# hotchpotch/open_provence

Hardware: AMD Instinct MI355X
Metric: query-context pairs/sec @ seq_len 512, xsmall-v1 (higher is better)
Workload: dtype fp16 single pass (11 significant bits per operand), fp32 accumulate

## Files before the change

include/open_provence_hip.h:

```cpp
#ifndef OPEN_PROVENCE_HIP_H
#define OPEN_PROVENCE_HIP_H

#include <stddef.h>
#include <stdint.h>

#ifdef __cplusplus
extern "C" {
#endif

#define OP_ABI_VERSION 10
#define OP_MAX_LAYERS 128

typedef struct op_handle op_handle;

enum op_status {
  OP_OK = 0,
  OP_ERR_INVALID = -1,
  OP_ERR_UNSUPPORTED = -2,
  OP_ERR_HIP = -3,
  OP_ERR_STATE = -4,
  OP_ERR_WORKSPACE = -5,
  OP_ERR_NOMEM = -6
};

enum op_dtype { OP_DTYPE_F32 = 0, OP_DTYPE_BF16 = 1, OP_DTYPE_F16 = 2 };

enum op_precision { OP_PRECISION_BF16X3 = 0, OP_PRECISION_BF16 = 1, OP_PRECISION_BF16X2 = 2, OP_PRECISION_CUSTOM = 3 };
enum op_term { OP_TERM_LEFT_LO = 1, OP_TERM_RIGHT_LO = 2 };
enum op_gemm_family {
  OP_FAM_WQKV = 0,
  OP_FAM_QK = 1,
  OP_FAM_PV = 2,
  OP_FAM_ATTN_OUT = 3,
  OP_FAM_WI = 4,
  OP_FAM_MLP_OUT = 5,
  OP_FAM_COUNT = 6
};

enum op_flags {
  OP_FLAG_FORCE_TILED = 1,
  OP_FLAG_NO_SMALL_BLOCKS = 2,
  OP_FLAG_ATT_WAVES_4 = 4,
  OP_FLAG_ATT_WAVES_8 = 8,
  OP_FLAG_NO_POLICY_KERNELS = 16,
  OP_FLAG_NO_LAYER_FUSION = 32,
  OP_FLAG_LAYER_8X16 = 64,
  OP_FLAG_NO_HEAD_FUSION = 256,
  OP_FLAG_LAYER_M32 = 128,
  OP_FLAG_ATTN_XCD_GROUP = 1024,
  OP_FLAG_PANEL_F8 = 2048,
  OP_FLAG_PANEL_F8_WI = 4096,
  OP_FLAG_NO_LAYER_PAIRS = 8192,
  OP_FLAG_NO_F8 = 512
};

enum op_pooling { OP_POOL_CLS = 0, OP_POOL_MEAN = 1 };

typedef struct op_config {
  uint32_t struct_bytes;
  int32_t device_id;
  int32_t vocab_size;
  int32_t hidden_size;
  int32_t intermediate_size;
  int32_t num_layers;
  int32_t num_heads;
  int32_t num_labels;
  int32_t local_attention;
  int32_t max_position_embeddings;
  int32_t pooling;
  int32_t precision;
  float norm_eps;
  float global_rope_theta;
  float local_rope_theta;
  int32_t chunk_rows;
  uint8_t layer_is_global[OP_MAX_LAYERS];
  uint8_t terms[8];
  uint32_t flags;
  int32_t prune_pre_final_norm;
} op_config;

int op_abi_version(void);

int op_create(const op_config* cfg, op_handle** out);

int op_load_weight(op_handle* h, const char* name, const void* data, int dtype, const int64_t* shape, int ndim);

int op_weights_ready(op_handle* h);

size_t op_workspace_bytes(const op_handle* h, int n_seqs, int total_tokens, int max_seqlen);

int op_effective_policy(op_handle* h, uint8_t* terms_out, int* kernel_set);

enum op_kernel_set {
  OP_KS_AUTO = -1,
  OP_KS_BF16X3 = 0,
  OP_KS_BF16_WEIGHTS = 1,
  OP_KS_BF16 = 2,
  OP_KS_F16_F8 = 3,
  OP_KS_F16_F8_W = 4,
  OP_KS_BF16X3_WI_F8 = 5,
  OP_KS_BF16_WEIGHTS_WI_F8 = 6,
  OP_KS_F16 = 7,
  OP_KS_F16_MLP_F8_W = 8,
  OP_KS_F16_MLP_F8 = 9,
  OP_KS_F16_F8_W_ATTN_F16 = 10,
  OP_KS_F16_F8_ATTN_F16 = 11,
  OP_KS_COUNT = 12
};

int op_select_kernel_set(op_handle* h, int kernel_set);

typedef struct op_calibration {
  uint32_t struct_bytes;
  float tolerance;
  int32_t reference_set;
  int32_t default_set;
  int32_t chosen_set;
  int32_t n_candidates;
  int32_t candidate_set[16];
  float candidate_err[16];
  int32_t n_rows, n_tokens;
  float default_err;
  uint32_t flags;
  float mlp_layers_err;
  uint64_t mlp_layers;
} op_calibration;
#define OP_CAL_FULL_REPORT 1u
#define OP_CAL_WHOLE_DEPTH 2u
int op_calibrate(op_handle* h, float tolerance, const int32_t* ids_host, const int32_t* cu_seqlens_host, int n_seqs,
                 op_calibration* report);

int op_mlp_correction_layers(op_handle* h, uint64_t* layer_mask);
int op_select_mlp_correction_layers(op_handle* h, uint64_t layer_mask);

int op_set_compact_operands(op_handle* h, int enabled, int* changed);

int op_forward_packed(op_handle* h, const int32_t* ids_dev, const int32_t* cu_seqlens_dev,
                      const int32_t* cu_seqlens_host, int n_seqs, int total_tokens, int max_seqlen,
                      float* prune_logits_dev, float* rank_logits_dev, float* keep_prob_dev,
                      void* workspace_dev, size_t workspace_bytes, void* hip_stream);

enum op_hidden_dtype { OP_HIDDEN_F32 = 0, OP_HIDDEN_BF16 = 1 };
typedef struct op_hidden_request {
  uint32_t struct_bytes;
  int32_t dtype;
  int32_t pad_width;
  const uint8_t* select;
  void* out_dev;
} op_hidden_request;
int op_forward_packed_hidden(op_handle* h, const int32_t* ids_dev, const int32_t* cu_seqlens_dev,
                             const int32_t* cu_seqlens_host, int n_seqs, int total_tokens, int max_seqlen,
                             float* prune_logits_dev, float* rank_logits_dev, float* keep_prob_dev,
                             void* workspace_dev, size_t workspace_bytes, void* hip_stream, const op_hidden_request* req);

int op_segment_means(op_handle* h, const float* keep_prob_dev, int n_values, const int32_t* seg_dev, int n_seg,
                     float* out_dev, void* hip_stream);

int op_debug_capture_hidden(op_handle* h, float* hidden_dev);

typedef struct op_profile_entry {
  int32_t kind;
  int32_t launches;
  double total_ms;
} op_profile_entry;
int op_profile_enable(op_handle* h, int enabled);
int op_profile_read(op_handle* h, op_profile_entry* entries, int max_entries);
int op_profile_reset(op_handle* h);
const char* op_profile_kind_name(int kind);

int op_debug_clock_probe(op_handle* h, int spin_us, unsigned long long* out_dev, void* hip_stream);

int op_device_count(int* count);

void op_destroy(op_handle* h);
const char* op_last_error(const op_handle* h);

#ifdef __cplusplus
}
#endif
#endif
```

open_provence_amd/_lib.py:

```python

from __future__ import annotations

import ctypes
import os
from pathlib import Path

OP_MAX_LAYERS = 128
OP_ABI_VERSION = 10

OP_OK = 0
OP_ERR_INVALID, OP_ERR_UNSUPPORTED, OP_ERR_HIP, OP_ERR_STATE, OP_ERR_WORKSPACE, OP_ERR_NOMEM = -1, -2, -3, -4, -5, -6
OP_DTYPE_F32, OP_DTYPE_BF16, OP_DTYPE_F16 = 0, 1, 2
OP_PRECISION_BF16X3, OP_PRECISION_BF16, OP_PRECISION_BF16X2, OP_PRECISION_CUSTOM = 0, 1, 2, 3
OP_TERM_LEFT_LO, OP_TERM_RIGHT_LO = 1, 2
OP_FAMILIES = ("wqkv", "qk", "pv", "attn_out", "wi", "mlp_out")
OP_FLAG_FORCE_TILED, OP_FLAG_NO_SMALL_BLOCKS, OP_FLAG_ATT_WAVES_4, OP_FLAG_ATT_WAVES_8, OP_FLAG_NO_POLICY_KERNELS = 1, 2, 4, 8, 16
OP_FLAG_NO_LAYER_FUSION = 32
OP_FLAG_LAYER_8X16 = 64
OP_FLAG_LAYER_M32 = 128
OP_FLAG_NO_HEAD_FUSION = 256
OP_FLAG_NO_F8 = 512
OP_FLAG_ATTN_XCD_GROUP = 1024
OP_FLAG_PANEL_F8 = 2048
OP_FLAG_PANEL_F8_WI = 4096
OP_FLAG_NO_LAYER_PAIRS = 8192
OP_POOL_CLS, OP_POOL_MEAN = 0, 1
OP_KS_AUTO = -1
KERNEL_SET_NAMES = {0: "bf16x3", 1: "bf16-weights", 2: "bf16", 3: "f16-f8", 4: "f16-f8-w", 5: "bf16x3+wi-f16-f8-w",
                    6: "bf16-weights+wi-f16-f8", 7: "f16", 8: "f16+mlp-f16-f8-w", 9: "f16+mlp-f16-f8",
                    10: "f16-f8-w+attn-f16", 11: "f16-f8+attn-f16",
                    -1: "all-terms kernels, cleared lo operands"}
KERNEL_SET_IDS = {name: number for number, name in KERNEL_SET_NAMES.items() if number >= 0}
FP16_PLANE_SETS = ("f16-f8", "f16-f8-w", "bf16x3+wi-f16-f8-w", "bf16-weights+wi-f16-f8", "f16", "f16+mlp-f16-f8-w", "f16+mlp-f16-f8",
                   "f16-f8-w+attn-f16", "f16-f8+attn-f16")

LIB_NAME = "libopenprovence_hip.so"

EXPORTED_SYMBOLS = (
    "op_abi_version",
    "op_create",
    "op_load_weight",
    "op_weights_ready",
    "op_effective_policy",
    "op_set_compact_operands",
    "op_select_kernel_set",
    "op_mlp_correction_layers",
    "op_select_mlp_correction_layers",
    "op_calibrate",
    "op_workspace_bytes",
    "op_forward_packed",
    "op_forward_packed_hidden",
    "op_segment_means",
    "op_debug_capture_hidden",
    "op_profile_enable",
    "op_profile_read",
    "op_profile_reset",
    "op_profile_kind_name",
    "op_device_count",
    "op_debug_clock_probe",
    "op_destroy",
    "op_last_error",
)


class HipLibraryError(RuntimeError):
    """The HIP library is missing, failed to load, or returned an error code."""


class OpConfig(ctypes.Structure):
    _fields_ = [
        ("struct_bytes", ctypes.c_uint32),
        ("device_id", ctypes.c_int32),
        ("vocab_size", ctypes.c_int32),
        ("hidden_size", ctypes.c_int32),
        ("intermediate_size", ctypes.c_int32),
        ("num_layers", ctypes.c_int32),
        ("num_heads", ctypes.c_int32),
        ("num_labels", ctypes.c_int32),
        ("local_attention", ctypes.c_int32),
        ("max_position_embeddings", ctypes.c_int32),
        ("pooling", ctypes.c_int32),
        ("precision", ctypes.c_int32),
        ("norm_eps", ctypes.c_float),
        ("global_rope_theta", ctypes.c_float),
        ("local_rope_theta", ctypes.c_float),
        ("chunk_rows", ctypes.c_int32),
        ("layer_is_global", ctypes.c_uint8 * OP_MAX_LAYERS),
        ("terms", ctypes.c_uint8 * 8),
        ("flags", ctypes.c_uint32),
        ("prune_pre_final_norm", ctypes.c_int32),
    ]


class OpCalibration(ctypes.Structure):
    _fields_ = [
        ("struct_bytes", ctypes.c_uint32),
        ("tolerance", ctypes.c_float),
        ("reference_set", ctypes.c_int32),
        ("default_set", ctypes.c_int32),
        ("chosen_set", ctypes.c_int32),
        ("n_candidates", ctypes.c_int32),
        ("candidate_set", ctypes.c_int32 * 16),
        ("candidate_err", ctypes.c_float * 16),
        ("n_rows", ctypes.c_int32),
        ("n_tokens", ctypes.c_int32),
        ("default_err", ctypes.c_float),
        ("flags", ctypes.c_uint32),
        ("mlp_layers_err", ctypes.c_float),
        ("mlp_layers", ctypes.c_uint64),
    ]


class OpHiddenRequest(ctypes.Structure):

    _fields_ = [
        ("struct_bytes", ctypes.c_uint32),
        ("dtype", ctypes.c_int32),
        ("pad_width", ctypes.c_int32),
        ("select", ctypes.POINTER(ctypes.c_uint8)),
        ("out_dev", ctypes.c_void_p),
    ]


OP_HIDDEN_F32, OP_HIDDEN_BF16 = 0, 1

OP_CAL_FULL_REPORT = 1
OP_CAL_WHOLE_DEPTH = 2


class OpProfileEntry(ctypes.Structure):
    _fields_ = [("kind", ctypes.c_int32), ("launches", ctypes.c_int32), ("total_ms", ctypes.c_double)]


def library_path() -> Path:
    override = os.environ.get("OPEN_PROVENCE_HIP_LIB")
    if override:
        return Path(override)
    return Path(__file__).resolve().parent / LIB_NAME


_LIB: ctypes.CDLL | None = None


def load_library() -> ctypes.CDLL:

    global _LIB
    if _LIB is not None:
        return _LIB
    path = library_path()
    if not path.exists():
        raise HipLibraryError(
            f"{path} not found. Build it with `python -c 'import __graft_entry__ as g; g.build()'` "
            "(hipcc --offload-arch=gfx950). There is no CPU or PyTorch fallback for the forward path."
        )
    try:
        lib = ctypes.CDLL(str(path))
    except OSError as exc:
        raise HipLibraryError(f"failed to load {path}: {exc}") from exc

    vp, ci, cs = ctypes.c_void_p, ctypes.c_int, ctypes.c_size_t
    lib.op_abi_version.restype = ci
    lib.op_abi_version.argtypes = []
    lib.op_create.restype = ci
    lib.op_create.argtypes = [ctypes.POINTER(OpConfig), ctypes.POINTER(vp)]
    lib.op_load_weight.restype = ci
    lib.op_load_weight.argtypes = [vp, ctypes.c_char_p, vp, ci, ctypes.POINTER(ctypes.c_int64), ci]
    lib.op_weights_ready.restype = ci
    lib.op_weights_ready.argtypes = [vp]
    lib.op_workspace_bytes.restype = cs
    lib.op_workspace_bytes.argtypes = [vp, ci, ci, ci]
    lib.op_forward_packed.restype = ci
    lib.op_forward_packed.argtypes = [vp, vp, vp, vp, ci, ci, ci, vp, vp, vp, vp, cs, vp]
    if hasattr(lib, "op_forward_packed_hidden"):
        lib.op_forward_packed_hidden.restype = ci
        lib.op_forward_packed_hidden.argtypes = [vp, vp, vp, vp, ci, ci, ci, vp, vp, vp, vp, cs, vp, ctypes.POINTER(OpHiddenRequest)]
    lib.op_effective_policy.restype = ci
    lib.op_effective_policy.argtypes = [vp, ctypes.POINTER(ctypes.c_uint8), ctypes.POINTER(ci)]
    if hasattr(lib, "op_set_compact_operands"):
# ... 50 lines not shown
```

open_provence_amd/csrc/op_api.hip:

```cpp
#include "../../include/open_provence_hip.h"

#include <hip/hip_runtime.h>

#include <algorithm>
#include <cmath>
#include <cstdarg>
#include <cstdio>
#include <cstdlib>
#include <cstring>
#include <string>
#include <vector>

#define OPK_PACK_KERNELS 1
#include "op_internal.h"
#include "opk_small.hip.h"
#include "opk_tiled.hip.h"

using namespace opk;
using opl::Policy;

namespace {

thread_local std::string g_last_error;

// ... 158 lines not shown

struct Launcher {
  op_handle* h;
  hipStream_t stream;
  int begin(int kind) {
    if (!h->profiling) return OP_OK;
    ProfileEvent ev;
    ev.kind = kind;
    OP_HIP(h, hipEventCreate(&ev.start));
    OP_HIP(h, hipEventCreate(&ev.stop));
    OP_HIP(h, hipEventRecord(ev.start, stream));
    h->events.push_back(ev);
    return OP_OK;
  }
  int end() {
    OP_HIP(h, hipGetLastError());
    if (!h->profiling) return OP_OK;
    OP_HIP(h, hipEventRecord(h->events.back().stop, stream));
    return OP_OK;
  }
};

#define OP_TRY(expr)             \
  do {                           \
    int _rc = (expr);            \
    if (_rc != OP_OK) return _rc; \
  } while (0)

int drain_profile(op_handle* h) {
  for (auto& ev : h->events) {
    OP_HIP(h, hipEventSynchronize(ev.stop));
    float ms = 0.f;
    OP_HIP(h, hipEventElapsedTime(&ms, ev.start, ev.stop));
    h->prof_ms[ev.kind] += ms;
    h->prof_launches[ev.kind] += 1;
    (void)hipEventDestroy(ev.start);
    (void)hipEventDestroy(ev.stop);
  }
  h->events.clear();
  return OP_OK;
}

struct Workspace {
  float* x;
  u16 *ln_hi, *ln_lo;
  u16 *q_hi, *q_lo, *k_hi, *k_lo;
  u16 *vt_hi, *vt_lo;
  u16 *o_hi, *o_lo;
  u16 *h_hi, *h_lo;
  int32_t *row_seq, *row_pos, *row_tok, *roff, *qboff, *qboff_l;
  float* cls;
  int* range_flag;
  size_t bytes;
};

int chunk_row_capacity(const op_handle* h, int n_seqs, int total_tokens, int max_seqlen) {
  const long upper = (long)total_tokens + (long)(ROW_ALIGN - 1) * n_seqs;
  const long all_rows = align_up((int)std::min<long>(upper, 1L << 30), ROW_ALIGN);
  const int one_seq = align_up(std::max(max_seqlen, 1), ROW_ALIGN);
  const long cap = std::max(h->chunk_rows, one_seq);
  return (int)std::min<long>(all_rows, cap);
}

void carve(const op_handle* h, char* base, int cap_rows_pad, int n_seqs, Workspace& ws) {
  size_t off = 0;
  auto take = [&](size_t bytes) {
    char* p = base ? base + off : nullptr;
    off += align_up_sz(bytes, 256);
    return p;
  };
  const size_t R = (size_t)cap_rows_pad;
  const size_t H = (size_t)h->H, I = (size_t)h->I;
  ws.x = (float*)take(R * H * 4);
  ws.ln_hi = (u16*)take(R * H * 2);
  ws.ln_lo = (u16*)take(R * H * 2);
  ws.q_hi = (u16*)take(R * H * 2);
  ws.q_lo = (u16*)take(R * H * 2);
  ws.k_hi = (u16*)take(R * H * 2);
  ws.k_lo = (u16*)take(R * H * 2);
  ws.vt_hi = (u16*)take(R * H * 2);
  ws.vt_lo = (u16*)take(R * H * 2);
  ws.o_hi = (u16*)take(R * H * 2);
  ws.o_lo = (u16*)take(R * H * 2);
  ws.h_hi = (u16*)take(R * I * 2);
  ws.h_lo = (u16*)take(R * I * 2);
  ws.row_seq = (int32_t*)take(R * 4);
  ws.row_pos = (int32_t*)take(R * 4);
  ws.row_tok = (int32_t*)take(R * 4);
  ws.roff = (int32_t*)take(((size_t)n_seqs + 1) * 4);
  ws.qboff = (int32_t*)take(((size_t)n_seqs + 1) * 4);
  ws.qboff_l = (int32_t*)take(((size_t)n_seqs + 1) * 4);
  ws.cls = (float*)take(std::max<size_t>((size_t)n_seqs, 1) * H * 4);
  ws.range_flag = (int*)take(sizeof(int));
  ws.bytes = off;
}

template <int EPI>
int launch_gemm(Launcher& L, int kind, const GemmParams& p, bool split) {
  OP_TRY(L.begin(kind));
  const dim3 grid((unsigned)(p.n_tiles * p.m_tiles));
  if (split)
    hipLaunchKernelGGL((gemm_kernel<EPI, true>), grid, dim3(256), 0, L.stream, p);
  else
    hipLaunchKernelGGL((gemm_kernel<EPI, false>), grid, dim3(256), 0, L.stream, p);
  return L.end();
}

int clear_lo(Launcher& L, u16* base, int unit, size_t n_pairs) {
  OP_TRY(L.begin(PK_CLEAR_LO));
  const size_t n = n_pairs * (size_t)(unit / 8);
  hipLaunchKernelGGL(zero_odd_units_kernel, dim3((unsigned)((n + 255) / 256)), dim3(256), 0, L.stream, base, unit, n_pairs);
  return L.end();
}

struct HiddenReq {
  char* out;
  int bf16, pad;
  size_t entry_bytes;
  std::vector<int> slot;
};

struct AttnPlan {
  int waves_g;
  int items_g;
  int items_l;
};

struct ChunkPass {
  op_handle* h;
  Launcher& L;
  const Workspace& ws;
  const int32_t* ids_dev;
  const int32_t* cu_dev;
  int s0, ns, rows, max_len, total_tokens;
  const AttnPlan& plan;
  float *prune_out, *rank_out, *keep_prob;
  const HiddenReq* hid;

  int H, I;
  bool fp_layout;
  int r_pad, m_tiles;
  unsigned row_blocks;
  hipStream_t st;
  Policy E, V;
  bool clr_q, clr_k, clr_v, clr_o, clr_h, clr_ln_attn, clr_ln_mlp, zero_p_lo, split;
  bool o_f8, f16, attn16, range_flagged, embed_in_qkv0;
  size_t plane_bytes;
  int q_tiles;
  bool small_blocks;
  unsigned row_grid;
  const char* no_kernel = "internal: no row-stationary kernel for hidden %d";
  bool layer_fused, head_in_last_layer;
  bool pair_layers;
  bool head_done = false;
  int hidden_stored = -1;

  ChunkPass(op_handle* h_, Launcher& L_, const Workspace& ws_, const int32_t* ids_dev_, const int32_t* cu_dev_, int s0_, int ns_, int rows_,
            int max_len_, int total_tokens_, const AttnPlan& plan_, float* prune_out_, float* rank_out_, float* keep_prob_,
            const HiddenReq* hid_)
      : h(h_), L(L_), ws(ws_), ids_dev(ids_dev_), cu_dev(cu_dev_), s0(s0_), ns(ns_), rows(rows_), max_len(max_len_),
        total_tokens(total_tokens_), plan(plan_), prune_out(prune_out_), rank_out(rank_out_), keep_prob(keep_prob_), hid(hid_) {
    H = h->H;
    I = h->I;
    fp_layout = h->row_path || h->panel_path;
    r_pad = fp_layout ? align_up(rows, ROW_BM) : align_up(rows + 64, 256);
    m_tiles = r_pad / GEMM_BM;
    row_blocks = (unsigned)((r_pad + 3) / 4);
    st = L.stream;
    E = h->eff;
    V = opl::kPolicies[h->pi];
    auto extra = [](int v, int e, int bit) { return (v & bit) != 0 && (e & bit) == 0; };
    clr_q = extra(V.qk, E.qk, 1);
    clr_k = extra(V.qk, E.qk, 2);
    clr_v = extra(V.pv, E.pv, 2);
    clr_o = extra(V.attn_out, E.attn_out, 1);
    clr_h = extra(V.mlp_out, E.mlp_out, 1);
    clr_ln_attn = extra(V.wqkv, E.wqkv, 1);
    clr_ln_mlp = extra(V.wi, E.wi, 1);
    zero_p_lo = extra(V.pv, E.pv, 1);
    split = (E.wqkv | E.qk | E.pv | E.attn_out | E.wi | E.mlp_out) != 0;
    o_f8 = (h->pi == opl::PI_F16_F8 || h->pi == opl::PI_F16_F8_W) && !h->emulate;
    f16 = h->pi == opl::PI_F16 && !h->emulate;
    attn16 = o_f8 && h->attn_f16 && h->panel_path;
    range_flagged = h->panel_path && !h->emulate && (o_f8 || (f16 && h->mlp_f8));
    embed_in_qkv0 = h->row_path && !h->capture && !(h->cfg.flags & OP_FLAG_NO_HEAD_FUSION);
    plane_bytes = (size_t)r_pad * H * sizeof(u16);
    q_tiles = (max_len + ATT_BQ - 1) / ATT_BQ;
    small_blocks = (r_pad / ROW_BM) <= h->n_cus && !(h->cfg.flags & OP_FLAG_NO_SMALL_BLOCKS);
    row_grid = (unsigned)(r_pad / (small_blocks ? 64 : ROW_BM));
    layer_fused = h->row_path && !h->emulate && opl::has_row_layer_fused(h->pi) && !(h->cfg.flags & OP_FLAG_NO_LAYER_FUSION);
    head_in_last_layer = layer_fused && h->cfg.pooling != OP_POOL_MEAN && !h->capture && !(h->cfg.flags & OP_FLAG_NO_HEAD_FUSION);
    pair_layers = layer_fused && H == 256 && I % 64 == 0 && (f16 || h->pi == 2) && !h->capture &&
                  !(h->cfg.flags & (OP_FLAG_NO_LAYER_PAIRS | OP_FLAG_LAYER_8X16 | OP_FLAG_LAYER_M32)) &&
                  h->layers[0].wo_pp[f16 ? 1 : 0] != nullptr;
  }

  int prologue() {
    OP_TRY(L.begin(PK_ROWMAP));
    hipLaunchKernelGGL(seq_offsets_kernel, dim3(1), dim3(1024), 0, st, cu_dev, s0, ns, ROW_ALIGN, ROW_ALIGN, ws.roff);
    if (fp_layout) {
      hipLaunchKernelGGL(seq_offsets_kernel, dim3(1), dim3(1024), 0, st, cu_dev, s0, ns, plan.waves_g * 32, 1, ws.qboff);
      hipLaunchKernelGGL(seq_offsets_kernel, dim3(1), dim3(1024), 0, st, cu_dev, s0, ns, 128, 1, ws.qboff_l);
    }
    hipLaunchKernelGGL(row_map_kernel, dim3((unsigned)((r_pad + 255) / 256)), dim3(256), 0, st, cu_dev, s0, ns, ws.roff,
                       r_pad, ws.row_seq, ws.row_pos, ws.row_tok);
    OP_TRY(L.end());

    if (range_flagged) OP_HIP(h, hipMemsetAsync(ws.range_flag, 0, sizeof(int), st));
    if (fp_layout && o_f8) {
      const size_t n16 = (size_t)((r_pad - rows) / 16);
      if (n16) OP_HIP(h, hipMemsetAsync(ws.o_hi + (size_t)(rows / 16) * (H / 32) * 512, 0, n16 * (H / 32) * 512 * sizeof(u16), st));
      if (n16) OP_HIP(h, hipMemsetAsync(ws.o_lo + (size_t)(rows / 16) * h->nh * 512, 0, n16 * h->nh * 512 * sizeof(u16), st));
    } else if (fp_layout) {
      const size_t tail_off = (size_t)(rows / 16) * (H / 32) * 2 * 512;
      const size_t tail_bytes = (size_t)((r_pad - rows) / 16) * (H / 32) * 2 * 512 * sizeof(u16);
      if (tail_bytes) OP_HIP(h, hipMemsetAsync(ws.o_hi + tail_off, 0, tail_bytes, st));
    } else {
      const size_t tail_off = (size_t)rows * H;
      const size_t tail_bytes = (size_t)(r_pad - rows) * H * sizeof(u16);
      if (tail_bytes) OP_HIP(h, hipMemsetAsync(ws.o_hi + tail_off, 0, tail_bytes, st));
      if (tail_bytes && split) OP_HIP(h, hipMemsetAsync(ws.o_lo + tail_off, 0, tail_bytes, st));
    }

    if (!embed_in_qkv0) {
      OP_TRY(L.begin(PK_EMBED_LN));
      if (split)
        hipLaunchKernelGGL((embed_ln_kernel<true>), dim3(row_blocks), dim3(256), 0, st, ids_dev, ws.row_tok, h->emb,
                           h->emb_norm, h->cfg.norm_eps, H, r_pad, h->V, ws.x, ws.ln_hi, ws.ln_lo);
      else
        hipLaunchKernelGGL((embed_ln_kernel<false>), dim3(row_blocks), dim3(256), 0, st, ids_dev, ws.row_tok, h->emb,
                           h->emb_norm, h->cfg.norm_eps, H, r_pad, h->V, ws.x, ws.ln_hi, ws.ln_lo);
      OP_TRY(L.end());
    }
    return OP_OK;
  }

  int capture(int index) {
    if (!h->capture) return OP_OK;
    OP_TRY(L.begin(PK_CAPTURE));
    hipLaunchKernelGGL(capture_rows_kernel, dim3(row_blocks), dim3(256), 0, st, ws.x, ws.row_tok, H, r_pad,
                       h->capture + (size_t)index * total_tokens * H);
    return L.end();
  }

  void* hidden_entry(int index) const {
    if (!hid || hid->slot[index] < 0) return nullptr;
    return hid->out + (size_t)hid->slot[index] * hid->entry_bytes;
  }
  int hidden(int index, const float* ln = nullptr) {
    void* dst = hidden_entry(index);
    if (!dst) return OP_OK;
    OP_TRY(L.begin(PK_CAPTURE));
    hipLaunchKernelGGL(hidden_rows_kernel, dim3(row_blocks), dim3(256), 0, st, ws.x, ln, h->cfg.norm_eps, H, r_pad,
                       ws.row_tok, ws.row_seq, ws.row_pos, s0, hid->pad, hid->bf16, dst);
    return L.end();
  }

  int attention(bool is_global) {
    OP_TRY(L.begin(is_global ? PK_ATTN_GLOBAL : PK_ATTN_LOCAL));
    const int window = is_global ? -1 : h->cfg.local_attention / 2;
    if (fp_layout) {
      AttnFpParams ap;
      ap.q_fp = ws.q_hi;
      ap.k_fp = ws.k_hi;
      ap.vt_fp = ws.vt_hi;
      ap.o_fp = ws.o_hi;
      ap.o_lo8 = ws.o_lo;
      ap.cu = cu_dev;
      ap.s0 = s0;
      ap.roff = ws.roff;
      ap.qboff = is_global ? ws.qboff : ws.qboff_l;
      ap.ns = ns;
      ap.H = H;
      ap.r_pad = r_pad;
      ap.window = window;
      ap.n_items = is_global ? plan.items_g : plan.items_l;
      ap.n_heads = h->nh;
      ap.xcd_group = (h->panel_path || o_f8 || (h->cfg.flags & OP_FLAG_ATTN_XCD_GROUP)) ? 1 : 0;
      ap.range_flag = range_flagged ? ws.range_flag : nullptr;
      const unsigned item_span = 8u * opk::ATT_ITEM_GROUP;
      const dim3 grid((ap.xcd_group ? ((unsigned)ap.n_items + item_span - 1) / item_span * item_span : (unsigned)ap.n_items) *
                      (unsigned)h->nh);
      if (!opl::launch_attn(st, ap, is_global ? plan.waves_g : 4, is_global ? 2 : 1, h->pi, zero_p_lo && !attn16, grid, attn16))
        return fail(h, OP_ERR_UNSUPPORTED, "internal: no attention kernel for this configuration");
    } else {
      const dim3 grid((unsigned)q_tiles, (unsigned)h->nh, (unsigned)ns);
      AttnParams ap;
      ap.q_hi = ws.q_hi;
      ap.q_lo = ws.q_lo;
      ap.k_hi = ws.k_hi;
      ap.k_lo = ws.k_lo;
      ap.vt_hi = ws.vt_hi;
      ap.vt_lo = ws.vt_lo;
      ap.o_hi = ws.o_hi;
      ap.o_lo = ws.o_lo;
      ap.cu = cu_dev;
      ap.s0 = s0;
      ap.roff = ws.roff;
      ap.H = H;
      ap.r_pad = r_pad;
      ap.window = window;
      ap.zero_p_lo = (E.pv & 1) ? 0 : 1;
      if (split)
        hipLaunchKernelGGL((attn_kernel<true>), grid, dim3(256), 0, st, ap);
      else
        hipLaunchKernelGGL((attn_kernel<false>), grid, dim3(256), 0, st, ap);
    }
    OP_TRY(L.end());
    if (fp_layout && clr_o) OP_TRY(clear_lo(L, ws.o_hi, 512, (size_t)(r_pad / 16) * (H / 32)));
    if (!fp_layout && split && !(E.attn_out & 1)) OP_HIP(h, hipMemsetAsync(ws.o_lo, 0, plane_bytes, st));
    return OP_OK;
  }
  int clear_qkv() {
    if (clr_q) OP_TRY(clear_lo(L, ws.q_hi, 512, (size_t)(r_pad / 16) * (H / 32)));
    if (clr_k) OP_TRY(clear_lo(L, ws.k_hi, 512, (size_t)(r_pad / 16) * (H / 32)));
    if (clr_v) OP_TRY(clear_lo(L, ws.vt_hi, 2048, (size_t)h->nh * (r_pad / 32)));
    return OP_OK;
  }
  int clear_h() {
    if (clr_h) OP_TRY(clear_lo(L, ws.h_hi, 512, (size_t)(r_pad / 16) * (I / 32)));
    return OP_OK;
  }

  RowGemmParams qkv_params(int li) {
    const LayerWeights& lw = h->layers[li];
    const bool is_global = h->cfg.layer_is_global[li] != 0;
    RowGemmParams rp;
    memset(&rp, 0, sizeof(rp));
    rp.eps = h->cfg.norm_eps;
    rp.hidden = H;
    rp.r_pad = r_pad;
    rp.row_pos = ws.row_pos;
    rp.rope_cos = h->rope_cos[is_global ? 1 : 0];
    rp.rope_sin = h->rope_sin[is_global ? 1 : 0];
    rp.max_pos = h->max_pos;
    rp.x_in = ws.x;
    rp.ln_w = lw.attn_norm;
    rp.wp = f16 ? lw.wqkv_h16 : lw.wqkv_pk;
    rp.n_chunks = 3 * H / ROW_CHUNK;
    rp.n_swapped = 2 * H / ROW_CHUNK;
    rp.o0_hi = ws.q_hi;
    rp.o1_hi = ws.k_hi;
    rp.o2_hi = ws.vt_hi;
    rp.ld_out = H;
    rp.zero_a_lo = clr_ln_attn ? 1 : 0;
    return rp;
  }

  int row_layer(int li) {
    const LayerWeights& lw = h->layers[li];
    const bool is_global = h->cfg.layer_is_global[li] != 0;
    if (li == 0) {
      RowGemmParams rp = qkv_params(0);
      if (embed_in_qkv0) {
        rp.emb_table = h->emb;
        rp.emb_ids = ids_dev;
        rp.emb_vocab = h->V;
        rp.row_tok = ws.row_tok;
        rp.ln_w = h->emb_norm;
        rp.x_io = ws.x;
      }
      OP_TRY(L.begin(PK_ROW_QKV));
      if (!opl::launch_row_qkv0(st, rp, H / 32, small_blocks, h->pi, row_grid)) return fail(h, OP_ERR_UNSUPPORTED, no_kernel, H);
      OP_TRY(L.end());
      OP_TRY(clear_qkv());
      if (embed_in_qkv0) OP_TRY(hidden(0));
    }
    OP_TRY(attention(is_global));

    if (layer_fused) {
      const bool with_qkv = li + 1 < h->N;
      if ((h->cfg.flags & OP_FLAG_LAYER_M32) && lw.wo_p32 && opl::has_layer32(h->pi) && I % 64 == 0) {
        Layer32Params lp;
        memset(&lp, 0, sizeof(lp));
        const LayerWeights& nx = h->layers[with_qkv ? li + 1 : li];
        lp.o_fp = ws.o_hi;
        lp.x_io = ws.x;
        lp.ln_mlp = lw.mlp_norm;
        lp.ln_next = with_qkv ? nx.attn_norm : nullptr;
        lp.eps = h->cfg.norm_eps;
        lp.wo_p = lw.wo_p32;
        lp.wi_p = lw.wi_p32;
        lp.wo2_p = lw.wo2_p32;
        lp.wqkv_p = nx.wqkv_p32;
        lp.n_pairs = I / 32;
        lp.q_fp = ws.q_hi;
        lp.k_fp = ws.k_hi;
        lp.vt_fp = ws.vt_hi;
        lp.r_pad = r_pad;
        lp.row_pos = ws.row_pos;
        const int gl = h->cfg.layer_is_global[with_qkv ? li + 1 : li] ? 1 : 0;
        lp.rope_cos = h->rope_cos[gl];
        lp.rope_sin = h->rope_sin[gl];
        lp.max_pos = h->max_pos;
        OP_TRY(L.begin(PK_FUSED_LAYER));
        if (!opl::launch_layer32(st, lp, h->pi, with_qkv, (unsigned)(r_pad / ROW_BM))) return fail(h, OP_ERR_UNSUPPORTED, no_kernel, H);
        OP_TRY(L.end());
        return OP_OK;
      }
      if (pair_layers && with_qkv) {
        Layer32Params lp;
        memset(&lp, 0, sizeof(lp));
        const LayerWeights& nx = h->layers[li + 1];
        lp.o_fp = ws.o_hi;
        lp.x_io = ws.x;
        lp.ln_mlp = lw.mlp_norm;
        lp.ln_next = nx.attn_norm;
        lp.eps = h->cfg.norm_eps;
        lp.wo_p = lw.wo_pp[f16 ? 1 : 0];
        lp.wi_p = lw.wi_pp[f16 ? 1 : 0];
        lp.wo2_p = lw.wo2_pp[f16 ? 1 : 0];
        lp.wqkv_p = nx.wqkv_pp[f16 ? 1 : 0];
        lp.n_pairs = I / 32;
        lp.q_fp = ws.q_hi;
        lp.k_fp = ws.k_hi;
        lp.vt_fp = ws.vt_hi;
        lp.r_pad = r_pad;
        lp.row_pos = ws.row_pos;
        const int gl = h->cfg.layer_is_global[li + 1] ? 1 : 0;
        lp.rope_cos = h->rope_cos[gl];
        lp.rope_sin = h->rope_sin[gl];
        lp.max_pos = h->max_pos;
        lp.hid_out = hidden_entry(li + 1);
        if (lp.hid_out) {
          lp.row_tok = ws.row_tok;
          lp.row_seq = ws.row_seq;
          lp.hid_bf16 = hid->bf16;
          lp.hid_pad = hid->pad;
          lp.hid_s0 = s0;
          hidden_stored = li + 1;
        }
        OP_TRY(L.begin(PK_FUSED_LAYER));
        if (!opl::launch_layer16p(st, lp, f16, true, li > 0, li + 2 < h->N, (unsigned)(r_pad / ROW_BM),
                                  lp.hid_out != nullptr))
          return fail(h, OP_ERR_UNSUPPORTED, no_kernel, H);
        OP_TRY(L.end());
        return OP_OK;
      }
      RowGemmParams rl = qkv_params(with_qkv ? li + 1 : li);
      rl.a1_fp = ws.o_hi;
      rl.w1p = f16 ? lw.wo_h16 : lw.wo_ks;
      rl.k1_steps = H / 32;
      rl.x_io = ws.x;
      rl.ln_w_mlp = lw.mlp_norm;
      rl.wi_pk = f16 ? lw.wi_h16 : lw.wi_pk;
      rl.wo2_ks = f16 ? lw.wo2_h16 : lw.wo2_pk;
      rl.n_pairs = I / 32;
      if (o_f8) {
        rl.a1_lo8 = ws.o_lo;
        rl.w1p = lw.wo_f16;
        rl.w1p8 = lw.wo_f8;
        rl.wi_pk = lw.wi_f8;
        rl.wo2_ks = lw.wo2_f16;
        rl.wp = h->layers[with_qkv ? li + 1 : li].wqkv_f8;
      }
      if (!with_qkv && head_in_last_layer) {
        rl.fin_ln = h->final_norm;
        rl.fin_pw = h->prune_w;
        rl.fin_pb = h->prune_b;
        rl.row_tok = ws.row_tok;
        rl.row_seq = ws.row_seq;
        rl.fin_prune = prune_out;
        rl.fin_keep = keep_prob;
        rl.fin_cls = ws.cls;
        rl.fin_pre_norm = h->cfg.prune_pre_final_norm ? 1 : 0;
        head_done = true;
        rl.hid_out = hidden_entry(h->N);
        if (rl.hid_out) {
          rl.hid_bf16 = hid->bf16;
          rl.hid_pad = hid->pad;
          rl.hid_s0 = s0;
        }
      }
      OP_TRY(L.begin(PK_FUSED_LAYER));
      if (!opl::launch_row_layer_fused(st, rl, H / 32, h->pi, with_qkv, (unsigned)(r_pad / ROW_BM),
                                       (h->cfg.flags & OP_FLAG_LAYER_8X16) != 0 || (opl::kPolicies[h->pi].wi & 1) == 0,
                                       rl.hid_out != nullptr))
        return fail(h, OP_ERR_UNSUPPORTED, no_kernel, H);
      OP_TRY(L.end());
      return OP_OK;
    }

    RowGemmParams rp;
    memset(&rp, 0, sizeof(rp));
    rp.eps = h->cfg.norm_eps;
    rp.hidden = H;
    rp.r_pad = r_pad;
    rp.ln_w = lw.mlp_norm;
    rp.wp = lw.wi_pk;
    rp.n_chunks = 2 * I / ROW_CHUNK;
    rp.o0_hi = ws.h_hi;
    rp.ld_out = I;
    rp.a1_fp = ws.o_hi;
    rp.w1p = lw.wo_ks;
    rp.k1_steps = H / 32;
    rp.x_io = ws.x;
    rp.zero_a_lo = clr_ln_mlp ? 1 : 0;
    OP_TRY(L.begin(PK_FUSED_ATTN_OUT_WI));
    if (!opl::launch_row_geglu_fused(st, rp, H / 32, small_blocks, h->pi, row_grid)) return fail(h, OP_ERR_UNSUPPORTED, no_kernel, H);
    OP_TRY(L.end());
    OP_TRY(clear_h());

    if (li + 1 < h->N) {
      RowGemmParams rq = qkv_params(li + 1);
      rq.a1_fp = ws.h_hi;
      rq.w1p = lw.wo2_pk;
      rq.k1_steps = I / 32;
      rq.x_io = ws.x;
      OP_TRY(L.begin(PK_FUSED_MLP_OUT_QKV));
      if (!opl::launch_row_qkv_fused(st, rq, H / 32, small_blocks, h->pi, row_grid)) return fail(h, OP_ERR_UNSUPPORTED, no_kernel, H);
      OP_TRY(L.end());
      OP_TRY(clear_qkv());
    } else {
      KStreamParams kp;
      kp.a_fp = ws.h_hi;
      kp.wp = lw.wo2_pk;
      kp.n_ksteps = I / 32;
      kp.x = ws.x;
      OP_TRY(L.begin(PK_KSTREAM_MLP_OUT));
      if (!opl::launch_kstream(st, kp, H / 16, h->pi, (unsigned)(r_pad / ROW_BM))) return fail(h, OP_ERR_UNSUPPORTED, no_kernel, H);
      OP_TRY(L.end());
    }
    return OP_OK;
  }

  int panel_layer(int li) {
    const LayerWeights& lw = h->layers[li];
    const bool is_global = h->cfg.layer_is_global[li] != 0;
    const dim3 ln_grid((unsigned)(r_pad / 16));
    const bool pf8 = o_f8;
    const bool mlp8 = f16 && h->mlp_f8 && (li >= 64 || ((h->mlp_layers >> li) & 1ull) != 0);
    const bool wlo8 = h->pi == opl::PI_F16_F8_W || (h->wi_f8 && h->pi == opl::PI_ALL_TERMS) || (mlp8 && h->mlp_wlo);
    auto layer_norm_fp = [&](const float* w, bool with_lo, bool clear, bool f8_here = false) -> int {
      OP_TRY(L.begin(PK_LN));
      if (pf8 || f8_here) {
        hipLaunchKernelGGL(ln_fp8_kernel, ln_grid, dim3(256), 0, st, ws.x, w, h->cfg.norm_eps, H, r_pad, w ? 1 : 0, ws.ln_hi,
                           ws.ln_lo);
        return L.end();
      }
      if (with_lo)
        hipLaunchKernelGGL((ln_fp_kernel<true>), ln_grid, dim3(256), 0, st, ws.x, w, h->cfg.norm_eps, H, r_pad,
                           w ? 1 : 0, ws.ln_hi);
      else if (f16)
        hipLaunchKernelGGL((ln_fp_kernel<false, true>), ln_grid, dim3(256), 0, st, ws.x, w, h->cfg.norm_eps, H, r_pad,
                           w ? 1 : 0, ws.ln_hi);
      else
        hipLaunchKernelGGL((ln_fp_kernel<false>), ln_grid, dim3(256), 0, st, ws.x, w, h->cfg.norm_eps, H, r_pad,
                           w ? 1 : 0, ws.ln_hi);
      OP_TRY(L.end());
      if (clear) OP_TRY(clear_lo(L, ws.ln_hi, 512, (size_t)(r_pad / 16) * (H / 32)));
      return OP_OK;
    };
    auto panel = [&](int kind, int epi, const PanelParams& pp, int n_tiles, bool f8_here = false, bool f8_full = false) -> int {
      OP_TRY(L.begin(kind));
      PanelParams q = pp;
      q.n_tiles = n_tiles;
      q.row_group = 8;
      const unsigned per_xcd = ((unsigned)(r_pad / ROW_BM) + 7) / 8;
      const unsigned groups = (per_xcd + q.row_group - 1) / q.row_group;
      const dim3 grid(8u * groups * (unsigned)q.row_group * (unsigned)n_tiles);
      const bool ok = f8_here ? opl::launch_panel_f8(st, q, 103, wlo8, grid)
                      : f8_full ? opl::launch_panel_f8(st, q, epi, wlo8, grid)
                      : pf8   ? (epi == 102 ? opl::launch_panel_f8_qkv(st, q, wlo8, attn16, grid) : opl::launch_panel_f8(st, q, epi, wlo8, grid))
                              : (epi == 102 ? opl::launch_panel_qkv(st, q, h->pi, grid) : opl::launch_panel(st, q, epi, h->pi, grid));
      if (!ok) return fail(h, OP_ERR_UNSUPPORTED, "internal: no panel kernel");
      return L.end();
    };
    OP_TRY(layer_norm_fp(li != 0 ? lw.attn_norm : nullptr, (V.wqkv & 1) != 0, clr_ln_attn));
    PanelParams pp;
    memset(&pp, 0, sizeof(pp));
    pp.r_pad = r_pad;
    pp.hidden = H;
    pp.range_flag = range_flagged ? ws.range_flag : nullptr;
    pp.row_pos = ws.row_pos;
    pp.rope_cos = h->rope_cos[is_global ? 1 : 0];
    pp.rope_sin = h->rope_sin[is_global ? 1 : 0];
    pp.max_pos = h->max_pos;
    pp.a_fp = ws.ln_hi;
    pp.a_lo8 = ws.ln_lo;
    pp.n_ksteps = H / 32;
    pp.wp = pf8 ? lw.wqkv_p16 : (f16 ? lw.wqkv_h16 : lw.wqkv_pk);
    pp.wp8 = lw.wqkv_p8;
    pp.w8_lo_off = (size_t)3 * H * H / 2;
    pp.o0 = ws.q_hi;
    pp.o1 = ws.k_hi;
    if (pf8 || !(h->cfg.flags & OP_FLAG_NO_LAYER_FUSION)) {
      pp.o2 = ws.vt_hi;
// ... 1236 lines not shown
```

open_provence_amd/csrc/op_internal.h:

```cpp
#pragma once

#include <hip/hip_runtime.h>
#include <stdint.h>

#include "opk_attn.hip.h"
#include "opk_common.hip.h"
#include "opk_layer32.hip.h"
#include "opk_layer16p.hip.h"
#include "opk_panel.hip.h"
#include "opk_rowgemm.hip.h"

namespace opl {

struct Policy {
  int wqkv, qk, pv, attn_out, wi, mlp_out;
  int fmt = 0;
  constexpr bool operator==(const Policy& o) const {
    return wqkv == o.wqkv && qk == o.qk && pv == o.pv && attn_out == o.attn_out && wi == o.wi && mlp_out == o.mlp_out;
  }
};

constexpr Policy kPolicies[] = {
    {3, 3, 3, 3, 3, 3},
    {1, 3, 3, 1, 1, 1},
    {0, 0, 0, 0, 0, 0},
    {1, 3, 3, 1, 1, 1, 1},
    {3, 3, 3, 3, 3, 3, 1},
    {0, 0, 0, 0, 0, 0, 2},
};
constexpr int PI_ALL_TERMS = 0, PI_BF16_WEIGHTS = 1, PI_BF16 = 2, PI_F16_F8 = 3, PI_F16_F8_W = 4, PI_F16 = 5;
constexpr int N_POLICIES = (int)(sizeof(kPolicies) / sizeof(kPolicies[0]));

constexpr int qkv_olo(const Policy& p) { return (p.qk & 1) | (p.qk & 2) | ((p.pv & 2) ? 4 : 0); }
constexpr int h_olo(const Policy& p) { return p.mlp_out & 1; }
constexpr bool o_lo(const Policy& p) { return (p.attn_out & 1) != 0; }

bool launch_row_qkv0(hipStream_t st, const opk::RowGemmParams& p, int ks, bool small, int pi, unsigned grid);
bool launch_row_geglu_fused(hipStream_t st, const opk::RowGemmParams& p, int ks, bool small, int pi, unsigned grid);
bool launch_row_qkv_fused(hipStream_t st, const opk::RowGemmParams& p, int ks, bool small, int pi, unsigned grid);
bool launch_kstream(hipStream_t st, const opk::KStreamParams& p, int nf, int pi, unsigned grid);
bool has_row_layer_fused(int pi);
bool launch_row_layer_fused(hipStream_t st, const opk::RowGemmParams& p, int ks, int pi, bool with_qkv, unsigned grid,
                            bool waves8, bool hout = false);
bool launch_row_layer_f8(hipStream_t st, const opk::RowGemmParams& p, int ks, bool with_qkv, unsigned grid, bool hout);
bool launch_row_layer_f8w(hipStream_t st, const opk::RowGemmParams& p, int ks, bool with_qkv, unsigned grid, bool hout);
bool launch_row_qkv0_h16(hipStream_t st, const opk::RowGemmParams& p, int ks, bool small, unsigned grid);
bool launch_row_layer_h16(hipStream_t st, const opk::RowGemmParams& p, int ks, bool with_qkv, unsigned grid, bool waves8, bool hout);
bool has_layer32(int pi);
bool launch_layer32(hipStream_t st, const opk::Layer32Params& p, int pi, bool with_qkv, unsigned grid);
bool launch_layer16p(hipStream_t st, const opk::Layer32Params& p, bool h16, bool with_qkv, bool xin_t, bool xout_t, unsigned grid,
                     bool hout = false);
bool launch_attn(hipStream_t st, const opk::AttnFpParams& p, int waves, int kt, int pi, bool zero_p_lo, dim3 grid,
                 bool f16_in_f8_out = false);
bool launch_panel(hipStream_t st, const opk::PanelParams& p, int epi, int pi, dim3 grid);
bool launch_panel_qkv(hipStream_t st, const opk::PanelParams& p, int pi, dim3 grid);
bool launch_panel_f8(hipStream_t st, const opk::PanelParams& p, int epi, bool wlo, dim3 grid);
bool launch_panel_f8_qkv(hipStream_t st, const opk::PanelParams& p, bool wlo, bool o16, dim3 grid);

}
```

open_provence_amd/csrc/op_launch_layer32.hip:

```cpp
#include "op_internal.h"

namespace opl {
using namespace opk;

namespace {
template <int PI>
bool launch_pi(hipStream_t st, const Layer32Params& p, bool with_qkv, unsigned grid) {
  constexpr Policy P = kPolicies[PI];
  constexpr bool single_plane = ((P.wqkv | P.attn_out | P.wi | P.mlp_out) & 2) == 0;
  constexpr bool uniform = (P.wqkv & 1) == (P.attn_out & 1) && (P.wi & 1) == (P.mlp_out & 1) && (P.wqkv & 1) == (P.wi & 1);
  if constexpr (!single_plane || !uniform) {
    return false;
  } else {
    constexpr bool ALO = (P.wi & 1) != 0;
    if (with_qkv) hipLaunchKernelGGL((layer32_kernel<8, true, ALO, qkv_olo(P)>), dim3(grid), dim3(256), 0, st, p);
    else hipLaunchKernelGGL((layer32_kernel<8, false, ALO, 0>), dim3(grid), dim3(256), 0, st, p);
    return true;
  }
}
}

bool has_layer32(int pi) {
  if (pi < 0 || pi >= N_POLICIES || kPolicies[pi].fmt != 0) return false;
  const Policy& P = kPolicies[pi];
  return ((P.wqkv | P.attn_out | P.wi | P.mlp_out) & 2) == 0 && (P.wqkv & 1) == (P.attn_out & 1) &&
         (P.wi & 1) == (P.mlp_out & 1) && (P.wqkv & 1) == (P.wi & 1);
}

bool launch_layer32(hipStream_t st, const Layer32Params& p, int pi, bool with_qkv, unsigned grid) {
  static_assert(N_POLICIES == 6, "extend the switch");
  switch (pi) {
    case 0: return launch_pi<0>(st, p, with_qkv, grid);
    case 1: return launch_pi<1>(st, p, with_qkv, grid);
    case 2: return launch_pi<2>(st, p, with_qkv, grid);
    case 3:
    case 4:
    case 5: return false;
    default: return false;
  }
}

bool launch_layer16p(hipStream_t st, const Layer32Params& p, bool h16, bool with_qkv, bool xin_t, bool xout_t, unsigned grid, bool hout) {
  if (hout && !with_qkv) return false;
  const dim3 g(grid), b(512);
#define OPL_L16P(H16, XI, XO)                                                                              \
  do {                                                                                                     \
    if (hout) hipLaunchKernelGGL((layer16p_hout_kernel<8, true, H16, XI, XO>), g, b, 0, st, p);            \
    else if (with_qkv) hipLaunchKernelGGL((layer16p_kernel<8, true, H16, XI, XO>), g, b, 0, st, p);        \
    else hipLaunchKernelGGL((layer16p_kernel<8, false, H16, XI, XO>), g, b, 0, st, p);                     \
  } while (0)
  if (h16) {
    if (xin_t && xout_t) OPL_L16P(true, true, true);
    else if (xin_t) OPL_L16P(true, true, false);
    else if (xout_t) OPL_L16P(true, false, true);
    else OPL_L16P(true, false, false);
  } else {
    if (xin_t && xout_t) OPL_L16P(false, true, true);
    else if (xin_t) OPL_L16P(false, true, false);
    else if (xout_t) OPL_L16P(false, false, true);
    else OPL_L16P(false, false, false);
  }
#undef OPL_L16P
  return true;
}

}
```

open_provence_amd/csrc/op_launch_row.hip:

```cpp
#include "op_internal.h"

namespace opl {
using namespace opk;

namespace {

template <int KS, int EPI, int PRO, int T1, int T2, int OLO>
void launch_shape(hipStream_t st, const RowGemmParams& p, bool small, unsigned grid) {
  if (small)
    hipLaunchKernelGGL((rowgemm_kernel<KS, EPI, PRO, T1, T2, OLO, 4, 1>), dim3(grid), dim3(256), 0, st, p);
  else
    hipLaunchKernelGGL((rowgemm_kernel<KS, EPI, PRO, T1, T2, OLO, 4, 2>), dim3(grid), dim3(256), 0, st, p);
}

template <int KS, int T1, int WAVES, int MF, int TW, int TM, int F8 = 0, bool H16 = false>
void launch_last_layer(hipStream_t st, const RowGemmParams& p, unsigned grid, bool hout) {
  if (hout)
    hipLaunchKernelGGL((rowgemm_hout_kernel<KS, RE_NONE, RP_MLP, T1, 0, 0, WAVES, MF, TW, TM, F8, H16>), dim3(grid), dim3(WAVES * 64), 0,
                       st, p);
  else
    hipLaunchKernelGGL((rowgemm_kernel<KS, RE_NONE, RP_MLP, T1, 0, 0, WAVES, MF, TW, TM, F8, H16>), dim3(grid), dim3(WAVES * 64), 0,
                       st, p);
}

template <int EPI, int PRO, int T1, int T2, int OLO>
bool launch_ks(hipStream_t st, const RowGemmParams& p, int ks, bool small, unsigned grid) {
  if (ks == 8) launch_shape<8, EPI, PRO, T1, T2, OLO>(st, p, small, grid);
  else if (ks == 4) launch_shape<4, EPI, PRO, T1, T2, OLO>(st, p, small, grid);
  else return false;
  return true;
}

}

#define OPL_SWITCH(CALL)                              \
  static_assert(N_POLICIES == 6, "extend the switch"); \
  switch (pi) {                                       \
    case 0: return CALL(0);                           \
    case 1: return CALL(1);                           \
    case 2: return CALL(2);                           \
    case 3: return CALL(1);                           \
    case 4: return CALL(0);                           \
    default: return false;                            \
  }

#if OPL_ROW_PART == 0
bool launch_row_geglu_fused(hipStream_t st, const RowGemmParams& p, int ks, bool small, int pi, unsigned grid) {
#define OPL_CALL(PI) (launch_ks<RE_GEGLU, RP_KSTREAM, kPolicies[PI].attn_out, kPolicies[PI].wi, h_olo(kPolicies[PI])>(st, p, ks, small, grid))
  OPL_SWITCH(OPL_CALL)
#undef OPL_CALL
}
#endif

#if OPL_ROW_PART == 1
bool launch_row_qkv_fused(hipStream_t st, const RowGemmParams& p, int ks, bool small, int pi, unsigned grid) {
#define OPL_CALL(PI) (launch_ks<RE_QKV, RP_KSTREAM, kPolicies[PI].mlp_out, kPolicies[PI].wqkv, qkv_olo(kPolicies[PI])>(st, p, ks, small, grid))
  OPL_SWITCH(OPL_CALL)
#undef OPL_CALL
}
#endif

#if OPL_ROW_PART == 2
bool launch_row_qkv0(hipStream_t st, const RowGemmParams& p, int ks, bool small, int pi, unsigned grid) {
  if (pi == PI_F16) return launch_row_qkv0_h16(st, p, ks, small, grid);
#define OPL_CALL(PI) (launch_ks<RE_QKV, RP_SPLIT, 0, kPolicies[PI].wqkv, qkv_olo(kPolicies[PI])>(st, p, ks, small, grid))
  OPL_SWITCH(OPL_CALL)
#undef OPL_CALL
}

namespace {
template <int T>
bool launch_kstream_t(hipStream_t st, const KStreamParams& p, int nf, unsigned grid) {
  if (nf == 16) hipLaunchKernelGGL((kstream_gemm_kernel<16, T, 4>), dim3(grid), dim3(256), 0, st, p);
  else if (nf == 8) hipLaunchKernelGGL((kstream_gemm_kernel<8, T, 4>), dim3(grid), dim3(256), 0, st, p);
  else return false;
  return true;
}
}

bool launch_kstream(hipStream_t st, const KStreamParams& p, int nf, int pi, unsigned grid) {
#define OPL_CALL(PI) (launch_kstream_t<kPolicies[PI].mlp_out>(st, p, nf, grid))
  OPL_SWITCH(OPL_CALL)
#undef OPL_CALL
}
#endif

#if OPL_ROW_PART == 3
namespace {
template <int PI, int KS>
bool launch_layer_ks(hipStream_t st, const RowGemmParams& p, bool with_qkv, unsigned grid, bool waves8, bool hout) {
  constexpr Policy P = kPolicies[PI];
  if constexpr ((P.wi & 2) != 0 || (P.mlp_out & 2) != 0) {
    return false;
  } else {
    if (waves8 && with_qkv)
      hipLaunchKernelGGL((rowgemm_kernel<KS, RE_QKV, RP_MLP, P.attn_out, P.wqkv, qkv_olo(P), 8, 1, P.wi, P.mlp_out>), dim3(grid),
                         dim3(512), 0, st, p);
    else if (waves8)
      launch_last_layer<KS, P.attn_out, 8, 1, P.wi, P.mlp_out>(st, p, grid, hout);
    else if (with_qkv)
      hipLaunchKernelGGL((rowgemm_kernel<KS, RE_QKV, RP_MLP, P.attn_out, P.wqkv, qkv_olo(P), 4, 2, P.wi, P.mlp_out>), dim3(grid),
                         dim3(256), 0, st, p);
    else
      launch_last_layer<KS, P.attn_out, 4, 2, P.wi, P.mlp_out>(st, p, grid, hout);
    return true;
  }
}
template <int PI>
bool launch_layer_pi(hipStream_t st, const RowGemmParams& p, int ks, bool with_qkv, unsigned grid, bool waves8, bool hout) {
  if (ks == 8) return launch_layer_ks<PI, 8>(st, p, with_qkv, grid, waves8, hout);
  if (ks == 4) return launch_layer_ks<PI, 4>(st, p, with_qkv, grid, waves8, hout);
  return false;
}
}

bool has_row_layer_fused(int pi) {
  return pi == PI_F16_F8_W || pi == PI_F16 || (pi >= 0 && pi < N_POLICIES && (kPolicies[pi].wi & 2) == 0 && (kPolicies[pi].mlp_out & 2) == 0);
}

bool launch_row_layer_fused(hipStream_t st, const RowGemmParams& p, int ks, int pi, bool with_qkv, unsigned grid, bool waves8, bool hout) {
  if (hout && (with_qkv || p.fin_ln == nullptr)) return false;
  if (pi == PI_F16_F8) return !waves8 && launch_row_layer_f8(st, p, ks, with_qkv, grid, hout);
  if (pi == PI_F16_F8_W) return !waves8 && launch_row_layer_f8w(st, p, ks, with_qkv, grid, hout);
  if (pi == PI_F16) return launch_row_layer_h16(st, p, ks, with_qkv, grid, waves8, hout);
#define OPL_CALL(PI) (launch_layer_pi<PI>(st, p, ks, with_qkv, grid, waves8, hout))
  OPL_SWITCH(OPL_CALL)
#undef OPL_CALL
}
#endif

#if OPL_ROW_PART == 4
namespace {
template <int KS>
void launch_layer_f8_ks(hipStream_t st, const RowGemmParams& p, bool with_qkv, unsigned grid, bool hout) {
  constexpr Policy P = kPolicies[PI_F16_F8];
  if (with_qkv)
    hipLaunchKernelGGL((rowgemm_kernel<KS, RE_QKV, RP_MLP, P.attn_out, P.wqkv, qkv_olo(P), 4, 2, P.wi, P.mlp_out, 1>), dim3(grid),
                       dim3(256), 0, st, p);
  else
    launch_last_layer<KS, P.attn_out, 4, 2, P.wi, P.mlp_out, 1>(st, p, grid, hout);
}
}

bool launch_row_layer_f8(hipStream_t st, const RowGemmParams& p, int ks, bool with_qkv, unsigned grid, bool hout) {
  if (ks == 8) launch_layer_f8_ks<8>(st, p, with_qkv, grid, hout);
  else if (ks == 4) launch_layer_f8_ks<4>(st, p, with_qkv, grid, hout);
  else return false;
  return true;
}
#endif

#if OPL_ROW_PART == 5
namespace {
template <int KS>
void launch_layer_f8w_ks(hipStream_t st, const RowGemmParams& p, bool with_qkv, unsigned grid, bool hout) {
  constexpr Policy P = kPolicies[PI_F16_F8_W];
  if (with_qkv)
    hipLaunchKernelGGL((rowgemm_kernel<KS, RE_QKV, RP_MLP, P.attn_out, P.wqkv, qkv_olo(P), 4, 2, P.wi, P.mlp_out, 2>), dim3(grid),
                       dim3(256), 0, st, p);
  else
    launch_last_layer<KS, P.attn_out, 4, 2, P.wi, P.mlp_out, 2>(st, p, grid, hout);
}
}

bool launch_row_layer_f8w(hipStream_t st, const RowGemmParams& p, int ks, bool with_qkv, unsigned grid, bool hout) {
  if (ks == 8) launch_layer_f8w_ks<8>(st, p, with_qkv, grid, hout);
  else if (ks == 4) launch_layer_f8w_ks<4>(st, p, with_qkv, grid, hout);
  else return false;
  return true;
}
#endif

#if OPL_ROW_PART == 6
namespace {
template <int KS>
void launch_qkv0_h16_ks(hipStream_t st, const RowGemmParams& p, bool small, unsigned grid) {
  if (small) hipLaunchKernelGGL((rowgemm_kernel<KS, RE_QKV, RP_SPLIT, 0, 0, 0, 4, 1, 0, 0, 0, true>), dim3(grid), dim3(256), 0, st, p);
  else hipLaunchKernelGGL((rowgemm_kernel<KS, RE_QKV, RP_SPLIT, 0, 0, 0, 4, 2, 0, 0, 0, true>), dim3(grid), dim3(256), 0, st, p);
}
template <int KS>
void launch_layer_h16_ks(hipStream_t st, const RowGemmParams& p, bool with_qkv, unsigned grid, bool waves8, bool hout) {
  if (waves8 && with_qkv)
    hipLaunchKernelGGL((rowgemm_kernel<KS, RE_QKV, RP_MLP, 0, 0, 0, 8, 1, 0, 0, 0, true>), dim3(grid), dim3(512), 0, st, p);
  else if (waves8)
    launch_last_layer<KS, 0, 8, 1, 0, 0, 0, true>(st, p, grid, hout);
  else if (with_qkv)
    hipLaunchKernelGGL((rowgemm_kernel<KS, RE_QKV, RP_MLP, 0, 0, 0, 4, 2, 0, 0, 0, true>), dim3(grid), dim3(256), 0, st, p);
  else
    launch_last_layer<KS, 0, 4, 2, 0, 0, 0, true>(st, p, grid, hout);
}
}

bool launch_row_qkv0_h16(hipStream_t st, const RowGemmParams& p, int ks, bool small, unsigned grid) {
  if (ks == 8) launch_qkv0_h16_ks<8>(st, p, small, grid);
  else if (ks == 4) launch_qkv0_h16_ks<4>(st, p, small, grid);
  else return false;
  return true;
}

bool launch_row_layer_h16(hipStream_t st, const RowGemmParams& p, int ks, bool with_qkv, unsigned grid, bool waves8, bool hout) {
  if (ks == 8) launch_layer_h16_ks<8>(st, p, with_qkv, grid, waves8, hout);
  else if (ks == 4) launch_layer_h16_ks<4>(st, p, with_qkv, grid, waves8, hout);
  else return false;
  return true;
}
#endif

}
```

open_provence_amd/csrc/opk_layer16p_body.inc:

```
  static_assert(NT == 8, "written for hidden = 256");
  static_assert(!HOUT || QKV, "the hidden-state store rides on the q / k / v^T loop's x stores");
  constexpr int H = NT * 32;
  constexpr int KP = NT;
  constexpr int CHUNK = KP * 2 * 512;
  constexpr int SLAB = NT * 2 * 512;
  constexpr int STAGE = 2 * CHUNK + SLAB;
  constexpr int STAGE_B = STAGE * 2;
  constexpr int EXTRA = 16 * 512;
  constexpr int XCH_B = STAGE_B;
  constexpr int HX_B = 2 * STAGE_B;
  constexpr int STAGE_PIECES = STAGE / 512;
  constexpr int O_PIECE0 = 80;
  constexpr int SW_ELEMS = (O_PIECE0 + 64) * 512;
  static_assert(SW_ELEMS >= 2 * STAGE + EXTRA && O_PIECE0 * 512 >= STAGE + 32 * 512, "the o pieces lie behind phase 1's stages");
  __shared__ __attribute__((aligned(16))) u16 sW[SW_ELEMS];
  __shared__ __attribute__((aligned(16))) float sLn[2 * H];
  __shared__ __attribute__((aligned(16))) float sStat[8 * 2 * 16 * 2];

  const int tid = threadIdx.x;
  const int lane = tid & 63;
  const int wave = __builtin_amdgcn_readfirstlane(tid >> 6);
  const int pw = wave & 3, hf = wave >> 2;
  const int n16 = lane & 15, g = lane >> 4;
  const int m0 = blockIdx.x * 128 + pw * 32;
  int hid_row[2] = {-1, -1};
  if constexpr (HOUT) {
#pragma unroll
    for (int mf = 0; mf < 2; ++mf) {
      const int row = m0 + 16 * mf + n16;
      const int tok = p.row_tok[row];
      if (tok >= 0) hid_row[mf] = (int)hidden_dst_row(tok, p.row_seq[row], p.row_pos[row], p.hid_pad, p.hid_s0);
    }
  }
#ifdef OPK_TIMING
  unsigned long long opk_ts[8] = {0, 0, 0, 0, 0, 0, 0, 0}, opk_wait = 0, opk_x[4] = {0, 0, 0, 0};
  const unsigned long long opk_rt0 = wall_clock64();
#define L16P_STAMP(i) opk_ts[i] = __builtin_readcyclecounter()
#else
#define L16P_STAMP(i)
#endif
  L16P_STAMP(0);
  if (hf) __builtin_amdgcn_s_setprio(1);

  const int ln_i = tid < H ? tid : H - 1;
  const float ln_fill0 = p.ln_mlp[ln_i];
  float ln_fill1 = 0.f;
  if (QKV) ln_fill1 = p.ln_next[ln_i];

  const uint32_t lds0 = (uint32_t)(uintptr_t)((__attribute__((address_space(3))) u16*)&sW[0]) + (uint32_t)lane * 16u;
  const uint32_t stat_addr = (uint32_t)(uintptr_t)((__attribute__((address_space(3))) float*)&sStat[0]);
  auto dma_piece = [&](const u16* src_piece0, int dst_piece) {
    __builtin_amdgcn_global_load_lds((const __attribute__((address_space(1))) void*)(src_piece0 + lane * 8),
                                     (__attribute__((address_space(3))) void*)(&sW[dst_piece * 512]), 16, 0, 0);
  };
  const uint32_t lane16 = (uint32_t)lane * 16u;
  auto weight_rsrc = [](const u16* base) { return __builtin_amdgcn_make_buffer_rsrc(const_cast<u16*>(base), 0, 0x7fffffff, 0x00020000); };
  const __amdgpu_buffer_rsrc_t rs_wo = weight_rsrc(p.wo_p), rs_wi = weight_rsrc(p.wi_p), rs_wo2 = weight_rsrc(p.wo2_p), rs_qkv = weight_rsrc(p.wqkv_p);
  auto dma_weight = [&](__amdgpu_buffer_rsrc_t rsrc, uint32_t byte_off, int dst_piece) {
    __builtin_amdgcn_raw_ptr_buffer_load_lds(rsrc, (__attribute__((address_space(3))) void*)(&sW[dst_piece * 512]), 16, (int)lane16, (int)byte_off, 0, 0);
  };
  const f32x4 zero4 = {0.f, 0.f, 0.f, 0.f};

  bf16x8 a[2][KP];
  const size_t rb0 = (size_t)(m0 >> 4);
#pragma unroll
  for (int j = 0; j < 8; ++j) {
    const int mf = j >> 2, kp = 4 * hf + (j & 3);
    dma_piece(p.o_fp + (((rb0 + mf) * NT + kp) * 2) * 512, O_PIECE0 + (2 * pw + mf) * 8 + kp);
  }
  auto stage_p1 = [&](int j, int stage) {
#pragma unroll
    for (int u = 0; u < 4; ++u) {
      const int piece = wave + 8 * u;
      dma_weight(rs_wo, (uint32_t)(((2 * j) * SLAB + piece * 512) * 2), stage * STAGE_PIECES + piece);
    }
  };
  stage_p1(0, 0);
  stage_p1(1, 1);
  __builtin_amdgcn_sched_barrier(0);
  float* xrow = p.x_io + (size_t)(m0 + n16) * H + 128 * hf + 8 * g;
  float* xtile = p.x_io + ((size_t)(m0 >> 5) * NT + 4 * hf) * 1024 + lane * 4;
  float4 xa[4][2][2];
#pragma unroll
  for (int i = 0; i < 4; ++i)
#pragma unroll
    for (int mf = 0; mf < 2; ++mf)
#pragma unroll
      for (int fh = 0; fh < 2; ++fh)
        xa[i][mf][fh] = XIN_T ? load_stream_f4(xtile + i * 1024 + (2 * mf + fh) * 256) : load_stream_f4(xrow + (size_t)(16 * mf) * H + 32 * i + 4 * fh);
  __builtin_amdgcn_sched_barrier(0);
  sLn[ln_i] = ln_fill0;
  sLn[H + ln_i] = ln_fill1;
  asm volatile("s_waitcnt lgkmcnt(0)" ::: "memory");
  asm volatile("s_waitcnt vmcnt(16)" ::: "memory");
  block_barrier();
#ifdef OPK_TIMING
  opk_x[0] = __builtin_readcyclecounter();
#endif
  {
    const uint32_t o_addr = lds0 + (uint32_t)(O_PIECE0 * 1024) + (uint32_t)pw * 16384u;
    static_for<16>([&](auto f_tag) {
      constexpr int f = decltype(f_tag)::value;
      a[f >> 3][f & 7] = lds_read_frag<f * 1024>(o_addr);
    });
    asm volatile("s_waitcnt lgkmcnt(0)"
                 : "+v"(a[0][0]), "+v"(a[0][1]), "+v"(a[0][2]), "+v"(a[0][3]), "+v"(a[0][4]), "+v"(a[0][5]), "+v"(a[0][6]), "+v"(a[0][7]),
                   "+v"(a[1][0]), "+v"(a[1][1]), "+v"(a[1][2]), "+v"(a[1][3]), "+v"(a[1][4]), "+v"(a[1][5]), "+v"(a[1][6]), "+v"(a[1][7]));
  }

  f32x4 acc1[4][2][2];
  struct P1Off {
    static constexpr int at(int st, int j) { return ((st >> 2) * 16 + 2 * (st & 3) + j) * 1024; }
    static constexpr int base(int, int) { return 0; }
  };
  auto p1_stage = [&](auto j_tag) {
    constexpr int j = decltype(j_tag)::value;
    const uint32_t addr[1] = {lds0 + (uint32_t)((j & 1) * STAGE_B) + (uint32_t)hf * 8192u};
    frag_stream_m<8, 2, 2, P1Off, 1>(addr, [&](auto step_tag, bf16x8(&w)[2]) {
      constexpr int st = decltype(step_tag)::value;
      constexpr int kp = 2 * j + (st >> 2), i = st & 3;
#pragma unroll
      for (int fh = 0; fh < 2; ++fh)
#pragma unroll
        for (int mf = 0; mf < 2; ++mf) acc1[i][fh][mf] = mfma16x<H16>(w[fh], a[mf][kp], kp == 0 ? zero4 : acc1[i][fh][mf]);
    });
  };
  p1_stage(std::integral_constant<int, 0>{});
  block_barrier();
  stage_p1(2, 0);
  p1_stage(std::integral_constant<int, 1>{});
  block_barrier();
  stage_p1(3, 1);
  asm volatile("s_waitcnt vmcnt(4)" ::: "memory");
  block_barrier();
  p1_stage(std::integral_constant<int, 2>{});
  asm volatile("s_waitcnt vmcnt(0)" ::: "memory");
  block_barrier();

  const int n_it = p.n_pairs;
  auto stage_piece = [&](auto u_tag, int t, int stage) {
    constexpr int u = decltype(u_tag)::value;
    const int tc = t < n_it ? t : n_it - 1;
    const int ts = t >= 2 ? (t - 2 < n_it ? t - 2 : n_it - 1) : 0;
    const int piece = wave + 8 * u;
    if constexpr (u < 4) dma_weight(rs_wi, (uint32_t)(((2 * tc) * CHUNK + piece * 512) * 2), stage * STAGE_PIECES + piece);
    else dma_weight(rs_wo2, (uint32_t)((ts * SLAB + (piece - 32) * 512) * 2), stage * STAGE_PIECES + piece);
  };
  static_for<6>([&](auto u) { stage_piece(u, 0, 0); });
  p1_stage(std::integral_constant<int, 3>{});
  block_barrier();
  L16P_STAMP(1);

  auto layer_ln = [&](auto load_tag, int which) {
    constexpr bool LOAD = decltype(load_tag)::value;
    float mean_a[2], m2_a[2];
    if constexpr (!LOAD) {
      asm volatile("s_nop 15\n\ts_nop 7"
                   : "+v"(acc1[0][0][0]), "+v"(acc1[0][0][1]), "+v"(acc1[0][1][0]), "+v"(acc1[0][1][1]), "+v"(acc1[1][0][0]), "+v"(acc1[1][0][1]),
                     "+v"(acc1[1][1][0]), "+v"(acc1[1][1][1]), "+v"(acc1[2][0][0]), "+v"(acc1[2][0][1]), "+v"(acc1[2][1][0]), "+v"(acc1[2][1][1]),
                     "+v"(acc1[3][0][0]), "+v"(acc1[3][0][1]), "+v"(acc1[3][1][0]), "+v"(acc1[3][1][1]));
    }
#pragma unroll
    for (int mf = 0; mf < 2; ++mf) {
      f32x2 v[4][4];
#pragma unroll
      for (int i = 0; i < 4; ++i)
#pragma unroll
        for (int fh = 0; fh < 2; ++fh) {
          f32x4 t = acc1[i][fh][mf];
          if constexpr (LOAD) {
            const float4 x4 = xa[i][mf][fh];
            t[0] += x4.x;
            t[1] += x4.y;
            t[2] += x4.z;
            t[3] += x4.w;
            acc1[i][fh][mf] = t;
          }
          v[i][2 * fh] = f32x2{t[0], t[1]};
          v[i][2 * fh + 1] = f32x2{t[2], t[3]};
        }
      f32x2 s4[4];
#pragma unroll
      for (int i = 0; i < 4; ++i)
#pragma unroll
        for (int q = 0; q < 4; ++q) s4[q] = i == 0 ? v[i][q] : pk_add(s4[q], v[i][q]);
      const f32x2 st2 = pk_add(pk_add(s4[0], s4[1]), pk_add(s4[2], s4[3]));
      float sum = st2.x + st2.y;
      sum += __shfl_xor(sum, 16, 64);
      sum += __shfl_xor(sum, 32, 64);
      mean_a[mf] = sum * (1.0f / 128.0f);
      const f32x2 ma2 = f32x2{mean_a[mf], mean_a[mf]};
      f32x2 q4s[4];
#pragma unroll
      for (int i = 0; i < 4; ++i)
#pragma unroll
        for (int q = 0; q < 4; ++q) {
          const f32x2 c = pk_sub(v[i][q], ma2);
          q4s[q] = i == 0 ? pk_mul(c, c) : pk_fma(c, c, q4s[q]);
        }
      const f32x2 qt2 = pk_add(pk_add(q4s[0], q4s[1]), pk_add(q4s[2], q4s[3]));
// ... 35 lines not shown
    const uint32_t oth = lds0 + (uint32_t)XCH_B + (uint32_t)(((wave ^ 4) * 8) * 1024);
    static_for<8>([&](auto f_tag) {
      constexpr int f = decltype(f_tag)::value;
      a[f >> 2][4 + (f & 3)] = lds_read_frag<f * 1024>(oth);
    });
    asm volatile("s_waitcnt lgkmcnt(0)" : "+v"(a[0][4]), "+v"(a[0][5]), "+v"(a[0][6]), "+v"(a[0][7]), "+v"(a[1][4]), "+v"(a[1][5]), "+v"(a[1][6]), "+v"(a[1][7]));
  };
  auto store_rows = [&]() {
#pragma unroll
    for (int i = 0; i < 4; ++i)
#pragma unroll
      for (int mf = 0; mf < 2; ++mf)
#pragma unroll
        for (int fh = 0; fh < 2; ++fh) {
          const f32x4 t = acc1[i][fh][mf];
          store_stream16(XOUT_T ? xtile + i * 1024 + (2 * mf + fh) * 256 : xrow + (size_t)(16 * mf) * H + 32 * i + 4 * fh, make_float4(t[0], t[1], t[2], t[3]));
        }
  };
  const std::true_type yes_{};
  const std::false_type no_{};

  layer_ln(yes_, 0);
  block_barrier();
  const uint32_t hx_pair = lds0 + (uint32_t)HX_B + (uint32_t)((pw * 2) * 1024);
  const uint32_t hx_own = hx_pair + (uint32_t)hf * 8u;
  {
    lds_write_u2(hx_own, 0u, 0u);
    lds_write_u2(hx_own + 1024u, 0u, 0u);
    lds_write_u2(hx_own + 8192u, 0u, 0u);
    lds_write_u2(hx_own + 8192u + 1024u, 0u, 0u);
  }

  f32x4 na[2][2][2];
#pragma unroll
  for (int q = 0; q < 8; ++q) na[q >> 2][(q >> 1) & 1][q & 1] = zero4;
  float gx[8], gq[8];
#pragma unroll
  for (int i = 0; i < 8; ++i) gx[i] = gq[i] = 0.f;
  const uint32_t b_lo = lds0 + (uint32_t)hf * (16384u + 8192u);
  const uint32_t b_hi = lds0 + (uint32_t)hf * (16384u - 8192u);
  const uint32_t b_wo = lds0 + 32768u + (uint32_t)hf * 8192u;
  struct MlpOff {
    static constexpr int at(int s, int j) { return j == 1 ? s * 1024 : (2 * s + (j >> 1)) * 1024; }
    static constexpr int base(int s, int j) { return j == 1 ? 2 : (s < 4 ? 0 : 1); }
  };
  struct WoOff {
    static constexpr int at(int s, int j) { return (2 * s + j) * 1024; }
    static constexpr int base(int, int) { return 0; }
  };
  auto geglu_stage = [&](auto stg_tag, const f32x4 (&src)[2][2], uint32_t dst_addr) {
    constexpr int stg = decltype(stg_tag)::value;
    static_for<8>([&](auto i_tag) {
      constexpr int i = decltype(i_tag)::value, mf = i >> 2, r = i & 3;
      if constexpr (stg == 0) {
        gx[i] = src[0][mf][r];
        gq[i] = gelu_erf_poly(0.f, fabsf(gx[i]), 0);
      } else if constexpr (stg < 5) gq[i] = gelu_erf_poly(gq[i], fabsf(gx[i]), stg);
      else if constexpr (stg == 5) gq[i] = __builtin_amdgcn_exp2f(gq[i]);
      else if constexpr (stg == 6) gq[i] = gelu_erf_finish(gq[i], gx[i]);
      else gq[i] = gq[i] * src[1][mf][r];
    });
    if constexpr (stg == 7) {
      lds_write_u2(dst_addr, pack2x<H16>(gq[0], gq[1]), pack2x<H16>(gq[2], gq[3]));
      lds_write_u2(dst_addr + 1024u, pack2x<H16>(gq[4], gq[5]), pack2x<H16>(gq[6], gq[7]));
    }
  };
  auto interleave6 = [&]() {
#pragma unroll
    for (int i = 0; i < 6; ++i) {
      __builtin_amdgcn_sched_group_barrier(0x008, 1, 0);
      __builtin_amdgcn_sched_group_barrier(0x002, 2, 0);
    }
  };
  auto end_of_stage = [&]() {
#ifdef OPK_TIMING
    const unsigned long long w0_ = __builtin_readcyclecounter();
#endif
    asm volatile("s_waitcnt vmcnt(0) lgkmcnt(0)" ::: "memory");
    block_barrier();
#ifdef OPK_TIMING
    opk_wait += __builtin_readcyclecounter() - w0_;
#endif
  };
  auto macro = [&](int t, auto par_tag) {
    constexpr int P = decltype(par_tag)::value;
    bf16x8 hb[2];
    hb[0] = lds_read_frag<0>(hx_pair + (uint32_t)(P * 8192));
    hb[1] = lds_read_frag<1024>(hx_pair + (uint32_t)(P * 8192));
    const uint32_t addr[3] = {b_lo + (uint32_t)(P * STAGE_B), b_hi + (uint32_t)(P * STAGE_B), b_wo + (uint32_t)(P * STAGE_B)};
    const uint32_t h_dst = hx_own + (uint32_t)((P ^ 1) * 8192);
    frag_stream_m<8, 3, 1, MlpOff, 3>(addr, [&](auto step_tag, bf16x8(&w)[3]) {
      constexpr int s = decltype(step_tag)::value;
      if constexpr (s == 0) asm volatile("" : "+v"(hb[0]), "+v"(hb[1]));
      if constexpr (s < 6) stage_piece(step_tag, t + 1, P ^ 1);
#pragma unroll
      for (int mf = 0; mf < 2; ++mf) na[P][0][mf] = mfma16x<H16>(w[0], a[mf][s], s == 0 ? zero4 : na[P][0][mf]);
#pragma unroll
      for (int mf = 0; mf < 2; ++mf) acc1[s >> 1][s & 1][mf] = mfma16x<H16>(w[1], hb[mf], acc1[s >> 1][s & 1][mf]);
#pragma unroll
      for (int mf = 0; mf < 2; ++mf) na[P][1][mf] = mfma16x<H16>(w[2], a[mf][s], s == 0 ? zero4 : na[P][1][mf]);
      geglu_stage(step_tag, na[P ^ 1], h_dst);
      interleave6();
    });
    end_of_stage();
  };
  asm volatile("s_waitcnt vmcnt(0) lgkmcnt(0)" ::: "memory");
  block_barrier();
  L16P_STAMP(2);
  {
    int t = 0;
    do {
      macro(t, std::integral_constant<int, 0>{});
      macro(t + 1, std::integral_constant<int, 1>{});
      t += 2;
    } while (t < n_it);
  }
  {
    bf16x8 hb[2];
    hb[0] = lds_read_frag<0>(hx_pair);
    hb[1] = lds_read_frag<1024>(hx_pair);
    {
      const uint32_t addr[1] = {b_wo};
      frag_stream_m<4, 2, 1, WoOff, 1>(addr, [&](auto step_tag, bf16x8(&w)[2]) {
        constexpr int s = decltype(step_tag)::value;
        if constexpr (s == 0) asm volatile("" : "+v"(hb[0]), "+v"(hb[1]));
        if constexpr (s < 2) stage_piece(std::integral_constant<int, 4 + s>{}, n_it + 1, 1);
#pragma unroll
        for (int fh = 0; fh < 2; ++fh)
#pragma unroll
          for (int mf = 0; mf < 2; ++mf) acc1[s][fh][mf] = mfma16x<H16>(w[fh], hb[mf], acc1[s][fh][mf]);
        geglu_stage(std::integral_constant<int, 2 * s>{}, na[1], hx_own + 8192u);
        geglu_stage(std::integral_constant<int, 2 * s + 1>{}, na[1], hx_own + 8192u);
      });
    }
    end_of_stage();
    hb[0] = lds_read_frag<0>(hx_pair + 8192u);
    hb[1] = lds_read_frag<1024>(hx_pair + 8192u);
    {
      const uint32_t addr[1] = {b_wo + (uint32_t)STAGE_B};
      frag_stream_m<4, 2, 1, WoOff, 1>(addr, [&](auto step_tag, bf16x8(&w)[2]) {
        constexpr int s = decltype(step_tag)::value;
        if constexpr (s == 0) asm volatile("" : "+v"(hb[0]), "+v"(hb[1]));
#pragma unroll
        for (int fh = 0; fh < 2; ++fh)
#pragma unroll
          for (int mf = 0; mf < 2; ++mf) acc1[s][fh][mf] = mfma16x<H16>(w[fh], hb[mf], acc1[s][fh][mf]);
      });
    }
  }
  block_barrier();
  L16P_STAMP(3);

  if constexpr (!QKV) {
    store_rows();
    L16P_STAMP(4);
  } else {
    constexpr int N_IT = 3 * NT / 2;
    constexpr int N_SW = 2 * NT / 2;
    auto stage_pair = [&](int it, int stage) {
#pragma unroll
      for (int u = 0; u < 4; ++u) {
        const int piece = wave + 8 * u;
        dma_weight(rs_qkv, (uint32_t)(((2 * it) * CHUNK + piece * 512) * 2), stage * STAGE_PIECES + piece);
      }
    };
    stage_pair(0, 0);
    f32x4 rc[2], rs[2];
#pragma unroll
    for (int mf = 0; mf < 2; ++mf) {
      int pos = p.row_pos[m0 + 16 * mf + n16];
      pos = pos < 0 ? 0 : (pos >= p.max_pos ? p.max_pos - 1 : pos);
      rc[mf] = *reinterpret_cast<const f32x4*>(p.rope_cos + (size_t)pos * ROPE_HALF + 16 * hf + 4 * g);
      rs[mf] = *reinterpret_cast<const f32x4*>(p.rope_sin + (size_t)pos * ROPE_HALF + 16 * hf + 4 * g);
    }
    layer_ln(no_, 1);
#ifdef OPK_TIMING
    opk_x[2] = __builtin_readcyclecounter();
#endif
    asm volatile("s_waitcnt vmcnt(0)" ::: "memory");
#ifdef OPK_TIMING
    opk_x[3] = __builtin_readcyclecounter();
#endif
    block_barrier();
    L16P_STAMP(4);

    struct QkvOff {
      static constexpr int at(int s, int j) { return (2 * s + j) * 1024; }
      static constexpr int base(int s, int) { return s < 4 ? 0 : 1; }
    };
    f32x4 qa[2][2][2];
    uint2 st_v[4];
    uint4 st_w[2];
    u16* st_p[2] = {nullptr, nullptr};
    float e_lo[4], e_hi[4];
    auto epilogue_slice = [&](int it, auto sw_tag, auto s_tag, const f32x4 (&c)[2][2]) {
      constexpr bool SW = decltype(sw_tag)::value;
      constexpr int s = decltype(s_tag)::value, mf = s >> 2, r = s & 3;
      if constexpr (SW) {
        const bool is_q = it < N_SW / 2;
        const float qscale = is_q ? 0.125f * 1.44269504088896340736f : 1.0f;
        const float cc = rc[mf][r], ss = rs[mf][r];
        e_lo[r] = rope_lo(c[0][mf][r], c[1][mf][r], cc, ss) * qscale;
        e_hi[r] = rope_hi(c[0][mf][r], c[1][mf][r], cc, ss) * qscale;
        if constexpr (r == 3) {
          st_v[2 * mf] = make_uint2(pack2x<H16>(e_lo[0], e_lo[1]), pack2x<H16>(e_lo[2], e_lo[3]));
          st_v[2 * mf + 1] = make_uint2(pack2x<H16>(e_hi[0], e_hi[1]), pack2x<H16>(e_hi[2], e_hi[3]));
          const int head = is_q ? it : it - N_SW / 2;
          u16* out = is_q ? p.q_fp : p.k_fp;
          st_p[mf] = out + (((rb0 + mf) * NT + 2 * head) * 2) * 512 + (16 * (2 * hf + (g >> 1)) + n16) * 8 + 4 * (g & 1);
        }
      } else {
        if constexpr (s == 7) {
#pragma unroll
          for (int fh = 0; fh < 2; ++fh)
            st_w[fh] = make_uint4(pack2x<H16>(c[fh][0][0], c[fh][0][1]), pack2x<H16>(c[fh][0][2], c[fh][0][3]),
                                  pack2x<H16>(c[fh][1][0], c[fh][1][1]), pack2x<H16>(c[fh][1][2], c[fh][1][3]));
          const size_t tb = (size_t)(m0 >> 5);
          st_p[0] = p.vt_fp + ((((size_t)(it - N_SW) * (size_t)(p.r_pad >> 5) + tb) * 2) * 4 + 2 * hf) * 512 + lane * 8;
        }
      }
    };
    auto epilogue_store = [&](auto sw_tag) {
      constexpr bool SW = decltype(sw_tag)::value;
      if constexpr (SW) {
#pragma unroll
        for (int mf = 0; mf < 2; ++mf) {
          store_stream8(st_p[mf], st_v[2 * mf]);
          store_stream8(st_p[mf] + 1024, st_v[2 * mf + 1]);
        }
      } else {
        store_stream16(st_p[0], st_w[0]);
        store_stream16(st_p[0] + 512, st_w[1]);
      }
    };
    auto interleave4 = [&]() {
#pragma unroll
      for (int i = 0; i < 4; ++i) {
        __builtin_amdgcn_sched_group_barrier(0x008, 1, 0);
        __builtin_amdgcn_sched_group_barrier(0x002, 2, 0);
      }
    };
    auto iteration = [&](auto it_tag, auto first_tag, auto sw_tag, auto swp_tag) {
      constexpr int it = decltype(it_tag)::value, cur = it & 1;
      constexpr bool FIRST = decltype(first_tag)::value, SW = decltype(sw_tag)::value, SWP = decltype(swp_tag)::value;
      constexpr bool XS = it < 8;
      stage_pair(it + 1 < N_IT ? it + 1 : it, cur ^ 1);
      __builtin_amdgcn_sched_barrier(0);
      const uint32_t addr[2] = {b_lo + (uint32_t)(cur * STAGE_B), b_hi + (uint32_t)(cur * STAGE_B)};
      frag_stream_m<8, 2, 2, QkvOff, 2>(addr, [&](auto step_tag, bf16x8(&w)[2]) {
        constexpr int s = decltype(step_tag)::value;
#pragma unroll
        for (int fh = 0; fh < 2; ++fh)
#pragma unroll
          for (int mf = 0; mf < 2; ++mf)
            qa[cur][fh][mf] = SW ? mfma16x<H16>(w[fh], a[mf][s], s == 0 ? zero4 : qa[cur][fh][mf]) : mfma16x<H16>(a[mf][s], w[fh], s == 0 ? zero4 : qa[cur][fh][mf]);
        if constexpr (!FIRST) {
          epilogue_slice(it - 1, swp_tag, step_tag, qa[cur ^ 1]);
          interleave4();
        }
      });
      if constexpr (!FIRST) epilogue_store(swp_tag);
      if constexpr (XS) {
#pragma unroll
        for (int fh = 0; fh < 2; ++fh) {
          const f32x4 t = acc1[it >> 1][fh][it & 1];
          store_stream16(XOUT_T ? xtile + (it >> 1) * 1024 + (2 * (it & 1) + fh) * 256 : xrow + (size_t)(16 * (it & 1)) * H + 32 * (it >> 1) + 4 * fh,
                       make_float4(t[0], t[1], t[2], t[3]));
        }
        if constexpr (HOUT) {
          const int hr = hid_row[it & 1];
          if (hr >= 0) {
#pragma unroll
            for (int fh = 0; fh < 2; ++fh) {
              const f32x4 t = acc1[it >> 1][fh][it & 1];
              const size_t e = (size_t)hr * H + 128 * hf + 8 * g + 32 * (it >> 1) + 4 * fh;
              if (p.hid_bf16)
                store_stream8(reinterpret_cast<u16*>(p.hid_out) + e, make_uint2(pack_bf16x2(t[0], t[1]), pack_bf16x2(t[2], t[3])));
              else
                store_stream16(reinterpret_cast<float*>(p.hid_out) + e, make_float4(t[0], t[1], t[2], t[3]));
            }
          }
        }
      }
      constexpr int N_STORES = (FIRST ? 0 : (SWP ? 4 : 2)) + (XS ? 2 : 0);
      asm volatile("s_waitcnt vmcnt(%0)" ::"n"(N_STORES) : "memory");
      block_barrier();
    };
    iteration(std::integral_constant<int, 0>{}, yes_, yes_, yes_);
    static_for<N_SW - 1>([&](auto j_tag) { iteration(std::integral_constant<int, 1 + decltype(j_tag)::value>{}, no_, yes_, yes_); });
    iteration(std::integral_constant<int, N_SW>{}, no_, no_, yes_);
    static_for<N_IT - N_SW - 1>([&](auto j_tag) { iteration(std::integral_constant<int, N_SW + 1 + decltype(j_tag)::value>{}, no_, no_, no_); });
    static_for<8>([&](auto s_tag) { epilogue_slice(N_IT - 1, no_, s_tag, qa[1]); });
    epilogue_store(no_);
  }
  L16P_STAMP(5);
#ifdef OPK_TIMING
  if (threadIdx.x == 0) {
    for (int i = 0; i < 8; ++i) p.dbg[(size_t)blockIdx.x * 16 + i] = opk_ts[i];
    p.dbg[(size_t)blockIdx.x * 16 + 8] = opk_wait;
    for (int i = 0; i < 4; ++i) p.dbg[(size_t)blockIdx.x * 16 + 11 + i] = opk_x[i];
    p.dbg[(size_t)blockIdx.x * 16 + 15] = wall_clock64() - opk_rt0;
  }
#endif
#undef L16P_STAMP
```

open_provence_amd/csrc/opk_layer32.hip.h:

```cpp
#pragma once

#include <type_traits>
#include <utility>

#include "opk_common.hip.h"

namespace opk {


typedef float f32x16 __attribute__((ext_vector_type(16)));

__device__ __forceinline__ f32x16 mfma32(bf16x8 a, bf16x8 b, f32x16 c) {
  return __builtin_amdgcn_mfma_f32_32x32x16_bf16(a, b, c, 0, 0, 0);
}

enum Layer32Pack { L32_RESID = 0, L32_GEGLU = 1, L32_QKV = 2 };

__host__ __device__ inline int l32_source_row(int mode, int T, int m, int H, int I) {
  const int j = m >> 3, hh = (m >> 2) & 1, r = m & 3;
  if (mode == L32_RESID)
    return 32 * T + 16 * (j >> 1) + 8 * hh + 4 * (j & 1) + r;
  if (mode == L32_GEGLU) {
    const int col = 16 * T + 8 * hh + 4 * (j & 1) + r;
    return j < 2 ? col : I + col;
  }
  const int per = H / 32;
  if (T < 2 * per) {
    const int blk = T / per, cc = T % per;
    const int d = 16 * (cc & 1) + 8 * hh + 4 * (j & 1) + r + (j >= 2 ? 32 : 0);
    return blk * H + (cc >> 1) * HEAD_DIM + d;
  }
  const int cv = T - 2 * per, nf = m >> 4, dd = m & 15;
  return 2 * H + (cv >> 1) * HEAD_DIM + 32 * (cv & 1) + 8 * (dd >> 2) + 4 * nf + (dd & 3);
}

#ifdef OPK_PACK_KERNELS
__global__ void pack_layer32_kernel(const float* __restrict__ src, int n_rows, int K, int mode, int kmajor, int H, int I,
                                    u16* __restrict__ dst, int f16 = 0) {
  const size_t idx = (size_t)blockIdx.x * blockDim.x + threadIdx.x;
  if (idx >= (size_t)n_rows * K) return;
  const int KS = K / 16, NT = n_rows / 32;
  size_t t = idx;
  const int e = (int)(t & 7); t >>= 3;
  const int l = (int)(t & 63); t >>= 6;
  int T, s;
  if (kmajor) {
    T = (int)(t % NT);
    s = (int)(t / NT);
  } else {
    s = (int)(t % KS);
    T = (int)(t / KS);
  }
  const int row = l32_source_row(mode, T, l & 31, H, I);
  const float v = src[(size_t)row * K + 16 * s + 8 * (l >> 5) + e];
  dst[idx] = f16 ? f2h(v) : f2bf(v);
}
#endif

struct Layer32Params {
#ifdef OPK_TIMING
  unsigned long long* dbg;
#endif
  const u16* o_fp;
  float* x_io;
  const float* ln_mlp;
  const float* ln_next;
  float eps;
  const u16* wo_p;
  const u16* wi_p;
  const u16* wo2_p;
  const u16* wqkv_p;
  int n_pairs;
  u16* q_fp;
  u16* k_fp;
  u16* vt_fp;
  int r_pad;
  const int32_t* row_pos;
  const float* rope_cos;
  const float* rope_sin;
  int max_pos;
  const int32_t* row_tok;
  const int32_t* row_seq;
  void* hid_out;
  int hid_bf16;
  int hid_pad;
  int hid_s0;
};

template <int NT, bool QKV, bool ALO, int OLO>
__global__ __launch_bounds__(256, 1) void layer32_kernel(Layer32Params p) {
  constexpr int H = NT * 32;
  constexpr int KS = NT * 2;
  constexpr int CHUNK = KS * 512;
  constexpr int SLAB = NT * 512;
  constexpr int STAGE = 2 * CHUNK + 2 * SLAB;
  static_assert(NT == 8, "written for hidden = 256 (4 waves share the DMA of a 48 KiB stage)");
  __shared__ __attribute__((aligned(16))) u16 sW[2][STAGE];
  __shared__ __attribute__((aligned(16))) float sLn[2 * H];

  const int tid = threadIdx.x;
  const int lane = tid & 63;
  const int wave = __builtin_amdgcn_readfirstlane(tid >> 6);
  const int n = lane & 31, hh = lane >> 5;
  const int m0 = blockIdx.x * 128 + wave * 32;
#ifdef OPK_TIMING
  unsigned long long opk_ts[8] = {0, 0, 0, 0, 0, 0, 0, 0}, opk_wait = 0;
  const unsigned long long opk_rt0 = wall_clock64();
#define L32_STAMP(i) opk_ts[i] = __builtin_readcyclecounter()
#else
#define L32_STAMP(i)
#endif
  L32_STAMP(0);

  const int ln_i = tid < H ? tid : H - 1;
  const float ln_fill0 = p.ln_mlp[ln_i];
  float ln_fill1 = 0.f;
  if (QKV) ln_fill1 = p.ln_next[ln_i];

  uint32_t lds_stage[2];
  lds_stage[0] = (uint32_t)(uintptr_t)((__attribute__((address_space(3))) u16*)&sW[0][0]) + (uint32_t)lane * 16u;
  lds_stage[1] = lds_stage[0] + (uint32_t)(STAGE * 2);
  auto dma_piece = [&](const u16* src_piece0, int stage, int dst_piece) {
    __builtin_amdgcn_global_load_lds((const __attribute__((address_space(1))) void*)(src_piece0 + lane * 8),
                                     (__attribute__((address_space(3))) void*)(&sW[stage][dst_piece * 512]), 16, 0, 0);
  };

  bf16x8 a_hi[KS], a_lo[KS];
  {
    const u16* o_base = p.o_fp + ((size_t)((m0 >> 4) + (n >> 4)) * NT * 2) * 512 + (16 * hh + (n & 15)) * 8;
#pragma unroll
    for (int ks = 0; ks < KS; ++ks) {
      const u16* src = o_base + ((ks >> 1) * 2) * 512 + (ks & 1) * 256;
      a_hi[ks] = load_stream_frag(src);
      a_lo[ks] = ALO ? load_stream_frag(src + 512) : a_hi[ks];
    }
  }
  auto stage_p1 = [&](int j, int stage) {
#pragma unroll
    for (int u = 0; u < NT; ++u) {
      const int piece = wave + 4 * u;
      dma_piece(p.wo_p + (size_t)(4 * j) * SLAB + piece * 512, stage, piece);
    }
  };
  stage_p1(0, 0);
  __builtin_amdgcn_sched_barrier(0);
  float* xrow = p.x_io + (size_t)(m0 + n) * H + 8 * hh;
  float4 xa[NT / 2][2][2];
#pragma unroll
  for (int T = 0; T < NT / 2; ++T)
#pragma unroll
    for (int jj = 0; jj < 2; ++jj)
#pragma unroll
      for (int q4 = 0; q4 < 2; ++q4) xa[T][jj][q4] = load_stream_f4(xrow + 32 * T + 16 * jj + 4 * q4);
  __builtin_amdgcn_sched_barrier(0);
  sLn[ln_i] = ln_fill0;
  sLn[H + ln_i] = ln_fill1;
  asm volatile("s_waitcnt lgkmcnt(0)" ::: "memory");
  asm volatile("s_waitcnt vmcnt(%0)" ::"n"(NT * 2) : "memory");
  __builtin_amdgcn_s_barrier();

  f32x16 acc1[NT];
  {
    struct P1Off {
      static constexpr int at(int st, int j) { return ((st >> 2) * NT + 2 * (st & 3) + j) * 1024; }
    };
    static_for<KS / 4>([&](auto j_tag) {
      constexpr int j = decltype(j_tag)::value;
      constexpr int cur = j & 1;
      if constexpr (j + 1 < KS / 4) stage_p1(j + 1, cur ^ 1);
      __builtin_amdgcn_sched_barrier(0);
      frag_stream2<16, 2, P1Off>(lds_stage[cur], [&](auto step_tag, bf16x8& w0, bf16x8& w1) {
        constexpr int st = decltype(step_tag)::value;
        constexpr int ks = 4 * j + (st >> 2), T = 2 * (st & 3);
        const f32x16 zero = {0.f, 0.f, 0.f, 0.f, 0.f, 0.f, 0.f, 0.f, 0.f, 0.f, 0.f, 0.f, 0.f, 0.f, 0.f, 0.f};
        if (ALO) {
          acc1[T] = mfma32(w0, a_lo[ks], ks == 0 ? zero : acc1[T]);
          acc1[T + 1] = mfma32(w1, a_lo[ks], ks == 0 ? zero : acc1[T + 1]);
        }
        acc1[T] = mfma32(w0, a_hi[ks], (ks == 0 && !ALO) ? zero : acc1[T]);
        acc1[T + 1] = mfma32(w1, a_hi[ks], (ks == 0 && !ALO) ? zero : acc1[T + 1]);
      });
      __syncthreads();
    });
  }
  L32_STAMP(1);

  auto layer_ln = [&](auto load_tag, auto lo_tag, int which) {
    constexpr bool LOAD = decltype(load_tag)::value, LO = decltype(lo_tag)::value;
    float4 xb[LOAD ? NT / 2 : 1][2][2];
    if (LOAD) {
#pragma unroll
      for (int T = NT / 2; T < NT; ++T)
#pragma unroll
        for (int jj = 0; jj < 2; ++jj)
#pragma unroll
          for (int q4 = 0; q4 < 2; ++q4) xb[LOAD ? T - NT / 2 : 0][jj][q4] = load_stream_f4(xrow + 32 * T + 16 * jj + 4 * q4);
    }
    const uint32_t ln_addr = (uint32_t)(uintptr_t)((__attribute__((address_space(3))) float*)&sLn[0]) + (uint32_t)(which * H + 8 * hh) * 4u;
    f32x4 wq[2][2];
    auto ln_read = [&](auto st_tag) {
      constexpr int st = decltype(st_tag)::value;
      wq[st & 1][0] = lds_read_f4<(32 * (st >> 1) + 16 * (st & 1)) * 4>(ln_addr);
      wq[st & 1][1] = lds_read_f4<(32 * (st >> 1) + 16 * (st & 1)) * 4 + 16>(ln_addr);
    };
    f32x2 v[NT][8];
    f32x2 s4[4];
#pragma unroll
    for (int T = 0; T < NT; ++T) {
      f32x16 a = acc1[T];
      if (LOAD) {
#pragma unroll
        for (int jj = 0; jj < 2; ++jj)
#pragma unroll
          for (int q4 = 0; q4 < 2; ++q4) {
            const float4 x4 = T < NT / 2 ? xa[T < NT / 2 ? T : 0][jj][q4] : xb[(LOAD && T >= NT / 2) ? T - NT / 2 : 0][jj][q4];
            a[8 * jj + 4 * q4 + 0] += x4.x;
            a[8 * jj + 4 * q4 + 1] += x4.y;
            a[8 * jj + 4 * q4 + 2] += x4.z;
            a[8 * jj + 4 * q4 + 3] += x4.w;
          }
        acc1[T] = a;
      }
#pragma unroll
      for (int pp = 0; pp < 8; ++pp) {
        v[T][pp] = f32x2{a[2 * pp], a[2 * pp + 1]};
        s4[pp & 3] = (T == 0 && pp < 4) ? v[T][pp] : pk_add(s4[pp & 3], v[T][pp]);
      }
    }
    const f32x2 st = pk_add(pk_add(s4[0], s4[1]), pk_add(s4[2], s4[3]));
    float sum = st.x + st.y;
    sum += __shfl_xor(sum, 32, 64);
    const float mean = sum * (1.0f / (float)H);
    const f32x2 m2 = f32x2{mean, mean};
    f32x2 q4s[4];
#pragma unroll
    for (int T = 0; T < NT; ++T)
#pragma unroll
      for (int pp = 0; pp < 8; ++pp) {
        v[T][pp] = pk_sub(v[T][pp], m2);
// ... 333 lines not shown
```

open_provence_amd/csrc/opk_rowgemm.hip.h:

```cpp
#pragma once

#include "opk_rowgemm_pack.hip.h"
#include "opk_rowgemm_stream.hip.h"
#include "opk_rowgemm_ln.hip.h"

namespace opk {

template <int KS, int EPI, int PRO, int T1, int T2, int OLO, int WAVES, int MF, int TW, int TM, int F8, bool H16, bool HOUT = false>
struct RowGemmBlock {
  static constexpr bool WLO = F8 == 2;
  static_assert(!H16 || (F8 == 0 && T1 == 0 && T2 == 0 && OLO == 0 && TW == 0 && TM == 0 && PRO != RP_KSTREAM && EPI != RE_GEGLU),
                "fp16 operands: the single-pass whole-layer / layer-0 q/k/v kernels only");
  static constexpr int TF8 = WLO ? 3 : T_LEFT_LO;
  static_assert(!F8 || (PRO == RP_MLP && WAVES == 4 && MF == 2 && KS % 4 == 0 && T1 == TF8 && TW == TF8 && TM == TF8 &&
                        (EPI == RE_NONE || T2 == TF8)),
                "f16 + fp8 kernel sets: whole-layer kernel, 4 waves x 32 rows, every activation lo term (+ F8 = 2: every weight lo term)");
  static constexpr int NS8 = F8 ? KS / 4 : 1;
  static_assert(MF == 1 || MF == 2, "one or two 16-row fragments per wave");
  static constexpr bool W_LO = !F8 && (T2 & T_RIGHT_LO) != 0, A_LO = (T2 & T_LEFT_LO) != 0;
  static constexpr bool PHASE1 = PRO == RP_KSTREAM || PRO == RP_MLP;
  static constexpr bool W_LO1 = !F8 && PHASE1 && (T1 & T_RIGHT_LO) != 0, A_LO1 = PHASE1 && (T1 & T_LEFT_LO) != 0;
  static_assert(PRO != RP_MLP || (((WAVES == 4 && MF == 2) || (WAVES == 8 && MF == 1)) && (WLO || ((TW & T_RIGHT_LO) == 0 && (TM & T_RIGHT_LO) == 0))),
                "fused MLP: 4 waves x 32 rows or 8 waves x 16 rows, single-plane Wi and Wo");
  static constexpr int PLANES = W_LO ? 2 : 1;
  static constexpr int PLANES1 = W_LO1 ? 2 : 1;
  static constexpr int K = KS * 32;
  static constexpr int CHUNK_PIECES8 = F8Chunk<KS, WLO>::PIECES;
  static constexpr int CHUNK_SRC = F8 ? F8Chunk<KS, WLO>::SRC_PIECES * 512 : KS * 2 * 1024;
  static constexpr int STAGE = F8 ? CHUNK_PIECES8 * 512 : KS * PLANES * 1024;
  static constexpr int MLP_UNIT = PRO == RP_MLP ? (WLO ? (CHUNK_PIECES8 + 2 * KS) * 512 : F8 ? (2 * CHUNK_PIECES8 + 2 * KS) * 512 : 3 * KS * 1024) : 0;
  static constexpr int STAGE_GEMM = WLO ? 8 * KS * 512 : F8 ? 6 * KS * 512 : KS * (PLANES > PLANES1 ? PLANES : PLANES1) * 1024;
  static constexpr int STAGE_ALLOC = STAGE_GEMM > MLP_UNIT ? STAGE_GEMM : MLP_UNIT;
  static_assert(STAGE % (WAVES * 512) == 0, "stage must split evenly over the waves");
  static constexpr bool LN_V2 = PRO == RP_MLP;
  static_assert(!F8 || LN_V2, "f16 + fp8 kernel set: LayerNorm phases of the whole-layer kernel");
  static constexpr bool FIN_HEAD = LN_V2 && EPI == RE_NONE;
  static constexpr int SLN_SIZE = LN_V2 ? (FIN_HEAD ? 4 : 2) * KS * 32 : 4;
  static constexpr int WAVE_PIECES = STAGE / (WAVES * 512);
  static constexpr bool QKV2 = PRO == RP_MLP && EPI == RE_QKV && !F8 && H16 && 2 * STAGE <= STAGE_ALLOC;
  static constexpr bool QKV_PAIRS = F8 != 0 && EPI == RE_QKV;
  static constexpr int FRAG_ILV = 4;
  static constexpr int PAIR_DMA = QKV_PAIRS ? 2 * CHUNK_PIECES8 / WAVES : 1;
  static constexpr int PAIR_GS = (2 * CHUNK_PIECES8 / 4) % WAVES == 0 ? 4 : 2;
  static_assert(!QKV_PAIRS || (CHUNK_PIECES8 % PAIR_GS == 0 && (2 * CHUNK_PIECES8 / PAIR_GS) % WAVES == 0 && 2 * STAGE <= STAGE_ALLOC),
                "a chunk pair is whole groups of pieces per wave and fits one LDS stage");
  static constexpr bool ROPE_PRELOAD = EPI == RE_QKV && PRO == RP_MLP;

  const RowGemmParams& p;
  u16 (&sW)[2][STAGE_ALLOC];
  float (&sLn)[SLN_SIZE];
  int tid, lane, wave, l15, g, m0, ln_i;
  float ln_fill0 = 0.f, ln_fill1 = 0.f, ln_fill2 = 0.f, ln_fill3 = 0.f;
  bf16x8 a_hi[MF][KS], a_lo[MF][KS];
  i32x8 a_lo8[MF][NS8];
  i32x8 a_h8[MF][NS8];
  const float* rope_c_row[MF];
  const float* rope_s_row[MF];
  f32x4 rope_c[MF], rope_s[MF];
  f32x4 rope_cc[MF][2], rope_ss[MF][2];
  static constexpr int NF1 = 2 * KS;
  f32x4 acc1[NF1][MF];
  float4 xq0[(PRO == RP_MLP) ? NF1 : 1];
  static constexpr bool MLP_REGS_IN_BLOCK = PRO == RP_MLP && WAVES == 8 && F8 == 0 && T1 == 0 && TW == 0 && TM == 0;
  struct MlpRegs {
    f32x4 acc_b[2][MF];
    uint2 hold_hi[MF];
    uint2 hold_lo[MF];
    bf16x8 h_hi[MF];
    bf16x8 h_lo[MF];
    float g_prev[MF][4];
    float g_cur[MF][4];
    float gx[MF * 4];
    float gq[MF * 4];
    uint2 pk_hi[MF];
    float pk_d[MF][4];
    f32x4 nbv[2][MF];
  } mlp_regs;
  uint32_t lds_stage[2];
#ifdef OPK_TIMING
  unsigned long long opk_ts[8] = {0, 0, 0, 0, 0, 0, 0, 0}, opk_wait = 0, opk_wait2 = 0, opk_wait1 = 0, opk_x[4] = {0, 0, 0, 0}, opk_rt0 = 0;
#ifdef OPK_SEG_TIMING
  unsigned long long opk_seg[3] = {0, 0, 0}, opk_seg_t = 0;
#endif
#endif

  __device__ __forceinline__ RowGemmBlock(const RowGemmParams& p_, u16 (&sW_)[2][STAGE_ALLOC], float (&sLn_)[SLN_SIZE]) : p(p_), sW(sW_), sLn(sLn_) {}

  __device__ __forceinline__ void stage_chunk(int chunk, int stage) {
    const u16* src = p.wp + (size_t)chunk * CHUNK_SRC;
    if constexpr (F8 != 0) {
      constexpr int PIECES = STAGE / 512;
      constexpr int GS = (PIECES / 4) % WAVES == 0 ? 4 : ((PIECES / 2) % WAVES == 0 ? 2 : 1);
      static_for<WAVE_PIECES>([&](auto u_tag) {
        constexpr int u = decltype(u_tag)::value;
        const int piece0 = GS * (wave + WAVES * (u / GS));
        __builtin_amdgcn_global_load_lds((const __attribute__((address_space(1))) void*)(src + piece0 * 512 + lane * 8),
                                         (__attribute__((address_space(3))) void*)(&sW[stage][piece0 * 512]), 16, (u % GS) * 1024, 0);
      });
      return;
    }
#pragma unroll
    for (int u = 0; u < WAVE_PIECES; ++u) {
      const int piece = wave + WAVES * u;
      const int elem = piece * 512;
      const int ks = elem / (PLANES * 1024);
      const int rem = elem % (PLANES * 1024);
      const int src_elem = F8 ? elem : ks * 2048 + rem;
      __builtin_amdgcn_global_load_lds(
          (const __attribute__((address_space(1))) void*)(src + src_elem + lane * 8),
          (__attribute__((address_space(3))) void*)(&sW[stage][elem]), 16, 0, 0);
    }
  }
  __device__ __forceinline__ void stage_chunk_at(int chunk, int stage, int elem_off) {
    const u16* src = p.wp + (size_t)chunk * CHUNK_SRC;
#pragma unroll
    for (int u = 0; u < WAVE_PIECES; ++u) {
      const int elem = (wave + WAVES * u) * 512;
      const int src_elem = (elem / 1024) * 2048 + elem % 1024;
      __builtin_amdgcn_global_load_lds((const __attribute__((address_space(1))) void*)(src + src_elem + lane * 8),
                                       (__attribute__((address_space(3))) void*)(&sW[stage][elem_off + elem]), 16, 0, 0);
    }
  }
  template <class UTag>
  __device__ __forceinline__ void stage_pair_piece(UTag u_tag, int pair, int stage) {
    constexpr int u = decltype(u_tag)::value;
    const int piece0 = PAIR_GS * (wave + WAVES * (u / PAIR_GS));
    const int second = piece0 >= CHUNK_PIECES8 ? 1 : 0;
    const u16* src = p.wp + (size_t)(2 * pair + second) * CHUNK_SRC + (piece0 - second * CHUNK_PIECES8) * 512 + lane * 8;
    __builtin_amdgcn_global_load_lds((const __attribute__((address_space(1))) void*)src,
                                     (__attribute__((address_space(3))) void*)(&sW[0][0] + stage * STAGE_ALLOC + piece0 * 512), 16,
                                     (u % PAIR_GS) * 1024, 0);
  }
  __device__ __forceinline__ void stage_pair(int pair, int stage) {
    static_for<PAIR_DMA>([&](auto u_tag) { stage_pair_piece(u_tag, pair, stage); });
  }
  __device__ __forceinline__ void rope_rows() {
#pragma unroll
    for (int mf = 0; mf < MF; ++mf) {
      int pos = p.row_pos[m0 + mf * 16 + l15];
      pos = pos < 0 ? 0 : (pos >= p.max_pos ? p.max_pos - 1 : pos);
      rope_c_row[mf] = p.rope_cos + (size_t)pos * ROPE_HALF + g * 8;
      rope_s_row[mf] = p.rope_sin + (size_t)pos * ROPE_HALF + g * 8;
      rope_c[mf] = rope_s[mf] = f32x4{0.f, 0.f, 0.f, 0.f};
    }
  }
  __device__ __forceinline__ void rope_preload() {
#pragma unroll
    for (int mf = 0; mf < MF; ++mf)
#pragma unroll
      for (int j = 0; j < 2; ++j) {
        rope_cc[mf][j] = *reinterpret_cast<const f32x4*>(rope_c_row[mf] + j * 4);
        rope_ss[mf][j] = *reinterpret_cast<const f32x4*>(rope_s_row[mf] + j * 4);
      }
  }

#ifdef OPK_SEG_TIMING
#define OPK_SEG_DUMP() for (int i_ = 0; i_ < 3; ++i_) p.dbg[(size_t)blockIdx.x * 16 + 11 + i_] = opk_seg[i_];
#else
#define OPK_SEG_DUMP()
#endif
#ifdef OPK_TIMING
#ifdef OPK_SEG_TIMING
#endif
#define OPK_STAMP(i) opk_ts[i] = __builtin_readcyclecounter()
#define OPK_DUMP()                                                                              \
  do {                                                                                          \
    if (threadIdx.x == 0) {                                                                     \
      for (int i_ = 0; i_ < 8; ++i_) p.dbg[(size_t)blockIdx.x * 16 + i_] = opk_ts[i_];          \
      p.dbg[(size_t)blockIdx.x * 16 + 8] = opk_wait;                                            \
      p.dbg[(size_t)blockIdx.x * 16 + 9] = opk_wait2;                                           \
      p.dbg[(size_t)blockIdx.x * 16 + 10] = opk_wait1;                                          \
      for (int i_ = 0; i_ < 4; ++i_) p.dbg[(size_t)blockIdx.x * 16 + 11 + i_] = opk_x[i_];     \
      OPK_SEG_DUMP()                                                                            \
      p.dbg[(size_t)blockIdx.x * 16 + 15] = wall_clock64() - opk_rt0;                           \
    }                                                                                           \
  } while (0)
#else
#define OPK_STAMP(i)
#define OPK_DUMP()
#endif

  __device__ __forceinline__ void phase1();
  __device__ __forceinline__ void mlp_phase();
  __device__ __forceinline__ void qkv_pairs_loop();
  __device__ __forceinline__ void chunk_loop();
  template <class LoadTag, class StoreTag, class LoTag>
  __device__ __forceinline__ void residual_ln(LoadTag, StoreTag, LoTag, const float* __restrict__ lnw) {
    rowgemm_residual_ln<KS, MF, PRO, LoadTag::value, StoreTag::value, LoTag::value>(p, m0, l15, g, lnw, acc1, xq0, a_hi, a_lo);
  }
  template <class LoadTag, class LoTag>
  __device__ __forceinline__ void layer_ln(LoadTag, LoTag, int which) {
    const uint32_t sln_addr = (uint32_t)(uintptr_t)((__attribute__((address_space(3))) float*)&sLn[0]);
#ifdef OPK_TIMING
    unsigned long long* const stamps = opk_x;
#else
    unsigned long long* const stamps = nullptr;
#endif
    rowgemm_layer_ln<KS, MF, F8, H16, LoadTag::value, LoTag::value>(p, m0, l15, g, sln_addr, which, acc1, xq0, a_hi, a_lo, a_lo8, a_h8, stamps);
  }
  __device__ __forceinline__ void store_rows() { rowgemm_store_rows<KS, MF>(p, m0, l15, g, acc1); }

  __device__ __forceinline__ void run() {
    tid = threadIdx.x;
    lane = tid & 63;
    wave = __builtin_amdgcn_readfirstlane(tid >> 6);
    l15 = lane & 15;
    g = lane >> 4;
    m0 = blockIdx.x * (WAVES * 16 * MF) + wave * (16 * MF);
    ln_i = tid < KS * 32 ? tid : KS * 32 - 1;
    if constexpr (LN_V2) {
      ln_fill0 = p.ln_w_mlp[ln_i];
      if (EPI != RE_NONE) ln_fill1 = p.ln_w[ln_i];
      if (FIN_HEAD && p.fin_ln != nullptr) {
        ln_fill1 = p.fin_ln[ln_i];
        ln_fill2 = p.fin_pw[ln_i];
        ln_fill3 = p.fin_pw[KS * 32 + ln_i];
      }
    }
#ifdef OPK_TIMING
    opk_rt0 = wall_clock64();
    OPK_STAMP(0);
#endif
    if constexpr (F8) set_saturating_conversions();
    if (ROPE_PRELOAD) rope_rows();
    lds_stage[0] = (uint32_t)(uintptr_t)((__attribute__((address_space(3))) u16*)&sW[0][0]) + (uint32_t)lane * 16u;
    lds_stage[1] = lds_stage[0] + (uint32_t)(STAGE_ALLOC * 2);
    if (PHASE1) {
      phase1();
      OPK_STAMP(1);
      const std::true_type yes_{};
      const std::false_type no_{};
      if constexpr (PRO == RP_KSTREAM) {
        stage_chunk(0, 0);
        residual_ln(yes_, yes_, std::integral_constant<bool, A_LO>{}, p.ln_w);
      } else {
        mlp_phase();
        if constexpr (EPI == RE_NONE) {
          if (FIN_HEAD && p.fin_ln != nullptr) rowgemm_final_head<KS, MF, HOUT>(p, sLn, m0, l15, g, acc1);
          else residual_ln(no_, yes_, no_, nullptr);
          OPK_STAMP(4);
          OPK_DUMP();
          return;
        } else {
          if constexpr (QKV_PAIRS) stage_pair(0, 0);
          else stage_chunk(0, 0);
          if constexpr (QKV2) stage_chunk_at(1, 0, STAGE);
          if (ROPE_PRELOAD) rope_preload();
          if constexpr (LN_V2) {
            layer_ln(no_, std::integral_constant<bool, A_LO>{}, 1);
#ifdef OPK_TIMING
            opk_x[2] = __builtin_readcyclecounter();
#endif
            asm volatile("s_waitcnt vmcnt(0)" ::: "memory");
#ifdef OPK_TIMING
            opk_x[3] = __builtin_readcyclecounter();
#endif
            store_rows();
          } else {
            residual_ln(no_, yes_, std::integral_constant<bool, A_LO>{}, p.ln_w);
          }
          OPK_STAMP(4);
        }
      }
    } else {
      stage_chunk(0, 0);
    }

    rowgemm_prologue_rows<KS, MF, PRO, A_LO, H16>(p, m0, l15, g, a_hi, a_lo);
    if (EPI == RE_QKV && !ROPE_PRELOAD) rope_rows();
    if constexpr (LN_V2) __builtin_amdgcn_s_barrier();
    else __syncthreads();

    if constexpr (QKV_PAIRS) qkv_pairs_loop();
    else chunk_loop();
  }
};

}

#define OPK_RG_TPL template <int KS, int EPI, int PRO, int T1, int T2, int OLO, int WAVES, int MF, int TW, int TM, int F8, bool H16, bool HOUT>
#define OPK_RG_BLOCK RowGemmBlock<KS, EPI, PRO, T1, T2, OLO, WAVES, MF, TW, TM, F8, H16, HOUT>
#include "opk_rowgemm_phase1.hip.h"
#include "opk_rowgemm_mlp.hip.h"
#include "opk_rowgemm_qkv_pairs.hip.h"
#include "opk_rowgemm_chunks.hip.h"
#undef OPK_RG_TPL
#undef OPK_RG_BLOCK
#undef OPK_STAMP
#undef OPK_DUMP

namespace opk {

template <int KS, int EPI, int PRO, int T1, int T2, int OLO, int WAVES, int MF = 2, int TW = 0, int TM = 0, int F8 = 0, bool H16 = false>
__global__ __launch_bounds__(WAVES * 64, PRO == RP_MLP ? (WAVES == 8 ? 2 : 1) : ((MF == 1 && WAVES == 8) ? 4 : 2)) void rowgemm_kernel(RowGemmParams p) {
  using Block = RowGemmBlock<KS, EPI, PRO, T1, T2, OLO, WAVES, MF, TW, TM, F8, H16>;
  __shared__ __attribute__((aligned(16))) u16 sW[2][Block::STAGE_ALLOC];
  __shared__ __attribute__((aligned(16))) float sLn[Block::SLN_SIZE];
  Block block(p, sW, sLn);
  block.run();
}

template <int KS, int EPI, int PRO, int T1, int T2, int OLO, int WAVES, int MF = 2, int TW = 0, int TM = 0, int F8 = 0, bool H16 = false>
__global__ __launch_bounds__(WAVES * 64, PRO == RP_MLP ? (WAVES == 8 ? 2 : 1) : ((MF == 1 && WAVES == 8) ? 4 : 2)) void rowgemm_hout_kernel(RowGemmParams p) {
  static_assert(EPI == RE_NONE && PRO == RP_MLP, "entry N is stored by the head epilogue of the last whole-layer launch");
  using Block = RowGemmBlock<KS, EPI, PRO, T1, T2, OLO, WAVES, MF, TW, TM, F8, H16, true>;
  __shared__ __attribute__((aligned(16))) u16 sW[2][Block::STAGE_ALLOC];
  __shared__ __attribute__((aligned(16))) float sLn[Block::SLN_SIZE];
  Block block(p, sW, sLn);
  block.run();
}

}

#include "opk_kstream.hip.h"
```

open_provence_amd/csrc/opk_rowgemm_ln.hip.h:

```cpp
#pragma once

#include "opk_rowgemm_stream.hip.h"

namespace opk {

template <int KS, int MF, int PRO, bool LOAD, bool STORE, bool LO, int NX>
__device__ __forceinline__ void rowgemm_residual_ln(const RowGemmParams& p, int m0, int l15, int g, const float* __restrict__ lnw,
                                                    f32x4 (&acc1)[2 * KS][MF], const float4 (&xq0)[NX], bf16x8 (&a_hi)[MF][KS],
                                                    bf16x8 (&a_lo)[MF][KS]) {
  constexpr int K = KS * 32, NF1 = 2 * KS;
  constexpr bool XPRE = LOAD && PRO == RP_MLP;
  float4 xq1[(XPRE && MF > 1) ? NF1 : 1];
  if (XPRE && MF > 1) {
    const float* xrow1 = p.x_io + (size_t)(m0 + 16 + l15) * K + g * 8;
#pragma unroll
    for (int nf = 0; nf < NF1; ++nf) xq1[nf] = load_stream_f4(xrow1 + 32 * (nf >> 1) + 4 * (nf & 1));
  }
#pragma unroll
  for (int mf = 0; mf < MF; ++mf) {
    float* xrow = p.x_io + (size_t)(m0 + mf * 16 + l15) * K + g * 8;
    float sum = 0.f;
#pragma unroll
    for (int nf = 0; nf < NF1; ++nf) {
      float4* px = reinterpret_cast<float4*>(xrow + 32 * (nf >> 1) + 4 * (nf & 1));
      float4 r4 = make_float4(acc1[nf][mf][0], acc1[nf][mf][1], acc1[nf][mf][2], acc1[nf][mf][3]);
      if (LOAD) {
        const float4 x4 = XPRE ? (mf == 0 ? xq0[nf] : xq1[(XPRE && MF > 1) ? nf : 0]) : load_stream_f4(reinterpret_cast<const float*>(px));
        r4.x += x4.x;
        r4.y += x4.y;
        r4.z += x4.z;
        r4.w += x4.w;
        acc1[nf][mf] = f32x4{r4.x, r4.y, r4.z, r4.w};
      }
      if (STORE) store_stream16(reinterpret_cast<float*>(px), r4);
      sum += (r4.x + r4.y) + (r4.z + r4.w);
      if (((LOAD && !XPRE) || STORE) && (nf & 3) == 3) __builtin_amdgcn_sched_barrier(0);
    }
    if (lnw == nullptr) continue;
    sum += __shfl_xor(sum, 16, 64);
    sum += __shfl_xor(sum, 32, 64);
    const float mean = sum / (float)K;
    float q = 0.f;
#pragma unroll
    for (int nf = 0; nf < NF1; ++nf)
#pragma unroll
      for (int r = 0; r < 4; ++r) {
        const float d = acc1[nf][mf][r] - mean;
        q += d * d;
      }
    q += __shfl_xor(q, 16, 64);
    q += __shfl_xor(q, 32, 64);
    const float rstd = 1.0f / sqrtf(q / (float)K + p.eps);
#pragma unroll
    for (int ks = 0; ks < KS; ++ks) {
      const float4 w0 = *reinterpret_cast<const float4*>(lnw + ks * 32 + g * 8);
      const float4 w1 = *reinterpret_cast<const float4*>(lnw + ks * 32 + g * 8 + 4);
      const float v[8] = {(acc1[2 * ks][mf][0] - mean) * rstd * w0.x,     (acc1[2 * ks][mf][1] - mean) * rstd * w0.y,
                          (acc1[2 * ks][mf][2] - mean) * rstd * w0.z,     (acc1[2 * ks][mf][3] - mean) * rstd * w0.w,
                          (acc1[2 * ks + 1][mf][0] - mean) * rstd * w1.x, (acc1[2 * ks + 1][mf][1] - mean) * rstd * w1.y,
                          (acc1[2 * ks + 1][mf][2] - mean) * rstd * w1.z, (acc1[2 * ks + 1][mf][3] - mean) * rstd * w1.w};
      pack8<LO>(v, a_hi[mf][ks], a_lo[mf][ks]);
    }
  }
}

template <int KS, int MF, int F8, bool H16, bool LOAD, bool LO, int NS8, int NX>
__device__ __forceinline__ void rowgemm_layer_ln(const RowGemmParams& p, int m0, int l15, int g, uint32_t sln_addr, int which,
                                                 f32x4 (&acc1)[2 * KS][MF], const float4 (&xq0)[NX], bf16x8 (&a_hi)[MF][KS],
                                                 bf16x8 (&a_lo)[MF][KS], i32x8 (&a_lo8)[MF][NS8], i32x8 (&a_h8)[MF][NS8],
                                                 unsigned long long* stamps) {
  constexpr int K = KS * 32, NF1 = 2 * KS;
  constexpr bool WLO = F8 == 2;
  float4 xq1[(LOAD && MF > 1) ? NF1 : 1];
  if (LOAD && MF > 1) {
    const float* xrow1 = p.x_io + (size_t)(m0 + 16 + l15) * K + g * 8;
#pragma unroll
    for (int nf = 0; nf < NF1; ++nf) xq1[nf] = load_stream_f4(xrow1 + 32 * (nf >> 1) + 4 * (nf & 1));
  }
  const uint32_t ln_addr = sln_addr + (uint32_t)(which * K + g * 8) * 4u;
  f32x4 wq[2][2];
  auto ln_read = [&](auto ks_tag) {
    constexpr int ks = decltype(ks_tag)::value;
    wq[ks & 1][0] = lds_read_f4<ks * 128>(ln_addr);
    wq[ks & 1][1] = lds_read_f4<ks * 128 + 16>(ln_addr);
  };
#pragma unroll
  for (int mf = 0; mf < MF; ++mf) {
    f32x2 v[2 * NF1];
#pragma unroll
    for (int nf = 0; nf < NF1; ++nf) {
      f32x4 a = acc1[nf][mf];
      if (LOAD) {
        const float4 x4 = mf == 0 ? xq0[nf] : xq1[(LOAD && MF > 1) ? nf : 0];
        a = f32x4{a[0] + x4.x, a[1] + x4.y, a[2] + x4.z, a[3] + x4.w};
        acc1[nf][mf] = a;
      }
      v[2 * nf] = f32x2{a[0], a[1]};
      v[2 * nf + 1] = f32x2{a[2], a[3]};
    }
    f32x2 s4[4] = {v[0], v[1], v[2], v[3]};
#pragma unroll
    for (int i = 4; i < 2 * NF1; ++i) s4[i & 3] = pk_add(s4[i & 3], v[i]);
    const f32x2 st = pk_add(pk_add(s4[0], s4[1]), pk_add(s4[2], s4[3]));
    float sum = st.x + st.y;
    sum += __shfl_xor(sum, 16, 64);
    sum += __shfl_xor(sum, 32, 64);
    const float mean = sum * (1.0f / (float)K);
    const f32x2 m2 = f32x2{mean, mean};
    f32x2 q4[4];
#pragma unroll
    for (int i = 0; i < 2 * NF1; ++i) {
      v[i] = pk_sub(v[i], m2);
      q4[i & 3] = i < 4 ? pk_mul(v[i], v[i]) : pk_fma(v[i], v[i], q4[i & 3]);
    }
    const f32x2 qt = pk_add(pk_add(q4[0], q4[1]), pk_add(q4[2], q4[3]));
    float q = qt.x + qt.y;
    q += __shfl_xor(q, 16, 64);
    q += __shfl_xor(q, 32, 64);
    const float rstd = 1.0f / sqrtf(q * (1.0f / (float)K) + p.eps);
    const f32x2 r2 = f32x2{rstd, rstd};
    ln_read(std::integral_constant<int, 0>{});
    if constexpr (KS > 1) ln_read(std::integral_constant<int, 1>{});
    static_for<KS>([&](auto ks_tag) {
      constexpr int ks = decltype(ks_tag)::value;
      f32x4& w0 = wq[ks & 1][0];
      f32x4& w1 = wq[ks & 1][1];
      lds_wait_f4<(ks + 1 < KS ? 2 : 0)>(w0, w1);
      const f32x2 lw[4] = {f32x2{w0[0], w0[1]}, f32x2{w0[2], w0[3]}, f32x2{w1[0], w1[1]}, f32x2{w1[2], w1[3]}};
      if constexpr (F8) {
        f32x2 y[4];
#pragma unroll
        for (int j = 0; j < 4; ++j) y[j] = pk_mul(pk_mul(v[4 * ks + j], r2), lw[j]);
        const float va[4] = {y[0].x, y[0].y, y[1].x, y[1].y}, vb[4] = {y[2].x, y[2].y, y[3].x, y[3].y};
        uint2 h0, h1;
        uint32_t l0, l1;
        split4_f8(va, h0, l0);
        split4_f8(vb, h1, l1);
        a_hi[mf][ks] = as_frag(make_uint4(h0.x, h0.y, h1.x, h1.y));
        constexpr int d0 = 4 * ((ks % 4) / 2) + 2 * (ks % 2);
        a_lo8[mf][ks / 4][d0] = (int)l0;
        a_lo8[mf][ks / 4][d0 + 1] = (int)l1;
        if constexpr (WLO) {
          a_h8[mf][ks / 4][d0] = (int)f32x4_to_e4m3(va);
          a_h8[mf][ks / 4][d0 + 1] = (int)f32x4_to_e4m3(vb);
        }
        if constexpr (LOAD && (ks % 4) == 3) {
          asm volatile("" : "+a"(a_lo8[mf][ks / 4]));
          if constexpr (WLO) asm volatile("" : "+a"(a_h8[mf][ks / 4]));
        }
      } else {
      uint32_t h[4], l[4];
#pragma unroll
      for (int j = 0; j < 4; ++j) split2x_pk<LO, H16>(pk_mul(pk_mul(v[4 * ks + j], r2), lw[j]), h[j], l[j]);
      a_hi[mf][ks] = as_frag(make_uint4(h[0], h[1], h[2], h[3]));
      a_lo[mf][ks] = as_frag(make_uint4(l[0], l[1], l[2], l[3]));
      if constexpr (LO && LOAD && MF == 2) asm volatile("" : "+a"(a_lo[mf][ks]));
      }
      if constexpr (ks + 2 < KS) ln_read(std::integral_constant<int, ks + 2>{});
    });
    if (stamps != nullptr && mf == 0) stamps[LOAD ? 0 : 1] = __builtin_readcyclecounter();
  }
}

template <int KS, int MF>
__device__ __forceinline__ void rowgemm_store_rows(const RowGemmParams& p, int m0, int l15, int g, const f32x4 (&acc1)[2 * KS][MF]) {
  constexpr int K = KS * 32, NF1 = 2 * KS;
#pragma unroll
  for (int mf = 0; mf < MF; ++mf) {
    float* xrow = p.x_io + (size_t)(m0 + mf * 16 + l15) * K + g * 8;
#pragma unroll
    for (int nf = 0; nf < NF1; ++nf)
      store_stream16(xrow + 32 * (nf >> 1) + 4 * (nf & 1),
                     make_float4(acc1[nf][mf][0], acc1[nf][mf][1], acc1[nf][mf][2], acc1[nf][mf][3]));
  }
}

template <int KS, int MF, int PRO, bool A_LO, bool H16>
__device__ __forceinline__ void rowgemm_prologue_rows(const RowGemmParams& p, int m0, int l15, int g, bf16x8 (&a_hi)[MF][KS],
                                                      bf16x8 (&a_lo)[MF][KS]) {
  constexpr int K = KS * 32;
  if (PRO == RP_SPLIT && p.emb_table != nullptr) {
    const float* lnw_g = p.ln_w + g * 8;
#pragma unroll
    for (int mf = 0; mf < MF; ++mf) {
      const int row = m0 + mf * 16 + l15;
      const int tok = p.row_tok[row];
      int id = p.emb_ids[tok < 0 ? 0 : tok];
      id = id < 0 ? 0 : (id >= p.emb_vocab ? p.emb_vocab - 1 : id);
      const float* src = p.emb_table + (size_t)id * K + g * 8;
      const float live = tok < 0 ? 0.f : 1.f;
      const f32x2 live2 = f32x2{live, live};
      f32x2 v[4 * KS];
#pragma unroll
      for (int ks = 0; ks < KS; ++ks) {
        const float4 f0 = *reinterpret_cast<const float4*>(src + ks * 32);
        const float4 f1 = *reinterpret_cast<const float4*>(src + ks * 32 + 4);
        v[4 * ks + 0] = pk_mul(f32x2{f0.x, f0.y}, live2);
        v[4 * ks + 1] = pk_mul(f32x2{f0.z, f0.w}, live2);
        v[4 * ks + 2] = pk_mul(f32x2{f1.x, f1.y}, live2);
        v[4 * ks + 3] = pk_mul(f32x2{f1.z, f1.w}, live2);
      }
      f32x2 s4[4] = {v[0], v[1], v[2], v[3]};
#pragma unroll
      for (int i = 4; i < 4 * KS; ++i) s4[i & 3] = pk_add(s4[i & 3], v[i]);
      const f32x2 st = pk_add(pk_add(s4[0], s4[1]), pk_add(s4[2], s4[3]));
      float sum = st.x + st.y;
      sum += __shfl_xor(sum, 16, 64);
      sum += __shfl_xor(sum, 32, 64);
      const float mean = sum * (1.0f / (float)K);
      const f32x2 m2 = f32x2{mean, mean};
      f32x2 q4[4];
#pragma unroll
      for (int i = 0; i < 4 * KS; ++i) {
        v[i] = pk_sub(v[i], m2);
        q4[i & 3] = i < 4 ? pk_mul(v[i], v[i]) : pk_fma(v[i], v[i], q4[i & 3]);
      }
      const f32x2 qt = pk_add(pk_add(q4[0], q4[1]), pk_add(q4[2], q4[3]));
      float q = qt.x + qt.y;
      q += __shfl_xor(q, 16, 64);
      q += __shfl_xor(q, 32, 64);
      const float rstd = 1.0f / sqrtf(q * (1.0f / (float)K) + p.eps);
      const f32x2 r2 = f32x2{rstd, rstd};
      float* xrow = p.x_io + (size_t)row * K + g * 8;
#pragma unroll
      for (int ks = 0; ks < KS; ++ks) {
        const float4 w0 = *reinterpret_cast<const float4*>(lnw_g + ks * 32);
        const float4 w1 = *reinterpret_cast<const float4*>(lnw_g + ks * 32 + 4);
        const f32x2 lw[4] = {f32x2{w0.x, w0.y}, f32x2{w0.z, w0.w}, f32x2{w1.x, w1.y}, f32x2{w1.z, w1.w}};
        f32x2 y[4];
        uint32_t hb[4], lb[4];
#pragma unroll
        for (int j = 0; j < 4; ++j) {
          y[j] = pk_mul(pk_mul(v[4 * ks + j], r2), lw[j]);
          split2x_pk<A_LO, H16>(y[j], hb[j], lb[j]);
        }
        store_stream16(xrow + ks * 32, make_float4(y[0].x, y[0].y, y[1].x, y[1].y));
        store_stream16(xrow + ks * 32 + 4, make_float4(y[2].x, y[2].y, y[3].x, y[3].y));
        a_hi[mf][ks] = as_frag(make_uint4(hb[0], hb[1], hb[2], hb[3]));
        a_lo[mf][ks] = as_frag(make_uint4(lb[0], lb[1], lb[2], lb[3]));
      }
    }
  } else if (PRO == RP_SPLIT) {
#pragma unroll
    for (int mf = 0; mf < MF; ++mf) {
      const size_t row = (size_t)(m0 + mf * 16 + l15);
#pragma unroll
      for (int ks = 0; ks < KS; ++ks) {
        const float4 f0 = load_stream_f4(p.x_in + row * K + ks * 32 + g * 8);
        const float4 f1 = load_stream_f4(p.x_in + row * K + ks * 32 + g * 8 + 4);
        const float v[8] = {f0.x, f0.y, f0.z, f0.w, f1.x, f1.y, f1.z, f1.w};
        pack8x<A_LO, H16>(v, a_hi[mf][ks], a_lo[mf][ks]);
      }
    }
  }
  if (A_LO && PRO != RP_MLP) {
    const unsigned keep = p.zero_a_lo ? 0u : 0xffffffffu;
#pragma unroll
    for (int mf = 0; mf < MF; ++mf)
#pragma unroll
      for (int ks = 0; ks < KS; ++ks) {
        FragU f;
        f.v = a_lo[mf][ks];
        f.u = make_uint4(f.u.x & keep, f.u.y & keep, f.u.z & keep, f.u.w & keep);
        a_lo[mf][ks] = f.v;
      }
  }
}

}
```

open_provence_amd/csrc/opk_small.hip.h:

```cpp
#pragma once

#include "opk_common.hip.h"

namespace opk {

__global__ __launch_bounds__(1024) void seq_offsets_kernel(const int32_t* __restrict__ cu, int s0, int ns, int unit,
                                                           int scale, int32_t* __restrict__ roff) {
  __shared__ int sh[1024];
  __shared__ int carry;
  const int tid = threadIdx.x;
  if (tid == 0) carry = 0;
  __syncthreads();
  for (int base = 0; base < ns; base += 1024) {
    const int i = base + tid;
    int v = 0;
    if (i < ns) {
      const int len = cu[s0 + i + 1] - cu[s0 + i];
      v = (len + unit - 1) / unit * scale;
    }
    sh[tid] = v;
    __syncthreads();
    for (int off = 1; off < 1024; off <<= 1) {
      const int t = tid >= off ? sh[tid - off] : 0;
      __syncthreads();
// ... 29 lines not shown
  }
  const int pos = r - roff[lo];
  const int start = cu[s0 + lo];
  const int len = cu[s0 + lo + 1] - start;
  row_seq[r] = lo;
  if (pos < len) {
    row_pos[r] = pos;
    row_tok[r] = start + pos;
  } else {
    row_pos[r] = -1;
    row_tok[r] = -1;
  }
}

constexpr int LN_MAX_CHUNKS = 4;

struct RowVec {
  float4 v[LN_MAX_CHUNKS];
};

__device__ __forceinline__ void row_load(const float* __restrict__ src, int H, int lane, RowVec& rv) {
  const int nchunk = H >> 2;
#pragma unroll
  for (int k = 0; k < LN_MAX_CHUNKS; ++k) {
    const int c = lane + 64 * k;
    rv.v[k] = (c < nchunk) ? reinterpret_cast<const float4*>(src)[c] : make_float4(0.f, 0.f, 0.f, 0.f);
  }
}

__device__ __forceinline__ void row_layer_norm(RowVec& rv, const float* __restrict__ w, int H, int lane, float eps) {
  const int nchunk = H >> 2;
  float s = 0.f;
#pragma unroll
  for (int k = 0; k < LN_MAX_CHUNKS; ++k) s += (rv.v[k].x + rv.v[k].y) + (rv.v[k].z + rv.v[k].w);
  const float mean = wave_sum(s) / (float)H;
  float q = 0.f;
#pragma unroll
  for (int k = 0; k < LN_MAX_CHUNKS; ++k) {
    const int c = lane + 64 * k;
    if (c < nchunk) {
      const float a = rv.v[k].x - mean, b = rv.v[k].y - mean, cc = rv.v[k].z - mean, d = rv.v[k].w - mean;
      q += (a * a + b * b) + (cc * cc + d * d);
    }
  }
  const float var = wave_sum(q) / (float)H;
  const float rstd = 1.0f / sqrtf(var + eps);
#pragma unroll
  for (int k = 0; k < LN_MAX_CHUNKS; ++k) {
    const int c = lane + 64 * k;
    if (c < nchunk) {
      const float4 ww = reinterpret_cast<const float4*>(w)[c];
      rv.v[k].x = (rv.v[k].x - mean) * rstd * ww.x;
      rv.v[k].y = (rv.v[k].y - mean) * rstd * ww.y;
      rv.v[k].z = (rv.v[k].z - mean) * rstd * ww.z;
      rv.v[k].w = (rv.v[k].w - mean) * rstd * ww.w;
    }
  }
}

template <bool SPLIT>
__device__ __forceinline__ void row_store_planes(const RowVec& rv, u16* __restrict__ hi, u16* __restrict__ lo, int H,
                                                 int lane) {
  const int nchunk = H >> 2;
#pragma unroll
  for (int k = 0; k < LN_MAX_CHUNKS; ++k) {
    const int c = lane + 64 * k;
    if (c < nchunk) {
      const float v[4] = {rv.v[k].x, rv.v[k].y, rv.v[k].z, rv.v[k].w};
      uint2 h2, l2;
      split4<SPLIT>(v, h2, l2);
      reinterpret_cast<uint2*>(hi)[c] = h2;
      if (SPLIT) reinterpret_cast<uint2*>(lo)[c] = l2;
    }
  }
}

__device__ __forceinline__ void row_store_f32(const RowVec& rv, float* __restrict__ dst, int H, int lane) {
  const int nchunk = H >> 2;
#pragma unroll
  for (int k = 0; k < LN_MAX_CHUNKS; ++k) {
    const int c = lane + 64 * k;
    if (c < nchunk) reinterpret_cast<float4*>(dst)[c] = rv.v[k];
  }
}

template <bool SPLIT>
__global__ __launch_bounds__(256) void embed_ln_kernel(const int32_t* __restrict__ ids,
                                                       const int32_t* __restrict__ row_tok,
                                                       const float* __restrict__ table, const float* __restrict__ lnw,
                                                       float eps, int H, int r_pad, int vocab, float* __restrict__ x,
                                                       u16* __restrict__ a_hi, u16* __restrict__ a_lo) {
  const int lane = threadIdx.x & 63;
  const int row = blockIdx.x * 4 + (threadIdx.x >> 6);
  if (row >= r_pad) return;
  const int tok = row_tok[row];
  RowVec rv;
  if (tok < 0) {
#pragma unroll
    for (int k = 0; k < LN_MAX_CHUNKS; ++k) rv.v[k] = make_float4(0.f, 0.f, 0.f, 0.f);
  } else {
    int id = ids[tok];
    id = id < 0 ? 0 : (id >= vocab ? vocab - 1 : id);
    row_load(table + (size_t)id * H, H, lane, rv);
    row_layer_norm(rv, lnw, H, lane, eps);
  }
  row_store_f32(rv, x + (size_t)row * H, H, lane);
  row_store_planes<SPLIT>(rv, a_hi + (size_t)row * H, a_lo + (size_t)row * H, H, lane);
}

template <bool SPLIT>
__global__ __launch_bounds__(256) void ln_kernel(const float* __restrict__ x, const float* __restrict__ lnw, float eps,
                                                 int H, int r_pad, u16* __restrict__ a_hi, u16* __restrict__ a_lo) {
  const int lane = threadIdx.x & 63;
  const int row = blockIdx.x * 4 + (threadIdx.x >> 6);
  if (row >= r_pad) return;
  RowVec rv;
  row_load(x + (size_t)row * H, H, lane, rv);
  row_layer_norm(rv, lnw, H, lane, eps);
  row_store_planes<SPLIT>(rv, a_hi + (size_t)row * H, a_lo + (size_t)row * H, H, lane);
}

__global__ __launch_bounds__(256) void capture_rows_kernel(const float* __restrict__ x,
                                                           const int32_t* __restrict__ row_tok, int H, int r_pad,
                                                           float* __restrict__ out) {
  const int lane = threadIdx.x & 63;
  const int row = blockIdx.x * 4 + (threadIdx.x >> 6);
  if (row >= r_pad) return;
  const int tok = row_tok[row];
  if (tok < 0) return;
  RowVec rv;
  row_load(x + (size_t)row * H, H, lane, rv);
  row_store_f32(rv, out + (size_t)tok * H, H, lane);
}

__global__ __launch_bounds__(256) void hidden_rows_kernel(const float* __restrict__ x, const float* __restrict__ lnw, float eps,
                                                          int H, int r_pad, const int32_t* __restrict__ row_tok,
                                                          const int32_t* __restrict__ row_seq, const int32_t* __restrict__ row_pos,
                                                          int s0, int pad, int bf16, void* __restrict__ out) {
  const int lane = threadIdx.x & 63;
  const int row = blockIdx.x * 4 + (threadIdx.x >> 6);
  if (row >= r_pad) return;
  const int tok = row_tok[row];
  if (tok < 0) return;
  RowVec rv;
  row_load(x + (size_t)row * H, H, lane, rv);
  if (lnw) row_layer_norm(rv, lnw, H, lane, eps);
  const size_t base = hidden_dst_row(tok, row_seq[row], row_pos[row], pad, s0) * (size_t)H;
  const int nchunk = H >> 2;
#pragma unroll
  for (int k = 0; k < LN_MAX_CHUNKS; ++k) {
    const int c = lane + 64 * k;
    if (c < nchunk) hidden_store4(out, bf16, base + 4 * c, rv.v[k].x, rv.v[k].y, rv.v[k].z, rv.v[k].w);
  }
}

__global__ __launch_bounds__(256) void final_ln_prune_kernel(float* __restrict__ x, const float* __restrict__ lnw,
                                                             float eps, int H, int r_pad,
                                                             const int32_t* __restrict__ row_tok,
                                                             const int32_t* __restrict__ row_seq,
                                                             const int32_t* __restrict__ row_pos,
                                                             const float* __restrict__ pw, const float* __restrict__ pb,
                                                             float* __restrict__ prune_out, float* __restrict__ keep_prob,
                                                             int pre_norm, int keep_all_rows, float* __restrict__ cls,
                                                             float* __restrict__ capture, const int* __restrict__ range_flag) {
  const int lane = threadIdx.x & 63;
  const int row = blockIdx.x * 4 + (threadIdx.x >> 6);
  if (row >= r_pad) return;
  const int tok = row_tok[row];
  if (tok < 0) return;
  RowVec rv;
  row_load(x + (size_t)row * H, H, lane, rv);
  const int nchunk = H >> 2;
  float d0 = 0.f, d1 = 0.f;
  auto head_dot = [&]() {
#pragma unroll
    for (int k = 0; k < LN_MAX_CHUNKS; ++k) {
      const int c = lane + 64 * k;
      if (c < nchunk) {
        const float4 w0 = reinterpret_cast<const float4*>(pw)[c];
        const float4 w1 = reinterpret_cast<const float4*>(pw + H)[c];
        d0 += (rv.v[k].x * w0.x + rv.v[k].y * w0.y) + (rv.v[k].z * w0.z + rv.v[k].w * w0.w);
        d1 += (rv.v[k].x * w1.x + rv.v[k].y * w1.y) + (rv.v[k].z * w1.z + rv.v[k].w * w1.w);
      }
    }
  };
  if (pre_norm) head_dot();
  row_layer_norm(rv, lnw, H, lane, eps);
  if (!pre_norm) head_dot();
  d0 = wave_sum(d0);
  d1 = wave_sum(d1);
  if (lane == 0) {
    const float poison = (range_flag != nullptr && *range_flag != 0) ? __builtin_nanf("") : 0.f;
    const float l0 = d0 + pb[0] + poison, l1 = d1 + pb[1] + poison;
    prune_out[(size_t)tok * 2 + 0] = l0;
    prune_out[(size_t)tok * 2 + 1] = l1;
    if (keep_prob) keep_prob[tok] = 1.0f / (1.0f + expf(l0 - l1));
  }
  if (keep_all_rows) row_store_f32(rv, x + (size_t)row * H, H, lane);
  if (row_pos[row] == 0) row_store_f32(rv, cls + (size_t)row_seq[row] * H, H, lane);
  if (capture) row_store_f32(rv, capture + (size_t)tok * H, H, lane);
}

__device__ __forceinline__ float block_sum_256(float v, float* red) {
  v = wave_sum(v);
  const int wave = threadIdx.x >> 6, lane = threadIdx.x & 63;
  __syncthreads();
  if (lane == 0) red[wave] = v;
  __syncthreads();
  return (red[0] + red[1]) + (red[2] + red[3]);
}

__global__ __launch_bounds__(256) void rank_head_kernel(const float* __restrict__ cls, const float* __restrict__ y,
                                                        const int32_t* __restrict__ cu, int s0,
                                                        const int32_t* __restrict__ roff, int mean_pool, int H, int nl,
                                                        const float* __restrict__ dense_t,
                                                        const float* __restrict__ head_norm, float eps,
                                                        const float* __restrict__ cls_w, const float* __restrict__ cls_b,
                                                        float* __restrict__ rank_out, const int* __restrict__ range_flag) {
  const bool poisoned = range_flag != nullptr && *range_flag != 0;
  __shared__ float pooled[1024];
  __shared__ float z[1024];
  __shared__ float red[4];
  const int s = blockIdx.x;
  const int tid = threadIdx.x;
  const int len = cu[s0 + s + 1] - cu[s0 + s];
  if (len <= 0) {
    if (tid < nl) rank_out[(size_t)(s0 + s) * nl + tid] = 0.f;
    return;
  }
  for (int k = tid; k < H; k += 256) {
    float v;
    if (mean_pool) {
      const float* base = y + (size_t)roff[s] * H + k;
      float acc = 0.f;
      for (int p = 0; p < len; ++p) acc += base[(size_t)p * H];
      v = acc / (float)len;
    } else {
      v = cls[(size_t)s * H + k];
    }
    pooled[k] = v;
  }
  __syncthreads();
  float lsum = 0.f;
  for (int n = tid; n < H; n += 256) {
    float acc = 0.f;
    for (int k = 0; k < H; ++k) acc = fmaf(pooled[k], dense_t[(size_t)k * H + n], acc);
    const float gl = gelu_erf(acc);
    z[n] = gl;
    lsum += gl;
  }
  const float mean = block_sum_256(lsum, red) / (float)H;
  float lq = 0.f;
  for (int n = tid; n < H; n += 256) {
    const float d = z[n] - mean;
    lq += d * d;
  }
  const float var = block_sum_256(lq, red) / (float)H;
  const float rstd = 1.0f / sqrtf(var + eps);
  for (int c = 0; c < nl; ++c) {
    float part = 0.f;
    for (int n = tid; n < H; n += 256) part += (z[n] - mean) * rstd * head_norm[n] * cls_w[(size_t)c * H + n];
    const float tot = block_sum_256(part, red);
    if (tid == 0) rank_out[(size_t)(s0 + s) * nl + c] = poisoned ? __builtin_nanf("") : tot + cls_b[c];
  }
}

__global__ void convert_to_f32_kernel(const void* __restrict__ src, int dtype, size_t n, float* __restrict__ dst) {
  const size_t i = (size_t)blockIdx.x * blockDim.x + threadIdx.x;
  if (i >= n) return;
  if (dtype == 0) {
    dst[i] = reinterpret_cast<const float*>(src)[i];
  } else if (dtype == 1) {
    dst[i] = bf2f(reinterpret_cast<const u16*>(src)[i]);
  } else {
    dst[i] = __half2float(reinterpret_cast<const __half*>(src)[i]);
  }
}

__global__ void split_planes_kernel(const float* __restrict__ src, int rows, int cols, int geglu_half,
                                    u16* __restrict__ hi, u16* __restrict__ lo, int zero_lo, int* __restrict__ any_lo) {
  const size_t i = (size_t)blockIdx.x * blockDim.x + threadIdx.x;
  if (i >= (size_t)rows * cols) return;
  const int r = (int)(i / cols), c = (int)(i % cols);
  int sr = r;
  if (geglu_half > 0) {
    const int b = r >> 6, j = r & 63;
    sr = (j < 32) ? (b * 32 + j) : (geglu_half + b * 32 + (j - 32));
  }
  const float v = src[(size_t)sr * cols + c];
  const u16 h = f2bf(v);
  const u16 l = f2bf(v - bf2f(h));
  if ((l & 0x7fffu) != 0) *any_lo = 1;
  hi[i] = h;
  lo[i] = zero_lo ? (u16)0 : l;
}

__global__ void transpose_f32_kernel(const float* __restrict__ src, int rows, int cols, float* __restrict__ dst) {
  const size_t i = (size_t)blockIdx.x * blockDim.x + threadIdx.x;
  if (i >= (size_t)rows * cols) return;
  const int r = (int)(i / cols), c = (int)(i % cols);
  dst[(size_t)c * rows + r] = src[i];
}

constexpr int LN_FP_SLAB = 16 * 16 + 16;

template <bool SPLIT, bool H16 = false>
// ... 191 lines not shown
```

open_provence_amd/engine.py:

```python

from __future__ import annotations

import ctypes
import os
from contextlib import contextmanager
from dataclasses import dataclass
from typing import Iterator, Mapping, Sequence

import numpy as np
import torch

from . import _lib
from .config import EncoderDims
from .packing import pack_rows

_PRECISIONS = {"bf16x3": _lib.OP_PRECISION_BF16X3, "bf16x2": _lib.OP_PRECISION_BF16X2, "bf16": _lib.OP_PRECISION_BF16}
_ENV_FLAGS = {
    "OPEN_PROVENCE_FORCE_TILED": _lib.OP_FLAG_FORCE_TILED,
    "OPEN_PROVENCE_NO_SMALL_BLOCKS": _lib.OP_FLAG_NO_SMALL_BLOCKS,
    "OPEN_PROVENCE_NO_POLICY_KERNELS": _lib.OP_FLAG_NO_POLICY_KERNELS,
    "OPEN_PROVENCE_NO_LAYER_FUSION": _lib.OP_FLAG_NO_LAYER_FUSION,
    "OPEN_PROVENCE_LAYER_8X16": _lib.OP_FLAG_LAYER_8X16,
    "OPEN_PROVENCE_LAYER_M32": _lib.OP_FLAG_LAYER_M32,
    "OPEN_PROVENCE_NO_HEAD_FUSION": _lib.OP_FLAG_NO_HEAD_FUSION,
    "OPEN_PROVENCE_NO_F8": _lib.OP_FLAG_NO_F8,
    "OPEN_PROVENCE_ATTN_XCD_GROUP": _lib.OP_FLAG_ATTN_XCD_GROUP,
    "OPEN_PROVENCE_PANEL_F8": _lib.OP_FLAG_PANEL_F8,
    "OPEN_PROVENCE_PANEL_F8_WI": _lib.OP_FLAG_PANEL_F8_WI,
    "OPEN_PROVENCE_NO_LAYER_PAIRS": _lib.OP_FLAG_NO_LAYER_PAIRS,
}


@dataclass(frozen=True)
class HiddenRequest:

    layers: "Sequence[int] | None" = None
    dtype: torch.dtype = torch.float32
    pad_width: int = 0


def parse_precision(precision: "str | Mapping[str, int]") -> tuple[int, list[int]]:

    terms = [3] * len(_lib.OP_FAMILIES) + [0] * (8 - len(_lib.OP_FAMILIES))
    if isinstance(precision, str) and precision in _PRECISIONS:
        return _PRECISIONS[precision], terms
    if isinstance(precision, str):
        try:
            mapping = {k.strip(): int(v) for k, v in (item.split("=") for item in precision.split(",") if item.strip())}
        except ValueError as exc:
            raise ValueError(f"precision must be one of {sorted(_PRECISIONS)} or 'family=mask,...': {precision!r}") from exc
    else:
        mapping = dict(precision)
    for name, mask in mapping.items():
        if name not in _lib.OP_FAMILIES:
            raise ValueError(f"unknown contraction family {name!r}; expected one of {_lib.OP_FAMILIES}")
        if int(mask) not in (0, 1, 2, 3):
            raise ValueError(f"term mask of {name!r} must be 0..3, got {mask!r}")
        terms[_lib.OP_FAMILIES.index(name)] = int(mask)
    return _lib.OP_PRECISION_CUSTOM, terms
_DTYPES = {torch.float32: _lib.OP_DTYPE_F32, torch.bfloat16: _lib.OP_DTYPE_BF16, torch.float16: _lib.OP_DTYPE_F16}

DEFAULT_CALIBRATION_TOLERANCE = 1e-4
PATH_TOLERANCE = 1e-3


def resolve_calibration_tolerance(calibrate: "bool | float | None") -> float:

    if isinstance(calibrate, (bool, np.bool_)):
        if not calibrate:
            return 0.0
        calibrate = None
    if calibrate is not None:
        tolerance = float(calibrate)
        if isinstance(calibrate, (int, np.integer)) and tolerance == 1.0:
            calibrate = None
        elif not tolerance < PATH_TOLERANCE:
            raise ValueError(f"calibration tolerance {calibrate!r} is not inside the path's own bar ({PATH_TOLERANCE:g} on a logit): "
                             "any candidate would pass; use kernel_set= to pin a set regardless of its error")
        else:
            return max(tolerance, 0.0)
    env = os.environ.get("OPEN_PROVENCE_CALIBRATE", "").strip().lower()
    if env in ("0", "off", "false", "no"):
        return 0.0
    if env and env not in ("1", "on", "true", "yes"):
        try:
            tolerance = max(float(env), 0.0)
            if not tolerance < PATH_TOLERANCE:
                raise ValueError
            return tolerance
        except ValueError as exc:
            raise ValueError(f"OPEN_PROVENCE_CALIBRATE must be 0 / off or a tolerance below {PATH_TOLERANCE:g}, got {env!r}") from exc
    return DEFAULT_CALIBRATION_TOLERANCE


def require_gpu(device: torch.device | str | int | None = None) -> torch.device:

    if not torch.cuda.is_available():
        raise _lib.HipLibraryError(
            "No HIP device visible to PyTorch-ROCm: the OpenProvence MI355X path runs only on a GPU "
            "(there is no CPU fallback; the CPU restatement under oracle/ is test infrastructure)."
        )
    if device is None:
        return torch.device("cuda", torch.cuda.current_device())
    dev = torch.device(device) if not isinstance(device, int) else torch.device("cuda", device)
    if dev.type != "cuda":
        raise _lib.HipLibraryError(f"device {dev} is not a HIP device")
    if dev.index is None:
        dev = torch.device("cuda", torch.cuda.current_device())
    return dev


class HipEncoder:

    def __init__(
        self,
        dims: EncoderDims,
        *,
        device: torch.device | str | int | None = None,
        precision: "str | Mapping[str, int]" = "bf16x3",
        chunk_rows: int | None = None,
        prune_pre_final_norm: bool = False,
        flags: int | None = None,
    ) -> None:
        precision_code, terms = parse_precision(precision)
        self.lib = _lib.load_library()
        self.device = require_gpu(device)
        self.dims = dims
        self.precision = precision
        if dims.num_layers > _lib.OP_MAX_LAYERS:
            raise ValueError("too many layers")
        cfg = _lib.OpConfig()
        cfg.struct_bytes = ctypes.sizeof(_lib.OpConfig)
        cfg.device_id = int(self.device.index)
        cfg.vocab_size = dims.vocab_size
        cfg.hidden_size = dims.hidden_size
        cfg.intermediate_size = dims.intermediate_size
        cfg.num_layers = dims.num_layers
        cfg.num_heads = dims.num_heads
        cfg.num_labels = dims.num_labels
        cfg.local_attention = dims.local_attention
        cfg.max_position_embeddings = dims.max_position_embeddings
        cfg.pooling = _lib.OP_POOL_MEAN if dims.classifier_pooling == "mean" else _lib.OP_POOL_CLS
        cfg.precision = precision_code
        for i, mask in enumerate(terms):
            cfg.terms[i] = mask
        if flags is None:
            flags = 0
            for name, bit in _ENV_FLAGS.items():
                if os.environ.get(name):
                    flags |= bit
            waves = os.environ.get("OPEN_PROVENCE_ATT_WAVES")
            if waves:
                flags |= _lib.OP_FLAG_ATT_WAVES_4 if int(waves) == 4 else _lib.OP_FLAG_ATT_WAVES_8
        cfg.flags = int(flags)
        cfg.prune_pre_final_norm = 1 if prune_pre_final_norm else 0
        self.prune_pre_final_norm = bool(prune_pre_final_norm)
        cfg.norm_eps = dims.norm_eps
        cfg.global_rope_theta = dims.global_rope_theta
        cfg.local_rope_theta = dims.local_rope_theta
        cfg.chunk_rows = int(chunk_rows or 0)
        for i, flag in enumerate(dims.layer_is_global):
            cfg.layer_is_global[i] = 1 if flag else 0
        handle = ctypes.c_void_p()
        code = self.lib.op_create(ctypes.byref(cfg), ctypes.byref(handle))
        _lib.check(self.lib, None, code, "op_create")
        self._handle = handle
        self._split_state: dict | None = None
        self._workspace: torch.Tensor | None = None
        self._capture: torch.Tensor | None = None
        self._capture_result: torch.Tensor | None = None
        self.calibration: dict | None = None

    def close(self) -> None:
        handle = getattr(self, "_handle", None)
        if handle is not None and handle.value:
            self.lib.op_destroy(handle)
            self._handle = ctypes.c_void_p()
        self._split_state = None

    def __del__(self) -> None:
        try:
            self.close()
# ... 528 lines not shown
```

Measured before the change: 68150.

## Keep residual stream in tiled layout at layer 0 and fuse final head into last layer

Layer 0's embedding+LayerNorm+QKV kernel now writes the residual stream directly in the tiled layout that the paired fused-layer kernels use. The first pair kernel can then read it tiled instead of converting from row layout. The last layer, which has no QKV, now also runs through the paired layer16p kernel, with the final norm, prune head and hidden capture fused in. This removes the row-layout conversions at both ends of the stack and the separate final head kernel. It adds more template variants and a new tiled hidden-capture kernel, and an env flag restores the old row-layout path.

```diff
diff --git a/include/open_provence_hip.h b/include/open_provence_hip.h
--- a/include/open_provence_hip.h
+++ b/include/open_provence_hip.h
@@ -51,6 +51,7 @@
   OP_FLAG_PANEL_F8 = 2048,
   OP_FLAG_PANEL_F8_WI = 4096,
   OP_FLAG_NO_LAYER_PAIRS = 8192,
+  OP_FLAG_ROW_LAYOUT_ENDS = 16384,
   OP_FLAG_NO_F8 = 512
 };
 
diff --git a/microbench/qkv0_stamps.hip b/microbench/qkv0_stamps.hip
--- /dev/null
+++ b/microbench/qkv0_stamps.hip
@@ -0,0 +1,151 @@
+#include <hip/hip_runtime.h>
+
+#include <cstdio>
+#include <cstdlib>
+#include <cstring>
+#include <vector>
+
+#include "opk_rowgemm.hip.h"
+
+using namespace opk;
+
+#define CHECK(x)                                                                    \
+  do {                                                                              \
+    hipError_t e_ = (x);                                                            \
+    if (e_ != hipSuccess) {                                                         \
+      fprintf(stderr, "%s:%d %s\n", __FILE__, __LINE__, hipGetErrorString(e_));     \
+      return 1;                                                                     \
+    }                                                                               \
+  } while (0)
+
+static u16 f2h_host(float f) {
+  _Float16 h = (_Float16)f;
+  u16 u;
+  memcpy(&u, &h, 2);
+  return u;
+}
+
+int main() {
+  const int R = getenv("Q0_ROWS") ? atoi(getenv("Q0_ROWS")) : 131072;
+  constexpr int H = 256, KS = 8, V = 102400, SEQ = 512;
+  if (R % 128) return 2;
+  std::vector<float> emb((size_t)V * H), lnw(H, 1.0f), cs((size_t)8192 * ROPE_HALF, 0.5f);
+  std::vector<u16> w((size_t)3 * H * H * 2);
+  std::vector<int32_t> ids(R), tok(R), pos(R);
+  unsigned s = 12345;
+  auto rnd = [&]() { s = s * 1664525u + 1013904223u; return s; };
+  for (auto& v : emb) v = ((int)(rnd() >> 9) / 8388608.0f - 0.5f) * 0.08f;
+  for (auto& v : w) v = f2h_host(((int)(rnd() >> 9) / 8388608.0f - 0.5f) * 0.08f);
+  for (int i = 0; i < R; ++i) {
+    ids[i] = (int32_t)(rnd() % V);
+    tok[i] = i;
+    pos[i] = i % SEQ;
+  }
+  float *d_emb, *d_ln, *d_cos, *d_sin, *d_x;
+  u16 *d_w, *d_q, *d_k, *d_v;
+  int32_t *d_ids, *d_tok, *d_pos;
+  CHECK(hipMalloc(&d_emb, emb.size() * 4));
+  CHECK(hipMalloc(&d_ln, H * 4));
+  CHECK(hipMalloc(&d_cos, cs.size() * 4));
+  CHECK(hipMalloc(&d_sin, cs.size() * 4));
+  CHECK(hipMalloc(&d_x, (size_t)R * H * 4));
+  CHECK(hipMalloc(&d_w, w.size() * 2));
+  CHECK(hipMalloc(&d_q, (size_t)R * H * 2 * 2));
+  CHECK(hipMalloc(&d_k, (size_t)R * H * 2 * 2));
+  CHECK(hipMalloc(&d_v, (size_t)R * H * 2 * 2));
+  CHECK(hipMalloc(&d_ids, R * 4));
+  CHECK(hipMalloc(&d_tok, R * 4));
+  CHECK(hipMalloc(&d_pos, R * 4));
+  CHECK(hipMemcpy(d_emb, emb.data(), emb.size() * 4, hipMemcpyHostToDevice));
+  CHECK(hipMemcpy(d_ln, lnw.data(), H * 4, hipMemcpyHostToDevice));
+  CHECK(hipMemcpy(d_cos, cs.data(), cs.size() * 4, hipMemcpyHostToDevice));
+  CHECK(hipMemcpy(d_sin, cs.data(), cs.size() * 4, hipMemcpyHostToDevice));
+  CHECK(hipMemcpy(d_w, w.data(), w.size() * 2, hipMemcpyHostToDevice));
+  CHECK(hipMemcpy(d_ids, ids.data(), R * 4, hipMemcpyHostToDevice));
+  CHECK(hipMemcpy(d_tok, tok.data(), R * 4, hipMemcpyHostToDevice));
+  CHECK(hipMemcpy(d_pos, pos.data(), R * 4, hipMemcpyHostToDevice));
+
+  RowGemmParams p;
+  memset(&p, 0, sizeof(p));
+  p.eps = 1e-5f;
+  p.hidden = H;
+  p.r_pad = R;
+  p.row_pos = d_pos;
+  p.rope_cos = d_cos;
+  p.rope_sin = d_sin;
+  p.max_pos = 8192;
+  p.x_in = d_x;
+  p.x_io = d_x;
+  p.ln_w = d_ln;
+  p.wp = d_w;
+  p.n_chunks = 3 * H / ROW_CHUNK;
+  p.n_swapped = 2 * H / ROW_CHUNK;
+  p.o0_hi = d_q;
+  p.o1_hi = d_k;
+  p.o2_hi = d_v;
+  p.ld_out = H;
+  p.emb_table = d_emb;
+  p.emb_ids = d_ids;
+  p.emb_vocab = V;
+  p.row_tok = d_tok;
+  const int blocks = R / 128;
+#ifdef OPK_TIMING
+  CHECK(hipMalloc(&p.dbg, (size_t)blocks * 16 * 8));
+  CHECK(hipMemset(p.dbg, 0, (size_t)blocks * 16 * 8));
+#endif
+  auto launch = [&]() {
+#ifdef Q0_XT
+    hipLaunchKernelGGL((rowgemm_xt_kernel<KS, RE_QKV, RP_SPLIT, 0, 0, 0, 4, 2, 0, 0, 0, true>), dim3(blocks), dim3(256), 0, 0, p);
+#else
+    hipLaunchKernelGGL((rowgemm_kernel<KS, RE_QKV, RP_SPLIT, 0, 0, 0, 4, 2, 0, 0, 0, true>), dim3(blocks), dim3(256), 0, 0, p);
+#endif
+  };
+  hipEvent_t e0, e1;
+  CHECK(hipEventCreate(&e0));
+  CHECK(hipEventCreate(&e1));
+  for (int i = 0; i < 5; ++i) launch();
+  CHECK(hipDeviceSynchronize());
+  float best = 1e9f, sum = 0.f;
+  const int reps = 20;
+  for (int i = 0; i < reps; ++i) {
+    CHECK(hipEventRecord(e0));
+    launch();
+    CHECK(hipEventRecord(e1));
+    CHECK(hipEventSynchronize(e1));
+    float ms;
+    CHECK(hipEventElapsedTime(&ms, e0, e1));
+    best = ms < best ? ms : best;
+    sum += ms;
+  }
+  CHECK(hipGetLastError());
+#ifdef Q0_XT
+  const char* name = "layer-0 launch, x tiled";
+#else
+  const char* name = "layer-0 launch, x rows";
+#endif
+  printf("%s, %d rows: avg %.1f us  best %.1f us\n", name, R, sum / reps * 1e3f, best * 1e3f);
+#ifdef OPK_TIMING
+  {
+    std::vector<unsigned long long> t((size_t)blocks * 16);
+    CHECK(hipMemcpy(t.data(), p.dbg, t.size() * 8, hipMemcpyDeviceToHost));
+    double seg[4] = {0, 0, 0, 0}, w1 = 0, w2 = 0, total = 0, real = 0;
+    for (int b = 0; b < blocks; ++b) {
+      const unsigned long long* q = &t[(size_t)b * 16];
+      seg[0] += (double)(q[1] - q[0]);
+      seg[1] += (double)(q[2] - q[1]);
+      seg[2] += (double)(q[3] - q[2]);
+      seg[3] += (double)(q[5] - q[3]);
+      w1 += (double)q[10];
+      w2 += (double)q[9];
+      total += (double)(q[5] - q[0]);
+      real += (double)q[15];
+    }
+    const double n = blocks;
+    printf("  shader clock while the blocks ran: %.3f GHz\n", total / real * 0.1);
+    printf("  cycles per block (wave 0): entry + chunk-0 request %.0f | gather + LayerNorm + x stores issued %.0f | first barrier (store acks, chunk 0) %.0f | "
+           "24 chunks + q/k/v^T stores %.0f (of which vmcnt wait %.0f, barrier %.0f) | total %.0f\n",
+           seg[0] / n, seg[1] / n, seg[2] / n, seg[3] / n, w1 / n, w2 / n, total / n);
+  }
+#endif
+  return 0;
+}
diff --git a/open_provence_amd/_lib.py b/open_provence_amd/_lib.py
--- a/open_provence_amd/_lib.py
+++ b/open_provence_amd/_lib.py
@@ -24,6 +24,7 @@
 OP_FLAG_PANEL_F8 = 2048
 OP_FLAG_PANEL_F8_WI = 4096
 OP_FLAG_NO_LAYER_PAIRS = 8192
+OP_FLAG_ROW_LAYOUT_ENDS = 16384
 OP_POOL_CLS, OP_POOL_MEAN = 0, 1
 OP_KS_AUTO = -1
 KERNEL_SET_NAMES = {0: "bf16x3", 1: "bf16-weights", 2: "bf16", 3: "f16-f8", 4: "f16-f8-w", 5: "bf16x3+wi-f16-f8-w",
diff --git a/open_provence_amd/csrc/op_api.hip b/open_provence_amd/csrc/op_api.hip
--- a/open_provence_amd/csrc/op_api.hip
+++ b/open_provence_amd/csrc/op_api.hip
@@ -334,6 +334,8 @@
   const char* no_kernel = "internal: no row-stationary kernel for hidden %d";
   bool layer_fused, head_in_last_layer;
   bool pair_layers;
+  bool pair_last;
+  bool x0_tiled;
   bool head_done = false;
   int hidden_stored = -1;
 
@@ -375,6 +377,8 @@
     pair_layers = layer_fused && H == 256 && I % 64 == 0 && (f16 || h->pi == 2) && !h->capture &&
                   !(h->cfg.flags & (OP_FLAG_NO_LAYER_PAIRS | OP_FLAG_LAYER_8X16 | OP_FLAG_LAYER_M32)) &&
                   h->layers[0].wo_pp[f16 ? 1 : 0] != nullptr;
+    pair_last = pair_layers && !(h->cfg.flags & OP_FLAG_ROW_LAYOUT_ENDS);
+    x0_tiled = pair_layers && embed_in_qkv0 && h->N >= 2 && !(h->cfg.flags & OP_FLAG_ROW_LAYOUT_ENDS);
   }
 
   int prologue() {
@@ -433,6 +437,11 @@
     void* dst = hidden_entry(index);
     if (!dst) return OP_OK;
     OP_TRY(L.begin(PK_CAPTURE));
+    if (index == 0 && x0_tiled) {
+      hipLaunchKernelGGL(hidden_rows_tiled_kernel, dim3(row_blocks), dim3(256), 0, st, ws.x, r_pad, ws.row_tok, ws.row_seq, ws.row_pos,
+                         s0, hid->pad, hid->bf16, dst);
+      return L.end();
+    }
     hipLaunchKernelGGL(hidden_rows_kernel, dim3(row_blocks), dim3(256), 0, st, ws.x, ln, h->cfg.norm_eps, H, r_pad,
                        ws.row_tok, ws.row_seq, ws.row_pos, s0, hid->pad, hid->bf16, dst);
     return L.end();
@@ -543,7 +552,7 @@
         rp.x_io = ws.x;
       }
       OP_TRY(L.begin(PK_ROW_QKV));
-      if (!opl::launch_row_qkv0(st, rp, H / 32, small_blocks, h->pi, row_grid)) return fail(h, OP_ERR_UNSUPPORTED, no_kernel, H);
+      if (!opl::launch_row_qkv0(st, rp, H / 32, small_blocks, h->pi, row_grid, x0_tiled)) return fail(h, OP_ERR_UNSUPPORTED, no_kernel, H);
       OP_TRY(L.end());
       OP_TRY(clear_qkv());
       if (embed_in_qkv0) OP_TRY(hidden(0));
@@ -580,14 +589,14 @@
         OP_TRY(L.end());
         return OP_OK;
       }
-      if (pair_layers && with_qkv) {
+      if (pair_layers && (with_qkv || pair_last)) {
         Layer32Params lp;
         memset(&lp, 0, sizeof(lp));
-        const LayerWeights& nx = h->layers[li + 1];
+        const LayerWeights& nx = h->layers[with_qkv ? li + 1 : li];
         lp.o_fp = ws.o_hi;
         lp.x_io = ws.x;
         lp.ln_mlp = lw.mlp_norm;
-        lp.ln_next = nx.attn_norm;
+        lp.ln_next = with_qkv ? nx.attn_norm : nullptr;
         lp.eps = h->cfg.norm_eps;
         lp.wo_p = lw.wo_pp[f16 ? 1 : 0];
         lp.wi_p = lw.wi_pp[f16 ? 1 : 0];
@@ -599,22 +608,34 @@
         lp.vt_fp = ws.vt_hi;
         lp.r_pad = r_pad;
         lp.row_pos = ws.row_pos;
-        const int gl = h->cfg.layer_is_global[li + 1] ? 1 : 0;
+        const int gl = h->cfg.layer_is_global[with_qkv ? li + 1 : li] ? 1 : 0;
         lp.rope_cos = h->rope_cos[gl];
         lp.rope_sin = h->rope_sin[gl];
         lp.max_pos = h->max_pos;
-        lp.hid_out = hidden_entry(li + 1);
+        lp.row_tok = ws.row_tok;
+        lp.row_seq = ws.row_seq;
+        if (with_qkv) {
+          lp.hid_out = hidden_entry(li + 1);
+          if (lp.hid_out) hidden_stored = li + 1;
+        } else if (head_in_last_layer) {
+          lp.fin_ln = h->final_norm;
+          lp.fin_pw = h->prune_w;
+          lp.fin_pb = h->prune_b;
+          lp.fin_prune = prune_out;
+          lp.fin_keep = keep_prob;
+          lp.fin_cls = ws.cls;
+          lp.fin_pre_norm = h->cfg.prune_pre_final_norm ? 1 : 0;
+          head_done = true;
+          lp.hid_out = hidden_entry(h->N);
+        }
         if (lp.hid_out) {
-          lp.row_tok = ws.row_tok;
-          lp.row_seq = ws.row_seq;
           lp.hid_bf16 = hid->bf16;
           lp.hid_pad = hid->pad;
           lp.hid_s0 = s0;
-          hidden_stored = li + 1;
         }
         OP_TRY(L.begin(PK_FUSED_LAYER));
-        if (!opl::launch_layer16p(st, lp, f16, true, li > 0, li + 2 < h->N, (unsigned)(r_pad / ROW_BM),
-                                  lp.hid_out != nullptr))
+        if (!opl::launch_layer16p(st, lp, f16, with_qkv, li > 0 || x0_tiled, li + 2 < h->N || (pair_last && with_qkv),
+                                  (unsigned)(r_pad / ROW_BM), lp.hid_out != nullptr))
           return fail(h, OP_ERR_UNSUPPORTED, no_kernel, H);
         OP_TRY(L.end());
         return OP_OK;
diff --git a/open_provence_amd/csrc/op_internal.h b/open_provence_amd/csrc/op_internal.h
--- a/open_provence_amd/csrc/op_internal.h
+++ b/open_provence_amd/csrc/op_internal.h
@@ -35,7 +35,7 @@
 constexpr int h_olo(const Policy& p) { return p.mlp_out & 1; }
 constexpr bool o_lo(const Policy& p) { return (p.attn_out & 1) != 0; }
 
-bool launch_row_qkv0(hipStream_t st, const opk::RowGemmParams& p, int ks, bool small, int pi, unsigned grid);
+bool launch_row_qkv0(hipStream_t st, const opk::RowGemmParams& p, int ks, bool small, int pi, unsigned grid, bool x_tiled = false);
 bool launch_row_geglu_fused(hipStream_t st, const opk::RowGemmParams& p, int ks, bool small, int pi, unsigned grid);
 bool launch_row_qkv_fused(hipStream_t st, const opk::RowGemmParams& p, int ks, bool small, int pi, unsigned grid);
 bool launch_kstream(hipStream_t st, const opk::KStreamParams& p, int nf, int pi, unsigned grid);
@@ -44,7 +44,7 @@
                             bool waves8, bool hout = false);
 bool launch_row_layer_f8(hipStream_t st, const opk::RowGemmParams& p, int ks, bool with_qkv, unsigned grid, bool hout);
 bool launch_row_layer_f8w(hipStream_t st, const opk::RowGemmParams& p, int ks, bool with_qkv, unsigned grid, bool hout);
-bool launch_row_qkv0_h16(hipStream_t st, const opk::RowGemmParams& p, int ks, bool small, unsigned grid);
+bool launch_row_qkv0_h16(hipStream_t st, const opk::RowGemmParams& p, int ks, bool small, unsigned grid, bool x_tiled = false);
 bool launch_row_layer_h16(hipStream_t st, const opk::RowGemmParams& p, int ks, bool with_qkv, unsigned grid, bool waves8, bool hout);
 bool has_layer32(int pi);
 bool launch_layer32(hipStream_t st, const opk::Layer32Params& p, int pi, bool with_qkv, unsigned grid);
diff --git a/open_provence_amd/csrc/op_launch_layer32.hip b/open_provence_amd/csrc/op_launch_layer32.hip
--- a/open_provence_amd/csrc/op_launch_layer32.hip
+++ b/open_provence_amd/csrc/op_launch_layer32.hip
@@ -41,13 +41,15 @@
 }
 
 bool launch_layer16p(hipStream_t st, const Layer32Params& p, bool h16, bool with_qkv, bool xin_t, bool xout_t, unsigned grid, bool hout) {
-  if (hout && !with_qkv) return false;
+  if (hout && !with_qkv && p.fin_ln == nullptr) return false;
+  if (!with_qkv && xout_t) return false;
   const dim3 g(grid), b(512);
 #define OPL_L16P(H16, XI, XO)                                                                              \
   do {                                                                                                     \
-    if (hout) hipLaunchKernelGGL((layer16p_hout_kernel<8, true, H16, XI, XO>), g, b, 0, st, p);            \
-    else if (with_qkv) hipLaunchKernelGGL((layer16p_kernel<8, true, H16, XI, XO>), g, b, 0, st, p);        \
-    else hipLaunchKernelGGL((layer16p_kernel<8, false, H16, XI, XO>), g, b, 0, st, p);                     \
+    if (!with_qkv && hout) hipLaunchKernelGGL((layer16p_hout_kernel<8, false, H16, XI, false>), g, b, 0, st, p); \
+    else if (!with_qkv) hipLaunchKernelGGL((layer16p_kernel<8, false, H16, XI, false>), g, b, 0, st, p);   \
+    else if (hout) hipLaunchKernelGGL((layer16p_hout_kernel<8, true, H16, XI, XO>), g, b, 0, st, p);       \
+    else hipLaunchKernelGGL((layer16p_kernel<8, true, H16, XI, XO>), g, b, 0, st, p);                      \
   } while (0)
   if (h16) {
     if (xin_t && xout_t) OPL_L16P(true, true, true);
diff --git a/open_provence_amd/csrc/op_launch_row.hip b/open_provence_amd/csrc/op_launch_row.hip
--- a/open_provence_amd/csrc/op_launch_row.hip
+++ b/open_provence_amd/csrc/op_launch_row.hip
@@ -61,8 +61,14 @@
 #endif
 
 #if OPL_ROW_PART == 2
-bool launch_row_qkv0(hipStream_t st, const RowGemmParams& p, int ks, bool small, int pi, unsigned grid) {
-  if (pi == PI_F16) return launch_row_qkv0_h16(st, p, ks, small, grid);
+bool launch_row_qkv0(hipStream_t st, const RowGemmParams& p, int ks, bool small, int pi, unsigned grid, bool x_tiled) {
+  if (pi == PI_F16) return launch_row_qkv0_h16(st, p, ks, small, grid, x_tiled);
+  if (x_tiled) {
+    if (pi != PI_BF16 || ks != 8 || p.emb_table == nullptr) return false;
+    if (small) hipLaunchKernelGGL((rowgemm_xt_kernel<8, RE_QKV, RP_SPLIT, 0, 0, 0, 4, 1>), dim3(grid), dim3(256), 0, st, p);
+    else hipLaunchKernelGGL((rowgemm_xt_kernel<8, RE_QKV, RP_SPLIT, 0, 0, 0, 4, 2>), dim3(grid), dim3(256), 0, st, p);
+    return true;
+  }
 #define OPL_CALL(PI) (launch_ks<RE_QKV, RP_SPLIT, 0, kPolicies[PI].wqkv, qkv_olo(kPolicies[PI])>(st, p, ks, small, grid))
   OPL_SWITCH(OPL_CALL)
 #undef OPL_CALL
@@ -191,7 +197,13 @@
 }
 }
 
-bool launch_row_qkv0_h16(hipStream_t st, const RowGemmParams& p, int ks, bool small, unsigned grid) {
+bool launch_row_qkv0_h16(hipStream_t st, const RowGemmParams& p, int ks, bool small, unsigned grid, bool x_tiled) {
+  if (x_tiled) {
+    if (ks != 8 || p.emb_table == nullptr) return false;
+    if (small) hipLaunchKernelGGL((rowgemm_xt_kernel<8, RE_QKV, RP_SPLIT, 0, 0, 0, 4, 1, 0, 0, 0, true>), dim3(grid), dim3(256), 0, st, p);
+    else hipLaunchKernelGGL((rowgemm_xt_kernel<8, RE_QKV, RP_SPLIT, 0, 0, 0, 4, 2, 0, 0, 0, true>), dim3(grid), dim3(256), 0, st, p);
+    return true;
+  }
   if (ks == 8) launch_qkv0_h16_ks<8>(st, p, small, grid);
   else if (ks == 4) launch_qkv0_h16_ks<4>(st, p, small, grid);
   else return false;
diff --git a/open_provence_amd/csrc/opk_layer16p_body.inc b/open_provence_amd/csrc/opk_layer16p_body.inc
--- a/open_provence_amd/csrc/opk_layer16p_body.inc
+++ b/open_provence_amd/csrc/opk_layer16p_body.inc
@@ -1,5 +1,4 @@
   static_assert(NT == 8, "written for hidden = 256");
-  static_assert(!HOUT || QKV, "the hidden-state store rides on the q / k / v^T loop's x stores");
   constexpr int H = NT * 32;
   constexpr int KP = NT;
   constexpr int CHUNK = KP * 2 * 512;
@@ -46,6 +45,7 @@
   const float ln_fill0 = p.ln_mlp[ln_i];
   float ln_fill1 = 0.f;
   if (QKV) ln_fill1 = p.ln_next[ln_i];
+  else if (p.fin_ln != nullptr) ln_fill1 = p.fin_ln[ln_i];
 
   const uint32_t lds0 = (uint32_t)(uintptr_t)((__attribute__((address_space(3))) u16*)&sW[0]) + (uint32_t)lane * 16u;
   const uint32_t stat_addr = (uint32_t)(uintptr_t)((__attribute__((address_space(3))) float*)&sStat[0]);
@@ -387,7 +387,127 @@
   L16P_STAMP(3);
 
   if constexpr (!QKV) {
-    store_rows();
+    if (p.fin_ln == nullptr) {
+      store_rows();
+    } else {
+      asm volatile("s_nop 15\n\ts_nop 7"
+                   : "+v"(acc1[0][0][0]), "+v"(acc1[0][0][1]), "+v"(acc1[0][1][0]), "+v"(acc1[0][1][1]), "+v"(acc1[1][0][0]), "+v"(acc1[1][0][1]),
+                     "+v"(acc1[1][1][0]), "+v"(acc1[1][1][1]), "+v"(acc1[2][0][0]), "+v"(acc1[2][0][1]), "+v"(acc1[2][1][0]), "+v"(acc1[2][1][1]),
+                     "+v"(acc1[3][0][0]), "+v"(acc1[3][0][1]), "+v"(acc1[3][1][0]), "+v"(acc1[3][1][1]));
+      float mean_a[2], m2_a[2];
+#pragma unroll
+      for (int mf = 0; mf < 2; ++mf) {
+        f32x2 v[4][4];
+#pragma unroll
+        for (int i = 0; i < 4; ++i)
+#pragma unroll
+          for (int fh = 0; fh < 2; ++fh) {
+            const f32x4 t = acc1[i][fh][mf];
+            v[i][2 * fh] = f32x2{t[0], t[1]};
+            v[i][2 * fh + 1] = f32x2{t[2], t[3]};
+          }
+        f32x2 s4[4];
+#pragma unroll
+        for (int i = 0; i < 4; ++i)
+#pragma unroll
+          for (int q = 0; q < 4; ++q) s4[q] = i == 0 ? v[i][q] : pk_add(s4[q], v[i][q]);
+        const f32x2 st2 = pk_add(pk_add(s4[0], s4[1]), pk_add(s4[2], s4[3]));
+        float sum = st2.x + st2.y;
+        sum += __shfl_xor(sum, 16, 64);
+        sum += __shfl_xor(sum, 32, 64);
+        mean_a[mf] = sum * (1.0f / 128.0f);
+        const f32x2 ma2 = f32x2{mean_a[mf], mean_a[mf]};
+        f32x2 q4s[4];
+#pragma unroll
+        for (int i = 0; i < 4; ++i)
+#pragma unroll
+          for (int q = 0; q < 4; ++q) {
+            const f32x2 c = pk_sub(v[i][q], ma2);
+            q4s[q] = i == 0 ? pk_mul(c, c) : pk_fma(c, c, q4s[q]);
+          }
+        const f32x2 qt2 = pk_add(pk_add(q4s[0], q4s[1]), pk_add(q4s[2], q4s[3]));
+        float m2 = qt2.x + qt2.y;
+        m2 += __shfl_xor(m2, 16, 64);
+        m2 += __shfl_xor(m2, 32, 64);
+        m2_a[mf] = m2;
+        lds_write_f2(stat_addr + (uint32_t)(((wave * 2 + mf) * 16 + n16) * 8), f32x2{mean_a[mf], m2});
+      }
+      asm volatile("s_waitcnt lgkmcnt(0)" ::: "memory");
+      block_barrier();
+      const float* lw = &sLn[H + 128 * hf + 8 * g];
+      const float* pw0 = p.fin_pw + 128 * hf + 8 * g;
+      const float* pw1 = pw0 + H;
+      const bool pre = p.fin_pre_norm != 0;
+      const uint32_t dot_addr = lds0 - lane16;
+      int tok[2];
+#pragma unroll
+      for (int mf = 0; mf < 2; ++mf) {
+        const int row = m0 + 16 * mf + n16;
+        tok[mf] = p.row_tok[row];
+        const bool is_cls = tok[mf] >= 0 && p.row_pos[row] == 0;
+        const f32x2 other = lds_read_f2(stat_addr + (uint32_t)((((wave ^ 4) * 2 + mf) * 16 + n16) * 8));
+        const float mean = 0.5f * (mean_a[mf] + other.x);
+        const float dm = mean_a[mf] - other.x;
+        const float m2 = (m2_a[mf] + other.y) + dm * dm * 64.0f;
+        const float rstd = 1.0f / sqrtf(m2 * (1.0f / (float)H) + p.eps);
+        const f32x2 mn2 = f32x2{mean, mean}, r2 = f32x2{rstd, rstd};
+        f32x2 d0[2], d1[2];
+        d0[0] = d0[1] = d1[0] = d1[1] = f32x2{0.f, 0.f};
+        float* cls_dst = is_cls ? p.fin_cls + (size_t)p.row_seq[row] * H + 128 * hf + 8 * g : nullptr;
+#pragma unroll
+        for (int i = 0; i < 4; ++i) {
+          const f32x4 w0 = *reinterpret_cast<const f32x4*>(lw + 32 * i), w1 = *reinterpret_cast<const f32x4*>(lw + 32 * i + 4);
+          const float4 a0 = *reinterpret_cast<const float4*>(pw0 + 32 * i), a1 = *reinterpret_cast<const float4*>(pw0 + 32 * i + 4);
+          const float4 c0 = *reinterpret_cast<const float4*>(pw1 + 32 * i), c1 = *reinterpret_cast<const float4*>(pw1 + 32 * i + 4);
+          const f32x4 t0 = acc1[i][0][mf], t1 = acc1[i][1][mf];
+          const f32x2 x[4] = {f32x2{t0[0], t0[1]}, f32x2{t0[2], t0[3]}, f32x2{t1[0], t1[1]}, f32x2{t1[2], t1[3]}};
+          const f32x2 lwv[4] = {f32x2{w0[0], w0[1]}, f32x2{w0[2], w0[3]}, f32x2{w1[0], w1[1]}, f32x2{w1[2], w1[3]}};
+          const f32x2 pa[4] = {f32x2{a0.x, a0.y}, f32x2{a0.z, a0.w}, f32x2{a1.x, a1.y}, f32x2{a1.z, a1.w}};
+          const f32x2 pc[4] = {f32x2{c0.x, c0.y}, f32x2{c0.z, c0.w}, f32x2{c1.x, c1.y}, f32x2{c1.z, c1.w}};
+          f32x2 y[4], hv[4];
+#pragma unroll
+          for (int j = 0; j < 4; ++j) {
+            y[j] = pk_mul(pk_mul(pk_sub(x[j], mn2), r2), lwv[j]);
+            hv[j] = pre ? x[j] : y[j];
+            d0[j & 1] = pk_fma(hv[j], pa[j], d0[j & 1]);
+            d1[j & 1] = pk_fma(hv[j], pc[j], d1[j & 1]);
+          }
+          if constexpr (HOUT) {
+            if (hid_row[mf] >= 0) {
+              const size_t e = (size_t)hid_row[mf] * H + 128 * hf + 32 * i + 8 * g;
+              hidden_store4(p.hid_out, p.hid_bf16, e, hv[0].x, hv[0].y, hv[1].x, hv[1].y);
+              hidden_store4(p.hid_out, p.hid_bf16, e + 4, hv[2].x, hv[2].y, hv[3].x, hv[3].y);
+            }
+          }
+          if (is_cls) {
+            *reinterpret_cast<float4*>(cls_dst + 32 * i) = make_float4(y[0].x, y[0].y, y[1].x, y[1].y);
+            *reinterpret_cast<float4*>(cls_dst + 32 * i + 4) = make_float4(y[2].x, y[2].y, y[3].x, y[3].y);
+          }
+        }
+        const f32x2 e0 = pk_add(d0[0], d0[1]), e1 = pk_add(d1[0], d1[1]);
+        float l0 = e0.x + e0.y, l1 = e1.x + e1.y;
+        l0 += __shfl_xor(l0, 16, 64);
+        l0 += __shfl_xor(l0, 32, 64);
+        l1 += __shfl_xor(l1, 16, 64);
+        l1 += __shfl_xor(l1, 32, 64);
+        if (g == 0) lds_write_f2(dot_addr + (uint32_t)(((wave * 2 + mf) * 16 + n16) * 8), f32x2{l0, l1});
+      }
+      asm volatile("s_waitcnt lgkmcnt(0)" ::: "memory");
+      block_barrier();
+      if (hf == 0 && g == 0) {
+        const float b0 = p.fin_pb[0], b1 = p.fin_pb[1];
+#pragma unroll
+        for (int mf = 0; mf < 2; ++mf) {
+          if (tok[mf] < 0) continue;
+          const f32x2 own = lds_read_f2(dot_addr + (uint32_t)(((wave * 2 + mf) * 16 + n16) * 8));
+          const f32x2 oth = lds_read_f2(dot_addr + (uint32_t)((((wave ^ 4) * 2 + mf) * 16 + n16) * 8));
+          const float l0 = (own.x + oth.x) + b0, l1 = (own.y + oth.y) + b1;
+          p.fin_prune[(size_t)tok[mf] * 2 + 0] = l0;
+          p.fin_prune[(size_t)tok[mf] * 2 + 1] = l1;
+          if (p.fin_keep) p.fin_keep[tok[mf]] = 1.0f / (1.0f + expf(l0 - l1));
+        }
+      }
+    }
     L16P_STAMP(4);
   } else {
     constexpr int N_IT = 3 * NT / 2;
diff --git a/open_provence_amd/csrc/opk_layer32.hip.h b/open_provence_amd/csrc/opk_layer32.hip.h
--- a/open_provence_amd/csrc/opk_layer32.hip.h
+++ b/open_provence_amd/csrc/opk_layer32.hip.h
@@ -85,6 +85,13 @@
   int hid_bf16;
   int hid_pad;
   int hid_s0;
+  const float* fin_ln;
+  const float* fin_pw;
+  const float* fin_pb;
+  float* fin_prune;
+  float* fin_keep;
+  float* fin_cls;
+  int fin_pre_norm;
 };
 
 template <int NT, bool QKV, bool ALO, int OLO>
diff --git a/open_provence_amd/csrc/opk_rowgemm.hip.h b/open_provence_amd/csrc/opk_rowgemm.hip.h
--- a/open_provence_amd/csrc/opk_rowgemm.hip.h
+++ b/open_provence_amd/csrc/opk_rowgemm.hip.h
@@ -6,7 +6,7 @@
 
 namespace opk {
 
-template <int KS, int EPI, int PRO, int T1, int T2, int OLO, int WAVES, int MF, int TW, int TM, int F8, bool H16, bool HOUT = false>
+template <int KS, int EPI, int PRO, int T1, int T2, int OLO, int WAVES, int MF, int TW, int TM, int F8, bool H16, bool HOUT = false, bool XT = false>
 struct RowGemmBlock {
   static constexpr bool WLO = F8 == 2;
   static_assert(!H16 || (F8 == 0 && T1 == 0 && T2 == 0 && OLO == 0 && TW == 0 && TM == 0 && PRO != RP_KSTREAM && EPI != RE_GEGLU),
@@ -266,10 +266,19 @@
       stage_chunk(0, 0);
     }
 
-    rowgemm_prologue_rows<KS, MF, PRO, A_LO, H16>(p, m0, l15, g, a_hi, a_lo);
+#ifdef OPK_TIMING
+    if (!PHASE1) OPK_STAMP(1);
+#endif
+    rowgemm_prologue_rows<KS, MF, PRO, A_LO, H16, XT>(p, m0, l15, g, a_hi, a_lo);
     if (EPI == RE_QKV && !ROPE_PRELOAD) rope_rows();
+#ifdef OPK_TIMING
+    if (!PHASE1) OPK_STAMP(2);
+#endif
     if constexpr (LN_V2) __builtin_amdgcn_s_barrier();
     else __syncthreads();
+#ifdef OPK_TIMING
+    if (!PHASE1) OPK_STAMP(3);
+#endif
 
     if constexpr (QKV_PAIRS) qkv_pairs_loop();
     else chunk_loop();
@@ -278,8 +287,8 @@
 
 }
 
-#define OPK_RG_TPL template <int KS, int EPI, int PRO, int T1, int T2, int OLO, int WAVES, int MF, int TW, int TM, int F8, bool H16, bool HOUT>
-#define OPK_RG_BLOCK RowGemmBlock<KS, EPI, PRO, T1, T2, OLO, WAVES, MF, TW, TM, F8, H16, HOUT>
+#define OPK_RG_TPL template <int KS, int EPI, int PRO, int T1, int T2, int OLO, int WAVES, int MF, int TW, int TM, int F8, bool H16, bool HOUT, bool XT>
+#define OPK_RG_BLOCK RowGemmBlock<KS, EPI, PRO, T1, T2, OLO, WAVES, MF, TW, TM, F8, H16, HOUT, XT>
 #include "opk_rowgemm_phase1.hip.h"
 #include "opk_rowgemm_mlp.hip.h"
 #include "opk_rowgemm_qkv_pairs.hip.h"
@@ -310,6 +319,16 @@
   block.run();
 }
 
+template <int KS, int EPI, int PRO, int T1, int T2, int OLO, int WAVES, int MF = 2, int TW = 0, int TM = 0, int F8 = 0, bool H16 = false>
+__global__ __launch_bounds__(WAVES * 64, (MF == 1 && WAVES == 8) ? 4 : 2) void rowgemm_xt_kernel(RowGemmParams p) {
+  static_assert(EPI == RE_QKV && PRO == RP_SPLIT && KS == 8, "the tiled residual stream is the wave-pair kernel's: hidden = 256, layer 0");
+  using Block = RowGemmBlock<KS, EPI, PRO, T1, T2, OLO, WAVES, MF, TW, TM, F8, H16, false, true>;
+  __shared__ __attribute__((aligned(16))) u16 sW[2][Block::STAGE_ALLOC];
+  __shared__ __attribute__((aligned(16))) float sLn[Block::SLN_SIZE];
+  Block block(p, sW, sLn);
+  block.run();
+}
+
 }
 
 #include "opk_kstream.hip.h"
diff --git a/open_provence_amd/csrc/opk_rowgemm_ln.hip.h b/open_provence_amd/csrc/opk_rowgemm_ln.hip.h
--- a/open_provence_amd/csrc/opk_rowgemm_ln.hip.h
+++ b/open_provence_amd/csrc/opk_rowgemm_ln.hip.h
@@ -175,11 +175,89 @@
   }
 }
 
-template <int KS, int MF, int PRO, bool A_LO, bool H16>
+template <int KS, int MF, int PRO, bool A_LO, bool H16, bool XT = false>
 __device__ __forceinline__ void rowgemm_prologue_rows(const RowGemmParams& p, int m0, int l15, int g, bf16x8 (&a_hi)[MF][KS],
                                                       bf16x8 (&a_lo)[MF][KS]) {
   constexpr int K = KS * 32;
-  if (PRO == RP_SPLIT && p.emb_table != nullptr) {
+  if constexpr (XT) {
+    static_assert(PRO == RP_SPLIT, "layer 0");
+    const float* lnw_g = p.ln_w + g * 8;
+    int tok[MF];
+#pragma unroll
+    for (int mf = 0; mf < MF; ++mf) tok[mf] = p.row_tok[m0 + mf * 16 + l15];
+    const float* src[MF];
+#pragma unroll
+    for (int mf = 0; mf < MF; ++mf) {
+      int id = p.emb_ids[tok[mf] < 0 ? 0 : tok[mf]];
+      id = id < 0 ? 0 : (id >= p.emb_vocab ? p.emb_vocab - 1 : id);
+      src[mf] = p.emb_table + (size_t)id * K + g * 8;
+    }
+    float4 f0[MF][KS], f1[MF][KS], w0[KS], w1[KS];
+#pragma unroll
+    for (int mf = 0; mf < MF; ++mf)
+#pragma unroll
+      for (int ks = 0; ks < KS; ++ks) {
+        f0[mf][ks] = *reinterpret_cast<const float4*>(src[mf] + ks * 32);
+        f1[mf][ks] = *reinterpret_cast<const float4*>(src[mf] + ks * 32 + 4);
+      }
+#pragma unroll
+    for (int ks = 0; ks < KS; ++ks) {
+      w0[ks] = *reinterpret_cast<const float4*>(lnw_g + ks * 32);
+      w1[ks] = *reinterpret_cast<const float4*>(lnw_g + ks * 32 + 4);
+    }
+    asm volatile("" ::: "memory");
+    __builtin_amdgcn_sched_barrier(0);
+#pragma unroll
+    for (int mf = 0; mf < MF; ++mf) {
+      const float live = tok[mf] < 0 ? 0.f : 1.f;
+      const f32x2 live2 = f32x2{live, live};
+      f32x2 v[4 * KS];
+#pragma unroll
+      for (int ks = 0; ks < KS; ++ks) {
+        v[4 * ks + 0] = pk_mul(f32x2{f0[mf][ks].x, f0[mf][ks].y}, live2);
+        v[4 * ks + 1] = pk_mul(f32x2{f0[mf][ks].z, f0[mf][ks].w}, live2);
+        v[4 * ks + 2] = pk_mul(f32x2{f1[mf][ks].x, f1[mf][ks].y}, live2);
+        v[4 * ks + 3] = pk_mul(f32x2{f1[mf][ks].z, f1[mf][ks].w}, live2);
+      }
+      f32x2 s4[4] = {v[0], v[1], v[2], v[3]};
+#pragma unroll
+      for (int i = 4; i < 4 * KS; ++i) s4[i & 3] = pk_add(s4[i & 3], v[i]);
+      const f32x2 st = pk_add(pk_add(s4[0], s4[1]), pk_add(s4[2], s4[3]));
+      float sum = st.x + st.y;
+      sum += __shfl_xor(sum, 16, 64);
+      sum += __shfl_xor(sum, 32, 64);
+      const float mean = sum * (1.0f / (float)K);
+      const f32x2 m2 = f32x2{mean, mean};
+      f32x2 q4[4];
+#pragma unroll
+      for (int i = 0; i < 4 * KS; ++i) {
+        v[i] = pk_sub(v[i], m2);
+        q4[i & 3] = i < 4 ? pk_mul(v[i], v[i]) : pk_fma(v[i], v[i], q4[i & 3]);
+      }
+      const f32x2 qt = pk_add(pk_add(q4[0], q4[1]), pk_add(q4[2], q4[3]));
+      float q = qt.x + qt.y;
+      q += __shfl_xor(q, 16, 64);
+      q += __shfl_xor(q, 32, 64);
+      const float rstd = 1.0f / sqrtf(q * (1.0f / (float)K) + p.eps);
+      const f32x2 r2 = f32x2{rstd, rstd};
+      float* xt = p.x_io + (size_t)((m0 + mf * 16) >> 5) * (KS * 1024) + (((m0 >> 4) + mf) & 1) * 512 + (g * 16 + l15) * 4;
+#pragma unroll
+      for (int ks = 0; ks < KS; ++ks) {
+        const f32x2 lw[4] = {f32x2{w0[ks].x, w0[ks].y}, f32x2{w0[ks].z, w0[ks].w}, f32x2{w1[ks].x, w1[ks].y}, f32x2{w1[ks].z, w1[ks].w}};
+        f32x2 y[4];
+        uint32_t hb[4], lb[4];
+#pragma unroll
+        for (int j = 0; j < 4; ++j) {
+          y[j] = pk_mul(pk_mul(v[4 * ks + j], r2), lw[j]);
+          split2x_pk<A_LO, H16>(y[j], hb[j], lb[j]);
+        }
+        store_stream16(xt + ks * 1024, make_float4(y[0].x, y[0].y, y[1].x, y[1].y));
+        store_stream16(xt + ks * 1024 + 256, make_float4(y[2].x, y[2].y, y[3].x, y[3].y));
+        a_hi[mf][ks] = as_frag(make_uint4(hb[0], hb[1], hb[2], hb[3]));
+        a_lo[mf][ks] = as_frag(make_uint4(lb[0], lb[1], lb[2], lb[3]));
+      }
+    }
+  } else if (PRO == RP_SPLIT && p.emb_table != nullptr) {
     const float* lnw_g = p.ln_w + g * 8;
 #pragma unroll
     for (int mf = 0; mf < MF; ++mf) {
diff --git a/open_provence_amd/csrc/opk_small.hip.h b/open_provence_amd/csrc/opk_small.hip.h
--- a/open_provence_amd/csrc/opk_small.hip.h
+++ b/open_provence_amd/csrc/opk_small.hip.h
@@ -205,6 +205,21 @@
     const int c = lane + 64 * k;
     if (c < nchunk) hidden_store4(out, bf16, base + 4 * c, rv.v[k].x, rv.v[k].y, rv.v[k].z, rv.v[k].w);
   }
+}
+
+__global__ __launch_bounds__(256) void hidden_rows_tiled_kernel(const float* __restrict__ x, int r_pad, const int32_t* __restrict__ row_tok,
+                                                                const int32_t* __restrict__ row_seq, const int32_t* __restrict__ row_pos,
+                                                                int s0, int pad, int bf16, void* __restrict__ out) {
+  constexpr int H = 256;
+  const int c = threadIdx.x & 63;
+  const int row = blockIdx.x * 4 + (threadIdx.x >> 6);
+  if (row >= r_pad) return;
+  const int tok = row_tok[row];
+  if (tok < 0) return;
+  const int T = c >> 3, g = (c & 7) >> 1, fh = c & 1;
+  const float4 v = *reinterpret_cast<const float4*>(x + ((size_t)(row >> 5) * (H / 32) + T) * 1024 + (2 * ((row >> 4) & 1) + fh) * 256 +
+                                                    (16 * g + (row & 15)) * 4);
+  hidden_store4(out, bf16, hidden_dst_row(tok, row_seq[row], row_pos[row], pad, s0) * (size_t)H + 4 * c, v.x, v.y, v.z, v.w);
 }
 
 __global__ __launch_bounds__(256) void final_ln_prune_kernel(float* __restrict__ x, const float* __restrict__ lnw,
diff --git a/open_provence_amd/engine.py b/open_provence_amd/engine.py
--- a/open_provence_amd/engine.py
+++ b/open_provence_amd/engine.py
@@ -28,6 +28,7 @@
     "OPEN_PROVENCE_PANEL_F8": _lib.OP_FLAG_PANEL_F8,
     "OPEN_PROVENCE_PANEL_F8_WI": _lib.OP_FLAG_PANEL_F8_WI,
     "OPEN_PROVENCE_NO_LAYER_PAIRS": _lib.OP_FLAG_NO_LAYER_PAIRS,
+    "OPEN_PROVENCE_ROW_LAYOUT_ENDS": _lib.OP_FLAG_ROW_LAYOUT_ENDS,
 }
 
 
```

New measurement: 68510 (median of 6 runs). No clear change (+0.5%).
